# NickTravers/NeuralNetworkLibrary

Hardware: AMD Instinct MI355X
Metric: ResNet-34 224x224 training throughput (Learner.train1minibatch, fwd+loss+bwd+optimizer) (higher is better)
Workload: dtype f32; 1 GPU; DogsCats ResNet-34 classifier, 224x224, bs=64 per GPU, SGD momentum 0.9, fp32; global_batch=64, image_size=224, parallelism=dp1

## Files before the change

include/nnl.h:

```cpp
#ifndef NNL_H_
#define NNL_H_

#include <stddef.h>
#include <stdint.h>

#ifdef __cplusplus
extern "C" {
#endif

typedef enum {
  NNL_OK = 0,
  NNL_ERR_INVALID_ARG = -1,
  NNL_ERR_HIP = -2,
  NNL_ERR_UNSUPPORTED = -3,
  NNL_ERR_WORKSPACE = -4
} nnl_status_t;

int nnl_version(void);
const char* nnl_last_error(void);
int nnl_reload_env(void);

enum { NNL_PROF_CONV_FWD = 0, NNL_PROF_CONV_DGRAD = 1, NNL_PROF_CONV_WGRAD = 2, NNL_PROF_EMBDOT = 3,
       NNL_PROF_TABULAR = 4, NNL_PROF_RETINA_LOSS = 5, NNL_PROF_LSTM = 6, NNL_PROF_SOFTMAX_CE = 7,
       NNL_PROF_ELEMENTWISE = 8, NNL_PROF_GEMM = 9, NNL_PROF_OPTIM = 10, NNL_PROF_KINDS = 11 };
int nnl_prof_enable(int enable);
int nnl_prof_collect(int64_t* launches, double* total_ms, double* total_work);
int nnl_prof_collect2(int64_t* launches, double* total_ms, double* total_work, double* total_exec);
int nnl_dp_bump(int32_t* step, void* stream);
int nnl_dp_signal(int32_t* flag, const int32_t* step, void* stream);
int nnl_dp_wait(const int32_t* flag, int32_t value, int64_t timeout_us, int32_t* err, void* stream);
const char* nnl_source_stamp(void);

int nnl_embdotbias_fwd(const int64_t* x, const float* U, const float* M, const float* bu, const float* bi,
                       float* y, float* z, int64_t n, int64_t n_user, int64_t n_item, int64_t D,
                       int has_range, float lo, float hi, int32_t* err_flag, void* stream);
size_t nnl_embdotbias_bwd_workspace_bytes(int64_t n);
int nnl_embdotbias_bwd(const int64_t* x, const float* U, const float* M, const float* z, const float* dy,
                       float* dU, float* dM, float* dbu, float* dbi, int64_t n, int64_t n_user,
                       int64_t n_item, int64_t D, int has_range, float lo, float hi, void* workspace, size_t workspace_bytes, void* stream);

typedef struct {
  int32_t N, H, W, C;
  int32_t K, R, S;
  int32_t stride, pad;
  int32_t P, Q;
} nnl_conv_geom_t;

size_t nnl_conv2d_fwd_workspace_bytes(const nnl_conv_geom_t* g);
int64_t nnl_conv2d_tile_counters(void);
int nnl_conv2d_fwd(const float* x, const float* w, const float* bias, float* y, const nnl_conv_geom_t* g,
                   int relu, void* workspace, size_t workspace_bytes, int32_t* tile_counters, float* bn_partials,
                   const float* bn_pivot, int32_t* bn_rows, void* stream);
int nnl_conv2d_fwd_add_up2(const float* x, const float* w, const float* bias, const float* small, float* y,
                           const nnl_conv_geom_t* g, void* stream);
int nnl_upsample2_bwd(const float* dy, float* dsmall, int64_t N, int64_t h, int64_t w, int64_t C, void* stream);
int nnl_conv2d_weight_transpose(const float* w, float* wt, int K, int R, int S, int C, void* stream);
typedef struct {
  const float* w;
  float* wt;
  int32_t K, RS, C, first_tile;
} nnl_wt_desc_t;
int nnl_conv2d_weight_transpose_multi(const nnl_wt_desc_t* desc, const int32_t* tile_tensor, int64_t n_tiles,
                                      double total_elems, void* stream);
size_t nnl_conv2d_dgrad_workspace_bytes(const nnl_conv_geom_t* g);
int nnl_conv2d_dgrad(const float* dy, const float* wt, float* dx, const nnl_conv_geom_t* g, const float* addend,
                     void* workspace, size_t workspace_bytes, int32_t* tile_counters, void* stream);
typedef struct {
  const float* src;
  float* dst;
  int32_t rows, ch, flip, first_block;
  int32_t two_d, reserved;
} nnl_wino_desc_t;
int nnl_conv2d_wino_preferred(const nnl_conv_geom_t* g, int dgrad);
int nnl_wino_filter_multi(const nnl_wino_desc_t* desc, const int32_t* block_desc, int64_t n_blocks, void* stream);
int nnl_conv2d_fwd_pre(const float* x, const float* w, const float* bias, float* y, const nnl_conv_geom_t* g, int relu,
                       void* workspace, size_t workspace_bytes, int32_t* tile_counters, float* bn_partials, const float* bn_pivot,
                       int32_t* bn_rows, const float* u, void* stream);
int nnl_conv2d_dgrad_pre(const float* dy, const float* wt, float* dx, const nnl_conv_geom_t* g, const float* addend,
                         void* workspace, size_t workspace_bytes, int32_t* tile_counters, const float* u, void* stream);
size_t nnl_debug_conv_wino_workspace_bytes(int N, int H, int W, int C, int K);
int nnl_debug_conv_wino_fwd(const float* x, const float* filt, const float* bias, const float* add, float* y, void* ws,
                            size_t ws_bytes, int32_t* counters, long n_counters, float* bn_part, const float* bn_pivot, int N,
                            int H, int W, int C, int K, int relu, int flip, void* stream);
size_t nnl_debug_conv_wino2_workspace_bytes(int N, int H, int W, int C, int K);
int nnl_debug_conv_wino2_fwd(const float* x, const float* filt, const float* bias, const float* add, float* y, void* ws,
                            size_t ws_bytes, int32_t* counters, long n_counters, float* bn_part, const float* bn_pivot, int N,
                            int H, int W, int C, int K, int relu, int flip, void* stream);
int nnl_debug_conv_plan_times(int N, int H, int W, int C, int K, double* out);

int nnl_debug_route_record(int enable);
int nnl_debug_route_collect(char* out, size_t n);
size_t nnl_conv2d_wgrad_workspace_bytes(const nnl_conv_geom_t* g);
int nnl_conv2d_wgrad(const float* x, const float* dy, float* dw, const nnl_conv_geom_t* g, void* workspace,
                     size_t workspace_bytes, void* stream);
size_t nnl_colsum_workspace_bytes(int64_t rows, int64_t cols);
int nnl_sum_tensors(const float* const* src, int n, float* out, int64_t numel, void* stream);
int nnl_colsum(const float* a, float* out, int64_t rows, int64_t cols, void* workspace, size_t workspace_bytes,
               void* stream);
int nnl_relu_gate_colsum(const float* dy, const float* y, float* g, float* colsum, int64_t rows, int64_t cols, void* workspace,
                         size_t workspace_bytes, void* stream);
int nnl_act_gate_colsum(const float* dy, const float* y, float* g, float* colsum, int64_t rows, int64_t cols, int act,
                        void* workspace, size_t workspace_bytes, void* stream);

size_t nnl_bn_workspace_bytes(int64_t rows, int64_t C);
int nnl_bn_fwd(const float* x, const float* gamma, const float* beta, const float* residual, float* y,
               float* save_mean, float* save_invstd, float* running_mean, float* running_var, int64_t rows,
               int64_t C, float eps, float momentum, int training, int relu, int64_t* num_batches_tracked,
               uint32_t* relu_mask, const float* ext_partials, int64_t ext_rows, const float* ext_pivot, float* pivot_out,
               void* workspace, size_t workspace_bytes, void* stream);
int nnl_bn_bwd(const float* dy, const float* y, const uint32_t* relu_mask, const float* x, const float* gamma,
               const float* mean, const float* invstd, float* dx, float* dres, float* dgamma, float* dbeta, int64_t rows,
               int64_t C, int training, int relu, void* workspace, size_t workspace_bytes, void* stream);

int nnl_bn_relu_maxpool_supported(int64_t C);
int nnl_bn_relu_maxpool_fwd(const float* x, const float* gamma, const float* beta, float* y, uint8_t* idx, float* save_mean,
                            float* save_invstd, float* save_scale, float* save_shift, float* running_mean, float* running_var,
                            int64_t N, int64_t H, int64_t W, int64_t C, int64_t P, int64_t Q, int ks, int stride, int pad, float eps,
                            float momentum, int training, int64_t* num_batches_tracked, void* workspace, size_t workspace_bytes,
                            void* stream);
int nnl_bn_relu_maxpool_bwd(const float* dpool, const float* y, const uint8_t* idx, const float* x, const float* gamma,
                            const float* beta, const float* mean, const float* invstd, const float* scale, const float* shift,
                            float* dx, float* dgamma, float* dbeta,
                            int64_t N, int64_t H, int64_t W, int64_t C, int64_t P, int64_t Q, int ks, int stride, int pad,
                            int training, void* workspace, size_t workspace_bytes, void* stream);

int nnl_bn_sync_stats(const float* x, float* stats, int64_t rows, int64_t C, void* workspace, size_t workspace_bytes,
                      void* stream);
int nnl_bn_sync_fwd(const float* x, const float* all_stats, int world, const float* gamma, const float* beta,
                    const float* residual, float* y, float* save_mean, float* save_invstd, float* running_mean,
                    float* running_var, int64_t rows, int64_t C, float eps, float momentum, int relu,
                    int64_t* num_batches_tracked, uint32_t* relu_mask, void* workspace, size_t workspace_bytes, void* stream);
int nnl_bn_sync_bwd_reduce(const float* dy, const float* y, const uint32_t* relu_mask, const float* x, const float* mean,
                           const float* invstd, float* sums, int64_t rows, int64_t C, int relu, void* workspace,
                           size_t workspace_bytes, void* stream);
int nnl_bn_sync_bwd(const float* dy, const float* y, const uint32_t* relu_mask, const float* x, const float* gamma,
                    const float* mean, const float* invstd, const float* local_sums, const float* global_sums,
                    const float* all_stats,
                    int world, float* dx, float* dres, float* dgamma, float* dbeta, int64_t rows, int64_t C, int relu,
                    void* workspace, size_t workspace_bytes, void* stream);

int nnl_maxpool2d_fwd(const float* x, float* y, uint8_t* idx, int64_t N, int64_t H, int64_t W, int64_t C, int64_t P,
                      int64_t Q, int ksize, int stride, int pad, void* stream);
int nnl_maxpool2d_bwd(const float* dy, const uint8_t* idx, float* dx, int64_t N, int64_t H, int64_t W, int64_t C,
                      int64_t P, int64_t Q, int ksize, int stride, int pad, void* stream);
int nnl_concat_pool_fwd(const float* x, float* out, int32_t* argmax, int64_t N, int64_t HW, int64_t C, void* stream);
int nnl_concat_pool_bwd(const float* dout, const int32_t* argmax, float* dx, int64_t N, int64_t HW, int64_t C, void* stream);

int nnl_bbox_decode(const float* anchors, const float* reg, const float* clas, int64_t bs, int64_t A, int64_t K,
                    const float* mean4, const float* std4, float thresh, float width, float height, float* cand_boxes,
                    int32_t* cand_classes, float* cand_scores, int32_t* cand_order, int32_t* cand_count, void* stream);
size_t nnl_nms_workspace_bytes(int64_t bs, int64_t top_k);
int nnl_nms(const float* cand_boxes, const int32_t* cand_classes, const float* cand_scores, const int32_t* cand_order,
            const int32_t* cand_count, int64_t bs, int64_t cap, int64_t top_k, float max_overlap, float* kept_boxes,
            int32_t* kept_classes, float* kept_scores, int32_t* kept_count, void* workspace, size_t workspace_bytes,
            void* stream);

int nnl_tab_renorm(const int64_t* xcat, float* const* tables, const int32_t* card, const int32_t* dim,
                   const int32_t* row_off, const int32_t* row_table, int32_t* flags, int64_t bs, int32_t ncat,
                   int32_t total_rows, float max_norm, int32_t* err_flag, void* stream);
int nnl_tab_gather_fwd(const int64_t* xcat, const float* const* tables, const int32_t* card, const int32_t* dim,
                       const int32_t* col_off, const int32_t* col_table, const float* row_mask, const float* cont,
                       const float* cont_mask, float* out, int64_t bs, int32_t ncat, int32_t cat_width,
                       int32_t n_cont, int32_t ld_out, void* stream);
size_t nnl_tab_scatter_bwd_workspace_bytes(int64_t bs, int32_t ncat);
int nnl_tab_scatter_bwd(const int64_t* xcat, const int32_t* card, const int32_t* dim, const int32_t* col_off,
                        const int32_t* col_table, const int64_t* grad_off, const float* row_mask,
                        const float* cont_mask, const float* dout, float* dtab_flat, int64_t dtab_elems,
                        float* dcont, int64_t bs, int32_t ncat, int32_t cat_width, int32_t n_cont, int32_t ld_out,
                        void* workspace, size_t workspace_bytes, void* stream);
int nnl_tab_scan_bwd(const int64_t* xcat, const int32_t* card, const int32_t* dim, const int32_t* col_off,
                     const int64_t* grad_off, const float* row_mask, const float* cont_mask, const float* dout,
                     float* dtab_flat, float* dcont, const int32_t* blk_col, const int32_t* blk_first, int32_t n_scan_blocks,
                     int32_t max_dim, int64_t bs, int32_t ncat, int32_t cat_width, int32_t n_cont, int32_t ld_out, void* stream);

int nnl_pad_cols(const float* src, float* dst, int64_t rows, int64_t C, int64_t Cp, void* stream);
int nnl_keep_masks(const float* u, float* a, int64_t na, float keep_a, float* b, int64_t nb, float keep_b, void* stream);

int nnl_linear_small_supported(int64_t N);
int nnl_linear_small_fwd(const float* x, const float* w, const float* bias, float* y, int64_t M, int64_t K, int64_t ldx, int64_t N,
                         void* stream);
size_t nnl_linear_small_bwd_workspace_bytes(int64_t M, int64_t K, int64_t N);
int nnl_linear_small_bwd(const float* dy, const float* x, const float* w, float* dx, float* dw, float* db, int64_t M, int64_t K,
                         int64_t ldx, int64_t N, void* workspace, size_t workspace_bytes, void* stream);

size_t nnl_retina_loss_workspace_bytes(int64_t bs, int64_t A);
int nnl_retina_loss_fwd(const float* anchors, const float* reg, const float* clas, const float* boxes,
                        const int64_t* cats, int32_t* state, float* npos, float* out, int64_t bs, int64_t A,
                        int64_t K, int64_t M, float beta, float alpha, float gamma, void* workspace,
                        size_t workspace_bytes, void* stream);
int nnl_retina_loss_bwd(const float* anchors, const float* reg, const float* clas, const float* boxes,
                        const int64_t* cats, const int32_t* state, const float* npos, const float* grad_out,
                        float* dreg, float* dclas, int64_t bs, int64_t A, int64_t K, int64_t M, float beta,
                        float alpha, float gamma, void* stream);

int64_t nnl_lstm_padded_hidden(int64_t H);
// ... 59 lines not shown
```

neuralnetworklibrary_amd/Applications/VisionModels/resnet.py:

```python
import torch.nn as nn

from .retinanet import BasicBlock, Bottleneck, HipConv2d, HipMaxPool2d, _Downsample
from ... import ops

__all__ = ['ResNet', 'resnet18', 'resnet34', 'resnet50', 'resnet101', 'resnet152']


class ResNet(nn.Module):
    def __init__(self, block, layers, num_classes=1000):
        super().__init__()
        self.inplanes = 64
        self.conv1 = HipConv2d(3, 64, kernel_size=7, stride=2, padding=3, bias=False)
        self.bn1 = nn.BatchNorm2d(64)
        self.relu = nn.ReLU(inplace=True)
        self.maxpool = HipMaxPool2d(kernel_size=3, stride=2, padding=1)
        self.layer1 = self._make_layer(block, 64, layers[0])
        self.layer2 = self._make_layer(block, 128, layers[1], stride=2)
        self.layer3 = self._make_layer(block, 256, layers[2], stride=2)
        self.layer4 = self._make_layer(block, 512, layers[3], stride=2)
        self.avgpool = nn.AdaptiveAvgPool2d((1, 1))
        self.fc = nn.Linear(512 * block.expansion, num_classes)
        for m in self.modules():
            if isinstance(m, nn.Conv2d):
                nn.init.kaiming_normal_(m.weight, mode='fan_out', nonlinearity='relu')
            elif isinstance(m, nn.BatchNorm2d):
                nn.init.constant_(m.weight, 1)
                nn.init.constant_(m.bias, 0)

    def _make_layer(self, block, planes, blocks, stride=1):
        downsample = None
        if stride != 1 or self.inplanes != planes * block.expansion:
            downsample = _Downsample(
                HipConv2d(self.inplanes, planes * block.expansion, kernel_size=1, stride=stride, bias=False),
                nn.BatchNorm2d(planes * block.expansion))
        layers = [block(self.inplanes, planes, stride, downsample)]
        self.inplanes = planes * block.expansion
        for _ in range(1, blocks):
            layers.append(block(self.inplanes, planes))
        return nn.Sequential(*layers)

    def forward(self, x):
        x = ops.conv_bn_relu_maxpool(self.conv1, self.bn1, self.maxpool, x)
        x = self.layer4(self.layer3(self.layer2(self.layer1(x))))
        x = self.avgpool(x).flatten(1)
        return ops.linear(x, self.fc.weight, self.fc.bias, relu=False)


class ResNetBody(nn.Sequential):

    def forward(self, x):
        mods = list(self.children())
        if len(mods) >= 4 and isinstance(mods[0], HipConv2d) and isinstance(mods[1], nn.BatchNorm2d) \
                and isinstance(mods[2], nn.ReLU) and isinstance(mods[3], nn.MaxPool2d):
            x = ops.conv_bn_relu_maxpool(mods[0], mods[1], mods[3], x)
            mods = mods[4:]
        elif len(mods) >= 3 and isinstance(mods[0], HipConv2d) and isinstance(mods[1], nn.BatchNorm2d) \
                and isinstance(mods[2], nn.ReLU):
            x = ops.conv_bn_act(mods[0], mods[1], x, relu=True)
            mods = mods[3:]
        for m in mods:
            x = m(x)
        return x


def resnet18(pretrained=False, **kw):
    return ResNet(BasicBlock, [2, 2, 2, 2], **kw)


def resnet34(pretrained=False, **kw):
    return ResNet(BasicBlock, [3, 4, 6, 3], **kw)


def resnet50(pretrained=False, **kw):
    return ResNet(Bottleneck, [3, 4, 6, 3], **kw)


def resnet101(pretrained=False, **kw):
    return ResNet(Bottleneck, [3, 4, 23, 3], **kw)


def resnet152(pretrained=False, **kw):
    return ResNet(Bottleneck, [3, 8, 36, 3], **kw)
```

neuralnetworklibrary_amd/Applications/VisionModels/retinanet.py:

```python
import numpy as np
import torch
import torch.nn as nn

from ... import ops
from ...General.Core import default_device

__all__ = ['HipConv2d', 'conv3x3', 'BasicBlock', 'Bottleneck', 'PyramidFeatures', 'RegressionModel',
           'ClassificationModel', 'RetinaNet', 'retinanet18', 'retinanet34', 'retinanet50', 'retinanet101',
           'retinanet152', 'get_anchor_set', 'get_anchor_shifts', 'AnchorGenerator', 'intersections', 'jaccard', 'nms',
           'BBoxPredictor']


class HipConv2d(nn.Conv2d):
    fuse_relu = False
    nnl_hip_conv = True

    def __init__(self, *args, **kwargs):
        super().__init__(*args, **kwargs)
        self.weight.data = self.weight.data.contiguous(memory_format=torch.channels_last)

    def forward(self, x, grad_slot=None, give_slot=None):
        if self.dilation != (1, 1) or self.groups != 1 or self.stride[0] != self.stride[1] \
                or self.padding[0] != self.padding[1] or self.padding_mode != 'zeros':
            raise NotImplementedError('HipConv2d: only the symmetric, dense convolutions the reference uses')
        return ops.conv2d(x, ops.fan_param(self.weight), ops.fan_param(self.bias), self.stride[0], self.padding[0], relu=self.fuse_relu,
                          grad_slot=grad_slot, give_slot=give_slot)


class HipMaxPool2d(nn.MaxPool2d):

    def forward(self, x):
        k, s, p = self.kernel_size, self.stride, self.padding
        if self.dilation != 1 or self.ceil_mode or self.return_indices or not all(isinstance(v, int) for v in (k, s, p)):
            raise NotImplementedError('HipMaxPool2d: only the square floor-mode pooling the reference uses')
        return ops.maxpool2d(x, k, s, p)


class _ConvReLU(HipConv2d):
    fuse_relu = True


def conv3x3(in_planes, out_planes, stride=1):
    return HipConv2d(in_planes, out_planes, kernel_size=3, stride=stride, padding=1, bias=False)


class BasicBlock(nn.Module):
    expansion = 1

    def __init__(self, inplanes, planes, stride=1, downsample=None):
        super().__init__()
        self.conv1 = conv3x3(inplanes, planes, stride)
        self.bn1 = nn.BatchNorm2d(planes)
        self.relu = nn.ReLU(inplace=True)
        self.conv2 = conv3x3(planes, planes)
        self.bn2 = nn.BatchNorm2d(planes)
        self.downsample = downsample
        self.stride = stride

    def forward(self, x):
        slot = ops.GradSlot() if (x.requires_grad and torch.is_grad_enabled()) else None
        out = ops.conv_bn_act(self.conv1, self.bn1, x, relu=True, conv_slot=slot)
        if self.downsample is None:
            return ops.conv_bn_act(self.conv2, self.bn2, out, residual=x, relu=True, bn_slot=slot)
        return ops.conv_bn_act(self.conv2, self.bn2, out, residual=_shortcut(self.downsample, x, slot), relu=True)


class Bottleneck(nn.Module):
    expansion = 4

    def __init__(self, inplanes, planes, stride=1, downsample=None):
        super().__init__()
        self.conv1 = HipConv2d(inplanes, planes, kernel_size=1, bias=False)
        self.bn1 = nn.BatchNorm2d(planes)
        self.conv2 = HipConv2d(planes, planes, kernel_size=3, stride=stride, padding=1, bias=False)
        self.bn2 = nn.BatchNorm2d(planes)
        self.conv3 = HipConv2d(planes, planes * 4, kernel_size=1, bias=False)
        self.bn3 = nn.BatchNorm2d(planes * 4)
        self.relu = nn.ReLU(inplace=True)
        self.downsample = downsample
        self.stride = stride

    def forward(self, x):
        slot = ops.GradSlot() if (x.requires_grad and torch.is_grad_enabled()) else None
        out = ops.conv_bn_act(self.conv1, self.bn1, x, relu=True, conv_slot=slot)
        out = ops.conv_bn_act(self.conv2, self.bn2, out, relu=True)
        if self.downsample is None:
            return ops.conv_bn_act(self.conv3, self.bn3, out, residual=x, relu=True, bn_slot=slot)
        return ops.conv_bn_act(self.conv3, self.bn3, out, residual=_shortcut(self.downsample, x, slot), relu=True)


class _Downsample(nn.Sequential):

    def forward(self, x, give_slot=None):
        return ops.conv_bn_act(self[0], self[1], x, relu=False, conv_give=give_slot)


def _shortcut(downsample, x, slot):
    return downsample(x, give_slot=slot) if isinstance(downsample, _Downsample) else downsample(x)


class PyramidFeatures(nn.Module):

    def __init__(self, C3_size, C4_size, C5_size, feature_size=256):
        super().__init__()
        self.P5_1 = HipConv2d(C5_size, feature_size, kernel_size=1, stride=1, padding=0)
        self.P5_upsampled = nn.Upsample(scale_factor=2, mode='nearest')
        self.P5_2 = HipConv2d(feature_size, feature_size, kernel_size=3, stride=1, padding=1)
        self.P4_1 = HipConv2d(C4_size, feature_size, kernel_size=1, stride=1, padding=0)
        self.P4_upsampled = nn.Upsample(scale_factor=2, mode='nearest')
        self.P4_2 = HipConv2d(feature_size, feature_size, kernel_size=3, stride=1, padding=1)
        self.P3_1 = HipConv2d(C3_size, feature_size, kernel_size=1, stride=1, padding=0)
        self.P3_2 = HipConv2d(feature_size, feature_size, kernel_size=3, stride=1, padding=1)
        self.P6 = HipConv2d(C5_size, feature_size, kernel_size=3, stride=2, padding=1)
        self.P7_1 = nn.ReLU()
        self.P7_2 = HipConv2d(feature_size, feature_size, kernel_size=3, stride=2, padding=1)

    @staticmethod
    def _fusable(lateral, big, small):
        return (big.is_cuda and lateral.kernel_size == (1, 1) and lateral.stride == (1, 1) and big.shape[1] % 16 == 0
                and big.shape[2] == 2 * small.shape[2] and big.shape[3] == 2 * small.shape[3])

    def forward(self, inputs):
        C3, C4, C5 = inputs
        P5_x = self.P5_1(C5)
        if self._fusable(self.P4_1, C4, P5_x) and self._fusable(self.P3_1, C3, C4):
            P4_x = ops.conv_add_upsampled(C4, self.P4_1.weight, self.P4_1.bias, P5_x)
            P5_x = self.P5_2(P5_x)
            P3_x = self.P3_2(ops.conv_add_upsampled(C3, self.P3_1.weight, self.P3_1.bias, P4_x))
            P4_x = self.P4_2(P4_x)
        else:
            P5_up = self.P5_upsampled(P5_x)
            P5_x = self.P5_2(P5_x)
            P4_x = P5_up + self.P4_1(C4)
            P4_up = self.P4_upsampled(P4_x)
            P4_x = self.P4_2(P4_x)
            P3_x = self.P3_2(self.P3_1(C3) + P4_up)
        P6_x = self.P6(C5)
        P7_x = self.P7_2(self.P7_1(P6_x))
        return [P3_x, P4_x, P5_x, P6_x, P7_x]


class _Head(nn.Module):

    def _build(self, num_features_in, feature_size, n_out, bn, drop):
        self.drop0 = nn.Dropout(drop[0]) if drop else None
        self.drop = nn.Dropout(drop[1]) if drop else None
        self.bn0 = nn.BatchNorm2d(num_features_in, momentum=0.01) if bn else None
        chans = [num_features_in, feature_size, feature_size, feature_size, feature_size]
        for i in range(1, 5):
            setattr(self, 'conv%d' % i, _ConvReLU(chans[i - 1], feature_size, kernel_size=3, padding=1))
            setattr(self, 'act%d' % i, nn.ReLU())
            setattr(self, 'bn%d' % i, nn.BatchNorm2d(feature_size, momentum=0.01) if bn else None)
        self.output = HipConv2d(feature_size, n_out, kernel_size=3, padding=1)

    def _trunk(self, x, sigmoid=False):
        if self.bn0:
            x = self.bn0(x)
        if self.drop0:
            x = self.drop0(x)
        out = x
        for i in range(1, 5):
            out = getattr(self, 'conv%d' % i)(out)
            bn = getattr(self, 'bn%d' % i)
            if bn:
                out = bn(out)
            if self.drop:
                out = self.drop(out)
        o = self.output
        if sigmoid and out.shape[1] % 16 == 0 and o.stride == (1, 1) and o.padding[0] == o.padding[1]:
            return ops.conv2d(out, o.weight, o.bias, 1, o.padding[0], relu=2)
        out = o(out)
        return self.output_act(out) if sigmoid else out


class RegressionModel(_Head):

    def __init__(self, num_features_in, num_anchors=9, feature_size=256, bn=False, drop=None):
        super().__init__()
        self._build(num_features_in, feature_size, num_anchors * 4, bn, drop)

    def forward(self, x):
        out = self._trunk(x)
        return out.permute(0, 2, 3, 1).reshape(out.shape[0], -1, 4)


class ClassificationModel(_Head):

    def __init__(self, num_features_in, num_anchors=9, num_classes=80, feature_size=256, bn=False, drop=None):
        super().__init__()
        self.num_classes, self.num_anchors = num_classes, num_anchors
        self._build(num_features_in, feature_size, num_anchors * num_classes, bn, drop)
        self.output_act = nn.Sigmoid()

    def forward(self, x):
        out = self._trunk(x, sigmoid=True)
        return out.permute(0, 2, 3, 1).reshape(out.shape[0], -1, self.num_classes)


class RetinaNet(nn.Module):

    def __init__(self, num_classes, block, layers):
        self.inplanes = 64
        super().__init__()
        self.conv1 = HipConv2d(3, 64, kernel_size=7, stride=2, padding=3, bias=False)
        self.bn1 = nn.BatchNorm2d(64)
        self.relu = nn.ReLU(inplace=True)
        self.maxpool = HipMaxPool2d(kernel_size=3, stride=2, padding=1)
        self.layer1 = self._make_layer(block, 64, layers[0])
        self.layer2 = self._make_layer(block, 128, layers[1], stride=2)
        self.layer3 = self._make_layer(block, 256, layers[2], stride=2)
        self.layer4 = self._make_layer(block, 512, layers[3], stride=2)
        last = 'conv2' if block == BasicBlock else 'conv3'
        fpn_sizes = [getattr(self.layer2[layers[1] - 1], last).out_channels,
                     getattr(self.layer3[layers[2] - 1], last).out_channels,
                     getattr(self.layer4[layers[3] - 1], last).out_channels]
        self.fpn = PyramidFeatures(fpn_sizes[0], fpn_sizes[1], fpn_sizes[2])
        self.regressionModel = RegressionModel(256)
        self.classificationModel = ClassificationModel(256, num_classes=num_classes)
        self.AnchorGenerator = AnchorGenerator()
        self.BBoxPredictor = BBoxPredictor()
        init_retina_modules(self.modules())
        prior = 0.01
        nn.init.constant_(self.classificationModel.output.weight, 0)
        nn.init.constant_(self.classificationModel.output.bias, -np.log((1.0 - prior) / prior))
        nn.init.constant_(self.regressionModel.output.weight, 0)
        nn.init.constant_(self.regressionModel.output.bias, 0)

    def _make_layer(self, block, planes, blocks, stride=1):
        downsample = None
        if stride != 1 or self.inplanes != planes * block.expansion:
            downsample = _Downsample(
                HipConv2d(self.inplanes, planes * block.expansion, kernel_size=1, stride=stride, bias=False),
                nn.BatchNorm2d(planes * block.expansion))
        layers = [block(self.inplanes, planes, stride, downsample)]
        self.inplanes = planes * block.expansion
        for _ in range(1, blocks):
            layers.append(block(self.inplanes, planes))
        return nn.Sequential(*layers)

    def stem(self, x):
        return ops.conv_bn_relu_maxpool(self.conv1, self.bn1, self.maxpool, x)

    def forward(self, img_batch):
        x = self.stem(img_batch)
        x1 = self.layer1(x)
        x2 = self.layer2(x1)
        x3 = self.layer3(x2)
        x4 = self.layer4(x3)
        features = self.fpn([x2, x3, x4])
        with ops.shared_params([self.regressionModel, self.classificationModel], len(features)):
            reg = torch.cat([self.regressionModel(f) for f in features], dim=1)
            clas = torch.cat([self.classificationModel(f) for f in features], dim=1)
        return [self.AnchorGenerator(img_batch), reg, clas]


def init_retina_modules(modules):
    for m in modules:
        if isinstance(m, nn.Conv2d):
            n = m.kernel_size[0] * m.kernel_size[1] * m.out_channels
            nn.init.normal_(m.weight, mean=0.0, std=np.sqrt(2 / n))
        elif isinstance(m, nn.BatchNorm2d):
            nn.init.constant_(m.weight, 1)
            nn.init.constant_(m.bias, 0)


def retinanet18(num_classes, pretrained=False, **kwargs):
    return RetinaNet(num_classes, BasicBlock, [2, 2, 2, 2], **kwargs)


def retinanet34(num_classes, pretrained=False, **kwargs):
    return RetinaNet(num_classes, BasicBlock, [3, 4, 6, 3], **kwargs)


def retinanet50(num_classes, pretrained=False, **kwargs):
    return RetinaNet(num_classes, Bottleneck, [3, 4, 6, 3], **kwargs)


def retinanet101(num_classes, pretrained=False, **kwargs):
    return RetinaNet(num_classes, Bottleneck, [3, 4, 23, 3], **kwargs)


def retinanet152(num_classes, pretrained=False, **kwargs):
    return RetinaNet(num_classes, Bottleneck, [3, 8, 36, 3], **kwargs)


def retinanet(weights_path=None):
    model = RetinaNet(80, Bottleneck, [3, 4, 6, 3])
    if weights_path is not None:
        model.load_state_dict(torch.load(weights_path, map_location='cpu'))
    return model



def get_anchor_set(ratios=[0.5, 1, 2], scales=[2 ** 0, 2 ** (1 / 3), 2 ** (2 / 3)]):
    S = np.tile(scales, len(ratios))
    Rt = np.repeat(ratios, len(scales))
    Hs, Ws = S / np.sqrt(Rt), S * np.sqrt(Rt)
    return np.array([-Ws / 2, -Hs / 2, Ws / 2, Hs / 2]).T


def get_anchor_shifts(shape, stride, anchors):
    sx = (np.arange(0, shape[1]) + 0.5) * stride
    sy = (np.arange(0, shape[0]) + 0.5) * stride
    sx, sy = np.meshgrid(sx, sy)
    shifts = np.stack([sx.ravel(), sy.ravel(), sx.ravel(), sy.ravel()], axis=1)
    return (shifts[:, None, :] + anchors[None, :, :]).reshape(-1, 4)


class AnchorGenerator(object):

    def __init__(self, ratios=[0.5, 1, 2], scales=[2 ** 0, 2 ** (1 / 3), 2 ** (2 / 3)]):
        self.pyramid_levels = [3, 4, 5, 6, 7]
        self.strides = [2 ** x for x in self.pyramid_levels]
        self.sizes = [2 ** (x + 2) for x in self.pyramid_levels]
        self.ratios, self.scales = np.array(ratios), np.array(scales)
        self.anchor_set = get_anchor_set(ratios, scales)
        self._cache = {}

    def numpy_anchors(self, H, W):
        shape = np.array([H, W])
        out = []
# ... 150 lines not shown
```

neuralnetworklibrary_amd/_lib.py:

```python
import ctypes as C
import os

import torch

_HERE = os.path.dirname(os.path.abspath(__file__))
LIB_PATH = os.environ.get('NNL_LIB_PATH') or os.path.join(_HERE, 'libnnl_hip.so')

if not os.path.exists(LIB_PATH):
    raise ImportError(
        f"{LIB_PATH} not found: build it with `python -c 'import __graft_entry__ as g; g.build()'` "
        "(or `make -C neuralnetworklibrary_amd/csrc`). There is no CPU fallback for the HIP hot path.")

lib = C.CDLL(LIB_PATH)

c_p = C.c_void_p
i32, i64, f32, f64 = C.c_int32, C.c_int64, C.c_float, C.c_double
sz = C.c_size_t


class ConvGeom(C.Structure):
    _fields_ = [('N', i32), ('H', i32), ('W', i32), ('C', i32), ('K', i32), ('R', i32), ('S', i32),
                ('stride', i32), ('pad', i32), ('P', i32), ('Q', i32)]


SIGNATURES = {
    'nnl_version': (C.c_int, []),
    'nnl_last_error': (C.c_char_p, []),
    'nnl_reload_env': (C.c_int, []),
    'nnl_prof_enable': (C.c_int, [C.c_int]),
    'nnl_prof_collect': (C.c_int, [C.POINTER(i64), C.POINTER(f64), C.POINTER(f64)]),
    'nnl_prof_collect2': (C.c_int, [C.POINTER(i64), C.POINTER(f64), C.POINTER(f64), C.POINTER(f64)]),
    'nnl_source_stamp': (C.c_char_p, []),
    'nnl_dp_bump': (C.c_int, [c_p, c_p]),
    'nnl_dp_signal': (C.c_int, [c_p, c_p, c_p]),
    'nnl_dp_wait': (C.c_int, [c_p, i32, i64, c_p, c_p]),
    'nnl_embdotbias_fwd': (C.c_int, [c_p, c_p, c_p, c_p, c_p, c_p, c_p, i64, i64, i64, i64, C.c_int, f32, f32,
                                     c_p, c_p]),
    'nnl_embdotbias_bwd_workspace_bytes': (sz, [i64]),
    'nnl_embdotbias_bwd': (C.c_int, [c_p, c_p, c_p, c_p, c_p, c_p, c_p, c_p, c_p, i64, i64, i64, i64, C.c_int,
                                     f32, f32, c_p, sz, c_p]),
    'nnl_conv2d_fwd_workspace_bytes': (sz, [C.POINTER(ConvGeom)]),
    'nnl_conv2d_dgrad_workspace_bytes': (sz, [C.POINTER(ConvGeom)]),
    'nnl_conv2d_tile_counters': (i64, []),
    'nnl_conv2d_wino_preferred': (C.c_int, [C.POINTER(ConvGeom), C.c_int]),
    'nnl_wino_filter_multi': (C.c_int, [c_p, c_p, i64, c_p]),
    'nnl_conv2d_fwd_pre': (C.c_int, [c_p, c_p, c_p, c_p, C.POINTER(ConvGeom), C.c_int, c_p, sz, c_p, c_p, c_p, C.POINTER(i32), c_p, c_p]),
    'nnl_conv2d_dgrad_pre': (C.c_int, [c_p, c_p, c_p, C.POINTER(ConvGeom), c_p, c_p, sz, c_p, c_p, c_p]),
    'nnl_debug_conv_wino_workspace_bytes': (sz, [C.c_int] * 5),
    'nnl_debug_conv_wino_fwd': (C.c_int, [c_p] * 6 + [sz, c_p, C.c_long, c_p, c_p] + [C.c_int] * 7 + [c_p]),
    'nnl_debug_conv_wino2_workspace_bytes': (sz, [C.c_int] * 5),
    'nnl_debug_conv_wino2_fwd': (C.c_int, [c_p] * 6 + [sz, c_p, C.c_long, c_p, c_p] + [C.c_int] * 7 + [c_p]),
    'nnl_debug_conv_plan_times': (C.c_int, [C.c_int] * 5 + [C.POINTER(C.c_double)]),
    'nnl_debug_route_record': (C.c_int, [C.c_int]),
    'nnl_debug_route_collect': (C.c_int, [C.c_char_p, sz]),
    'nnl_conv2d_fwd': (C.c_int, [c_p, c_p, c_p, c_p, C.POINTER(ConvGeom), C.c_int, c_p, sz, c_p, c_p, c_p, C.POINTER(i32), c_p]),
    'nnl_conv2d_weight_transpose': (C.c_int, [c_p, c_p, C.c_int, C.c_int, C.c_int, C.c_int, c_p]),
    'nnl_conv2d_weight_transpose_multi': (C.c_int, [c_p, c_p, i64, f64, c_p]),
    'nnl_conv2d_dgrad': (C.c_int, [c_p, c_p, c_p, C.POINTER(ConvGeom), c_p, c_p, sz, c_p, c_p]),
    'nnl_conv2d_wgrad_workspace_bytes': (sz, [C.POINTER(ConvGeom)]),
    'nnl_conv2d_wgrad': (C.c_int, [c_p, c_p, c_p, C.POINTER(ConvGeom), c_p, sz, c_p]),
    'nnl_colsum_workspace_bytes': (sz, [i64, i64]),
    'nnl_colsum': (C.c_int, [c_p, c_p, i64, i64, c_p, sz, c_p]),
    'nnl_relu_gate_colsum': (C.c_int, [c_p, c_p, c_p, c_p, i64, i64, c_p, sz, c_p]),
    'nnl_conv2d_fwd_add_up2': (C.c_int, [c_p, c_p, c_p, c_p, c_p, C.POINTER(ConvGeom), c_p]),
    'nnl_upsample2_bwd': (C.c_int, [c_p, c_p, i64, i64, i64, i64, c_p]),
    'nnl_act_gate_colsum': (C.c_int, [c_p, c_p, c_p, c_p, i64, i64, C.c_int, c_p, sz, c_p]),
    'nnl_maxpool2d_fwd': (C.c_int, [c_p, c_p, c_p, i64, i64, i64, i64, i64, i64, C.c_int, C.c_int, C.c_int, c_p]),
    'nnl_maxpool2d_bwd': (C.c_int, [c_p, c_p, c_p, i64, i64, i64, i64, i64, i64, C.c_int, C.c_int, C.c_int, c_p]),
    'nnl_sum_tensors': (C.c_int, [c_p, C.c_int, c_p, i64, c_p]),
    'nnl_bn_relu_maxpool_supported': (C.c_int, [i64]),
    'nnl_bn_relu_maxpool_fwd': (C.c_int, [c_p, c_p, c_p, c_p, c_p, c_p, c_p, c_p, c_p, c_p, c_p, i64, i64, i64, i64, i64, i64,
                                          C.c_int, C.c_int, C.c_int, f32, f32, C.c_int, c_p, c_p, sz, c_p]),
    'nnl_bn_relu_maxpool_bwd': (C.c_int, [c_p, c_p, c_p, c_p, c_p, c_p, c_p, c_p, c_p, c_p, c_p, c_p, c_p, i64, i64, i64, i64, i64, i64,
                                          C.c_int, C.c_int, C.c_int, C.c_int, c_p, sz, c_p]),
    'nnl_concat_pool_fwd': (C.c_int, [c_p, c_p, c_p, i64, i64, i64, c_p]),
    'nnl_concat_pool_bwd': (C.c_int, [c_p, c_p, c_p, i64, i64, i64, c_p]),
    'nnl_bbox_decode': (C.c_int, [c_p, c_p, c_p, i64, i64, i64, c_p, c_p, f32, f32, f32, c_p, c_p, c_p, c_p, c_p, c_p]),
    'nnl_nms_workspace_bytes': (sz, [i64, i64]),
    'nnl_nms': (C.c_int, [c_p, c_p, c_p, c_p, c_p, i64, i64, i64, f32, c_p, c_p, c_p, c_p, c_p, sz, c_p]),
    'nnl_tab_renorm': (C.c_int, [c_p, c_p, c_p, c_p, c_p, c_p, c_p, i64, i32, i32, f32, c_p, c_p]),
    'nnl_tab_gather_fwd': (C.c_int, [c_p, c_p, c_p, c_p, c_p, c_p, c_p, c_p, c_p, c_p, i64, i32, i32, i32, i32, c_p]),
    'nnl_tab_scatter_bwd_workspace_bytes': (sz, [i64, i32]),
    'nnl_tab_scatter_bwd': (C.c_int, [c_p, c_p, c_p, c_p, c_p, c_p, c_p, c_p, c_p, c_p, i64, c_p, i64, i32, i32, i32, i32, c_p, sz, c_p]),
    'nnl_tab_scan_bwd': (C.c_int, [c_p] * 12 + [i32, i32, i64, i32, i32, i32, i32, c_p]),
    'nnl_pad_cols': (C.c_int, [c_p, c_p, i64, i64, i64, c_p]),
    'nnl_keep_masks': (C.c_int, [c_p, c_p, i64, f32, c_p, i64, f32, c_p]),
    'nnl_linear_small_supported': (C.c_int, [i64]),
    'nnl_linear_small_fwd': (C.c_int, [c_p, c_p, c_p, c_p, i64, i64, i64, i64, c_p]),
    'nnl_linear_small_bwd_workspace_bytes': (sz, [i64, i64, i64]),
    'nnl_linear_small_bwd': (C.c_int, [c_p, c_p, c_p, c_p, c_p, c_p, i64, i64, i64, i64, c_p, sz, c_p]),
    'nnl_retina_loss_workspace_bytes': (sz, [i64, i64]),
    'nnl_retina_loss_fwd': (C.c_int, [c_p, c_p, c_p, c_p, c_p, c_p, c_p, c_p, i64, i64, i64, i64, f32, f32, f32, c_p, sz, c_p]),
    'nnl_retina_loss_bwd': (C.c_int, [c_p, c_p, c_p, c_p, c_p, c_p, c_p, c_p, c_p, c_p, i64, i64, i64, i64, f32, f32, f32, c_p]),
    'nnl_lstm_padded_hidden': (i64, [i64]),
    'nnl_lstm_padded_gates': (i64, [i64]),
    'nnl_lstm_workspace_bytes': (sz, [i64, i64, i64]),
    'nnl_lstm_fwd': (C.c_int, [c_p, c_p, c_p, c_p, c_p, c_p, c_p, i64, i64, i64, c_p, sz, c_p, c_p]),
    'nnl_lstm_bwd': (C.c_int, [c_p, c_p, c_p, c_p, c_p, c_p, c_p, c_p, c_p, c_p, i64, i64, i64, c_p, sz, c_p, c_p]),
    'nnl_debug_lstm_bptt2_plan': (C.c_int, [i64, i64, c_p]),
    'nnl_embedding_rowmask_fwd': (C.c_int, [c_p, c_p, c_p, c_p, i64, i64, i64, c_p, c_p]),
    'nnl_embedding_rowmask_bwd_workspace_bytes': (sz, [i64]),
    'nnl_embedding_rowmask_bwd': (C.c_int, [c_p, c_p, c_p, c_p, i64, i64, i64, i64, c_p, sz, c_p]),
    'nnl_softmax_ce_fwd': (C.c_int, [c_p, c_p, c_p, c_p, c_p, i64, i64, c_p, c_p]),
    'nnl_softmax_ce_bwd': (C.c_int, [c_p, c_p, c_p, c_p, c_p, i64, i64, i64, c_p]),
    'nnl_mse_workspace_bytes': (sz, [i64]),
    'nnl_mse_fwd': (C.c_int, [c_p, c_p, c_p, i64, c_p, sz, c_p]),
    'nnl_mse_bwd': (C.c_int, [c_p, c_p, c_p, c_p, i64, c_p]),
    'nnl_scaled_sigmoid_fwd': (C.c_int, [c_p, c_p, c_p, i64, C.c_float, C.c_float, c_p]),
    'nnl_scaled_sigmoid_bwd': (C.c_int, [c_p, c_p, c_p, i64, C.c_float, C.c_float, c_p]),
    'nnl_seq_reg_workspace_bytes': (sz, [i64, i64]),
    'nnl_seq_reg_fwd': (C.c_int, [c_p, c_p, i64, i64, C.c_float, C.c_float, c_p, sz, c_p]),
    'nnl_seq_reg_bwd': (C.c_int, [c_p, c_p, c_p, i64, i64, C.c_float, C.c_float, c_p]),
    'nnl_weight_drop': (C.c_int, [c_p, i64, c_p, c_p, i64, i64, i64, C.c_uint64, C.c_float, c_p]),
    'nnl_attn_pool_workspace_bytes': (sz, [i64, i64, i64, i64]),
    'nnl_attn_pool_fwd': (C.c_int, [c_p, c_p, c_p, c_p, c_p, i64, c_p, c_p, i64, i64, i64, i64, c_p, sz, c_p, i64, c_p]),
    'nnl_attn_pool_bwd': (C.c_int, [c_p, c_p, c_p, c_p, c_p, c_p, c_p, c_p, c_p, c_p, i64, i64, i64, i64, c_p, sz, c_p, i64, c_p]),
    'nnl_optim_chunk_elems': (i64, []),
    'nnl_optim_patch': (C.c_int, [c_p, c_p, c_p, i64, c_p]),
    'nnl_optim_step': (C.c_int, [c_p, c_p, c_p, i64, C.c_int, c_p, C.c_int, c_p, c_p]),
    'nnl_bn_workspace_bytes': (sz, [i64, i64]),
    'nnl_bn_fwd': (C.c_int, [c_p, c_p, c_p, c_p, c_p, c_p, c_p, c_p, c_p, i64, i64, f32, f32, C.c_int, C.c_int, c_p, c_p, c_p, i64,
                             c_p, c_p, c_p, sz, c_p]),
    'nnl_bn_sync_stats': (C.c_int, [c_p, c_p, i64, i64, c_p, sz, c_p]),
    'nnl_bn_sync_fwd': (C.c_int, [c_p, c_p, C.c_int, c_p, c_p, c_p, c_p, c_p, c_p, c_p, c_p, i64, i64, f32, f32, C.c_int, c_p,
                                  c_p, c_p, sz, c_p]),
    'nnl_bn_sync_bwd_reduce': (C.c_int, [c_p, c_p, c_p, c_p, c_p, c_p, c_p, i64, i64, C.c_int, c_p, sz, c_p]),
    'nnl_bn_sync_bwd': (C.c_int, [c_p, c_p, c_p, c_p, c_p, c_p, c_p, c_p, c_p, c_p, C.c_int, c_p, c_p, c_p, c_p, i64, i64,
                                  C.c_int, c_p, sz, c_p]),
    'nnl_bn_bwd': (C.c_int, [c_p, c_p, c_p, c_p, c_p, c_p, c_p, c_p, c_p, c_p, c_p, i64, i64, C.c_int, C.c_int, c_p, sz, c_p]),
}

for _name, (_res, _args) in SIGNATURES.items():
    try:
        _fn = getattr(lib, _name)
    except AttributeError as e:
        raise ImportError(f"libnnl_hip.so does not export {_name}; rebuild it") from e
    _fn.restype = _res
    _fn.argtypes = _args

PROF_KINDS = ['conv_fwd', 'conv_dgrad', 'conv_wgrad', 'embdot', 'tabular', 'retina_loss', 'lstm',
              'softmax_ce', 'elementwise', 'gemm', 'optim']


class NnlError(RuntimeError):
    pass


def check(status):
    if status != 0:
        raise NnlError(f"nnl error {status}: {lib.nnl_last_error().decode()}")


def ptr(t):
    return None if t is None else C.c_void_p(t.data_ptr())


def stream():
    return C.c_void_p(torch.cuda.current_stream().cuda_stream)


def require_cuda(*tensors):
    for t in tensors:
        if t is not None and not t.is_cuda:
            raise NnlError("nnl HIP op called with a non-CUDA tensor: the MI355X path has no CPU fallback")


def prof_enable(flag=True):
    check(lib.nnl_prof_enable(1 if flag else 0))


def prof_collect():
    n = len(PROF_KINDS)
    a, b, c, d = (i64 * n)(), (f64 * n)(), (f64 * n)(), (f64 * n)()
    check(lib.nnl_prof_collect2(a, b, c, d))
    return {k: {'launches': int(a[i]), 'ms': float(b[i]), 'work': float(c[i]), 'exec': float(d[i])} for i, k in enumerate(PROF_KINDS)}


def source_stamp_of_tree():
    import glob
    import hashlib
    csrc = os.path.join(os.path.dirname(os.path.abspath(__file__)), 'csrc')
    names = sorted(os.path.basename(p) for p in glob.glob(os.path.join(csrc, '*.hip')) + glob.glob(os.path.join(csrc, '*.h')))
    hsh = hashlib.sha256()
    for p in [os.path.join(csrc, n) for n in names] + [os.path.join(csrc, 'Makefile'), os.path.join(csrc, '..', '..', 'include', 'nnl.h')]:
        with open(p, 'rb') as f:
            hsh.update(f.read())
    return hsh.hexdigest()[:16]


def source_stamp():
    return lib.nnl_source_stamp().decode()
```

neuralnetworklibrary_amd/csrc/batchnorm.hip:

```cpp
#include "nnl_common.h"

namespace {

typedef float f32x4 __attribute__((ext_vector_type(4)));

template <int VEC> struct VecT;
template <> struct VecT<4> { typedef f32x4 type; };
template <> struct VecT<1> { typedef float type; };

template <int VEC> __device__ __forceinline__ float vget(const typename VecT<VEC>::type& v, int i);
template <> __device__ __forceinline__ float vget<4>(const f32x4& v, int i) { return v[i]; }
template <> __device__ __forceinline__ float vget<1>(const float& v, int i) { return v; }
template <int VEC> __device__ __forceinline__ void vset(typename VecT<VEC>::type& v, int i, float x);
template <> __device__ __forceinline__ void vset<4>(f32x4& v, int i, float x) { v[i] = x; }
template <> __device__ __forceinline__ void vset<1>(float& v, int i, float x) { v = x; }

constexpr int kBlock = 256;
constexpr int kMaxRowBlocks = 1024;
constexpr int kFinLanes = 64;

struct Shape {
  int L;
  int rpb;
  int gx, gy;
// ... 273 lines not shown
                                                                const float* __restrict__ x, const float* __restrict__ mean,
                                                                const float* __restrict__ invstd, float* __restrict__ part,
                                                                long rows, int C, int L, int relu,
                                                                const unsigned* __restrict__ mask) {
  typedef typename VecT<VEC>::type V;
  __shared__ float red[kBlock * 2 * VEC];
  const int CG = C / VEC;
  const int tx = threadIdx.x & (L - 1), ty = threadIdx.x / L;
  const int rpb = kBlock / L;
  const int g = blockIdx.y * L + tx;
  const bool ok = g < CG;
  float s1[VEC], s2[VEC], mu[VEC], is[VEC];
#pragma unroll
  for (int e = 0; e < VEC; ++e) { s1[e] = 0.f; s2[e] = 0.f; mu[e] = 0.f; is[e] = 0.f; }
  if (ok) {
#pragma unroll
    for (int e = 0; e < VEC; ++e) { mu[e] = mean[(long)g * VEC + e]; is[e] = invstd[(long)g * VEC + e]; }
    const long rstep = (long)gridDim.x * rpb;
    long r = (long)blockIdx.x * rpb + ty;
    for (; r + rstep < rows; r += 2 * rstep) {
      V dv[2], xv[2], yv[2];
      unsigned kb[2] = {~0u, ~0u};
#pragma unroll
      for (int u = 0; u < 2; ++u) {
        const long off = (r + u * rstep) * C + (long)g * VEC;
        dv[u] = *reinterpret_cast<const V*>(dy + off);
        xv[u] = *reinterpret_cast<const V*>(x + off);
        yv[u] = dv[u];
        if (relu) {
          if (mask) kb[u] = keep_bits<VEC>(mask, off / VEC);
          else yv[u] = *reinterpret_cast<const V*>(y + off);
        }
      }
#pragma unroll
      for (int u = 0; u < 2; ++u)
#pragma unroll
        for (int e = 0; e < VEC; ++e) {
          float gg = vget<VEC>(dv[u], e);
          if (relu && (mask ? !((kb[u] >> e) & 1u) : !(vget<VEC>(yv[u], e) > 0.f))) gg = 0.f;
          s1[e] += gg;
          s2[e] += gg * ((vget<VEC>(xv[u], e) - mu[e]) * is[e]);
        }
    }
    for (; r < rows; r += rstep) {
      const long off = r * C + (long)g * VEC;
      const V dv = *reinterpret_cast<const V*>(dy + off);
      const V xv = *reinterpret_cast<const V*>(x + off);
      V yv = dv;
      unsigned kb = ~0u;
      if (relu) {
        if (mask) kb = keep_bits<VEC>(mask, off / VEC);
        else yv = *reinterpret_cast<const V*>(y + off);
      }
#pragma unroll
      for (int e = 0; e < VEC; ++e) {
        float gg = vget<VEC>(dv, e);
        if (relu && (mask ? !((kb >> e) & 1u) : !(vget<VEC>(yv, e) > 0.f))) gg = 0.f;
        s1[e] += gg;
        s2[e] += gg * ((vget<VEC>(xv, e) - mu[e]) * is[e]);
      }
    }
  }
#pragma unroll
  for (int e = 0; e < VEC; ++e) {
    red[(threadIdx.x * VEC + e) * 2 + 0] = s1[e];
    red[(threadIdx.x * VEC + e) * 2 + 1] = s2[e];
  }
  __syncthreads();
  if (ty == 0 && ok) {
#pragma unroll
    for (int e = 0; e < VEC; ++e) {
      float a = 0.f, b = 0.f;
      for (int j = 0; j < rpb; ++j) {
        a += red[((j * L + tx) * VEC + e) * 2 + 0];
        b += red[((j * L + tx) * VEC + e) * 2 + 1];
      }
      const long c = (long)g * VEC + e;
      part[((long)blockIdx.x * C + c) * 2 + 0] = a;
      part[((long)blockIdx.x * C + c) * 2 + 1] = b;
    }
  }
}

__global__ void bn_bwd_finalize_kernel(const float* __restrict__ part, int nparts, const float* __restrict__ gamma,
                                       const float* __restrict__ mean, const float* __restrict__ invstd,
                                       float* __restrict__ dgamma, float* __restrict__ dbeta, float* __restrict__ coef,
                                       long rows, int C, int training) {
  __shared__ float red[4][kFinLanes][2];
  const int c = blockIdx.x * 4 + threadIdx.x / kFinLanes;
  float s1, s2;
  reduce_partials(part, nparts, C, c, c < C, red, s1, s2);
  if (c >= C || (threadIdx.x & (kFinLanes - 1)) != 0) return;
  if (dbeta) dbeta[c] = s1;
  if (dgamma) dgamma[c] = s2;
  const float gm = gamma ? gamma[c] : 1.f;
  const float is = invstd[c], mu = mean[c];
  const float a = gm * is;
  if (training) {
    const float n = (float)rows;
    const float bq = -a * is * (s2 / n);
    coef[c] = a;
    coef[C + c] = bq;
    coef[2 * C + c] = -a * (s1 / n) - bq * mu;
  } else {
    coef[c] = a;
    coef[C + c] = 0.f;
    coef[2 * C + c] = 0.f;
  }
}

__global__ void bn_sync_bwd_sums_kernel(const float* __restrict__ part, int nparts, float* __restrict__ sums, int C) {
  __shared__ float red[4][kFinLanes][2];
  const int c = blockIdx.x * 4 + threadIdx.x / kFinLanes;
  float s1, s2;
  reduce_partials(part, nparts, C, c, c < C, red, s1, s2);
  if (c >= C || (threadIdx.x & (kFinLanes - 1)) != 0) return;
  sums[c] = s1;
  sums[C + c] = s2;
}

__global__ void bn_sync_bwd_coef_kernel(const float* __restrict__ local_sums, const float* __restrict__ global_sums,
                                        const float* __restrict__ all_stats, int world, const float* __restrict__ gamma,
                                        const float* __restrict__ mean, const float* __restrict__ invstd,
                                        float* __restrict__ dgamma, float* __restrict__ dbeta, float* __restrict__ coef, int C) {
  const int c = blockIdx.x * blockDim.x + threadIdx.x;
  if (c >= C) return;
  float n = 0.f;
  for (int r = 0; r < world; ++r) n += sync_count(all_stats + r * (2L * C + 2), C);
  if (dbeta) dbeta[c] = local_sums[c];
  if (dgamma) dgamma[c] = local_sums[C + c];
  const float s1 = global_sums[c], s2 = global_sums[C + c];
  const float is = invstd[c], mu = mean[c];
  const float a = (gamma ? gamma[c] : 1.f) * is;
  const float bq = -a * is * (s2 / n);
  coef[c] = a;
  coef[C + c] = bq;
  coef[2 * C + c] = -a * (s1 / n) - bq * mu;
}

template <int VEC>
__global__ __launch_bounds__(kBlock) void bn_bwd_apply_kernel(const float* __restrict__ dy, const float* __restrict__ y,
                                                               const float* __restrict__ x, const float* __restrict__ coef,
                                                               float* __restrict__ dx, float* __restrict__ dres,
                                                               long total_v, int CG, int C, int relu,
                                                               const unsigned* __restrict__ mask) {
  typedef typename VecT<VEC>::type V;
  const long stride = (long)gridDim.x * blockDim.x;
  const long i0 = (long)blockIdx.x * blockDim.x + threadIdx.x;
  const int g = (int)((unsigned)i0 % (unsigned)CG);
  const V ca = reinterpret_cast<const V*>(coef)[g];
  const V cb = reinterpret_cast<const V*>(coef + C)[g];
  const V cc = reinterpret_cast<const V*>(coef + 2 * C)[g];
  for (long i = i0; i < total_v; i += stride) {
    const V dv = reinterpret_cast<const V*>(dy)[i];
    const V xv = reinterpret_cast<const V*>(x)[i];
    V gv = dv;
    if (relu) {
      if (mask) {
        const unsigned kb = keep_bits<VEC>(mask, i);
#pragma unroll
        for (int e = 0; e < VEC; ++e)
          if (!((kb >> e) & 1u)) vset<VEC>(gv, e, 0.f);
      } else {
        const V yv = reinterpret_cast<const V*>(y)[i];
#pragma unroll
        for (int e = 0; e < VEC; ++e)
          if (!(vget<VEC>(yv, e) > 0.f)) vset<VEC>(gv, e, 0.f);
      }
    }
    V out;
#pragma unroll
    for (int e = 0; e < VEC; ++e)
      vset<VEC>(out, e, vget<VEC>(ca, e) * vget<VEC>(gv, e) + vget<VEC>(cb, e) * vget<VEC>(xv, e) + vget<VEC>(cc, e));
    reinterpret_cast<V*>(dx)[i] = out;
    if (dres) reinterpret_cast<V*>(dres)[i] = gv;
// ... 15 lines not shown

extern "C" size_t nnl_bn_workspace_bytes(int64_t rows, int64_t C) {
  if (rows <= 0 || C <= 0) return 0;
  return (size_t)((long)kMaxRowBlocks * C * 2 + 5 * C) * sizeof(float);
}

extern "C" int nnl_bn_fwd(const float* x, const float* gamma, const float* beta, const float* residual, float* y,
                          float* save_mean, float* save_invstd, float* running_mean, float* running_var, int64_t rows,
                          int64_t C, float eps, float momentum, int training, int relu, int64_t* num_batches_tracked,
                          uint32_t* relu_mask, const float* ext_partials, int64_t ext_rows, const float* ext_pivot,
                          float* pivot_out, void* workspace, size_t workspace_bytes, void* stream) {
  NNL_CHECK_ARG(rows > 0 && C > 0 && C < (1 << 24), "bn_fwd: bad sizes rows=%ld C=%ld", (long)rows, (long)C);
  NNL_CHECK_ARG(x && y && save_mean && save_invstd, "bn_fwd: null pointer");
  NNL_CHECK_ARG(training || (running_mean && running_var), "bn_fwd: eval mode needs running statistics");
  if (workspace == nullptr || workspace_bytes < nnl_bn_workspace_bytes(rows, C))
    return nnl_set_error(NNL_ERR_WORKSPACE, "bn_fwd: workspace too small");
  hipStream_t s = (hipStream_t)stream;
  float* part = (float*)workspace;
  float* scale = part + (long)kMaxRowBlocks * C * 2;
  float* shift = scale + C;
  const int VEC = (C % 4 == 0) ? 4 : 1;
  const long CG = C / VEC;
  NnlProfScope prof(NNL_PROF_ELEMENTWISE, s, (double)rows * C * (training ? 12.0 : 8.0) + (residual ? 4.0 * rows * C : 0.0));
  if (training && ext_partials != nullptr && ext_rows > 0 && ext_pivot != nullptr) {
    if (ext_rows >= 1024)
      hipLaunchKernelGGL(bn_finalize_kernel<256>, dim3((unsigned)C), dim3(256), 0, s, ext_pivot, ext_partials, (int)ext_rows, gamma, beta,
                         save_mean, save_invstd, running_mean, running_var, scale, shift, (long)rows, (int)C, eps, momentum,
                         (long long*)num_batches_tracked, pivot_out);
    else
      hipLaunchKernelGGL(bn_finalize_kernel<kFinLanes>, dim3((unsigned)nnl_cdiv(C, 4)), dim3(256), 0, s, ext_pivot, ext_partials,
                         (int)ext_rows, gamma, beta, save_mean, save_invstd, running_mean, running_var, scale, shift, (long)rows,
                         (int)C, eps, momentum, (long long*)num_batches_tracked, pivot_out);
    NNL_CHECK_LAUNCH();
  } else if (training) {
    const Shape sh = make_shape(rows, CG);
    if (VEC == 4)
      hipLaunchKernelGGL(bn_stats_kernel<4>, dim3(sh.gx, sh.gy), dim3(kBlock), 0, s, x, part, (long)rows, (int)C, sh.L);
    else
      hipLaunchKernelGGL(bn_stats_kernel<1>, dim3(sh.gx, sh.gy), dim3(kBlock), 0, s, x, part, (long)rows, (int)C, sh.L);
    NNL_CHECK_LAUNCH();
    hipLaunchKernelGGL(bn_finalize_kernel<kFinLanes>, dim3((unsigned)nnl_cdiv(C, 4)), dim3(256), 0, s, x, part, sh.gx, gamma, beta,
                       save_mean, save_invstd, running_mean, running_var, scale, shift, (long)rows, (int)C, eps, momentum,
                       (long long*)num_batches_tracked, pivot_out);
    NNL_CHECK_LAUNCH();
  } else {
    NNL_CHECK_HIP(hipMemcpyAsync(save_mean, running_mean, sizeof(float) * C, hipMemcpyDeviceToDevice, s));
    hipLaunchKernelGGL(bn_eval_scale_kernel, dim3((unsigned)nnl_cdiv(C, 256)), dim3(256), 0, s, gamma, beta, running_mean,
                       running_var, scale, shift, save_invstd, (int)C, eps);
    NNL_CHECK_LAUNCH();
  }
  const long total_v = rows * CG;
  if (VEC == 4)
    hipLaunchKernelGGL(bn_apply_kernel<4>, dim3(ew_grid(total_v, CG)), dim3(kBlock), 0, s, x, scale, shift, residual, y, total_v,
                       (int)CG, relu, relu ? relu_mask : nullptr);
  else
    hipLaunchKernelGGL(bn_apply_kernel<1>, dim3(ew_grid(total_v, CG)), dim3(kBlock), 0, s, x, scale, shift, residual, y, total_v,
                       (int)CG, relu, relu ? relu_mask : nullptr);
  NNL_CHECK_LAUNCH();
  return NNL_OK;
}

extern "C" int nnl_bn_bwd(const float* dy, const float* y, const uint32_t* relu_mask, const float* x, const float* gamma,
                          const float* mean, const float* invstd, float* dx, float* dres, float* dgamma, float* dbeta,
                          int64_t rows, int64_t C, int training, int relu, void* workspace, size_t workspace_bytes,
                          void* stream) {
  NNL_CHECK_ARG(rows > 0 && C > 0 && C < (1 << 24), "bn_bwd: bad sizes");
  NNL_CHECK_ARG(dy && x && mean && invstd && dx && (y || relu_mask || !relu), "bn_bwd: null pointer");
  if (workspace == nullptr || workspace_bytes < nnl_bn_workspace_bytes(rows, C))
    return nnl_set_error(NNL_ERR_WORKSPACE, "bn_bwd: workspace too small");
  hipStream_t s = (hipStream_t)stream;
  float* part = (float*)workspace;
  float* coef = part + (long)kMaxRowBlocks * C * 2 + 2 * C;
  const int VEC = (C % 4 == 0) ? 4 : 1;
  const long CG = C / VEC;
  const Shape sh = make_shape(rows, CG);
  NnlProfScope prof(NNL_PROF_ELEMENTWISE, s, (double)rows * C * (relu ? 28.0 : 20.0) + (dres ? 4.0 * rows * C : 0.0));
  if (VEC == 4)
    hipLaunchKernelGGL(bn_bwd_reduce_kernel<4>, dim3(sh.gx, sh.gy), dim3(kBlock), 0, s, dy, y, x, mean, invstd, part, (long)rows,
                       (int)C, sh.L, relu, relu_mask);
  else
    hipLaunchKernelGGL(bn_bwd_reduce_kernel<1>, dim3(sh.gx, sh.gy), dim3(kBlock), 0, s, dy, y, x, mean, invstd, part, (long)rows,
                       (int)C, sh.L, relu, relu_mask);
  NNL_CHECK_LAUNCH();
  hipLaunchKernelGGL(bn_bwd_finalize_kernel, dim3((unsigned)nnl_cdiv(C, 4)), dim3(256), 0, s, part, sh.gx, gamma, mean, invstd,
                     dgamma, dbeta, coef, (long)rows, (int)C, training);
  NNL_CHECK_LAUNCH();
  const long total_v = rows * CG;
  if (VEC == 4)
    hipLaunchKernelGGL(bn_bwd_apply_kernel<4>, dim3(ew_grid(total_v, CG)), dim3(kBlock), 0, s, dy, y, x, coef, dx, dres, total_v,
                       (int)CG, (int)C, relu, relu_mask);
  else
    hipLaunchKernelGGL(bn_bwd_apply_kernel<1>, dim3(ew_grid(total_v, CG)), dim3(kBlock), 0, s, dy, y, x, coef, dx, dres, total_v,
                       (int)CG, (int)C, relu, relu_mask);
  NNL_CHECK_LAUNCH();
  return NNL_OK;
}

namespace {

__device__ __forceinline__ f32x4 bnpool_affine(const f32x4& x, const f32x4& sc, const f32x4& sh) {
  f32x4 z;
#pragma unroll
  for (int e = 0; e < 4; ++e) z[e] = x[e] * sc[e] + sh[e];
  return z;
}

__global__ __launch_bounds__(kBlock) void bnpool_fwd_kernel(const float* __restrict__ x, const float* __restrict__ scale,
                                                            const float* __restrict__ shift, float* __restrict__ y,
                                                            uint8_t* __restrict__ idx, int N, int H, int W, int C4, int P, int Q,
                                                            int ks, int stride, int pad) {
  const long total = (long)N * P * Q * C4;
  const long i0 = (long)blockIdx.x * blockDim.x + threadIdx.x;
  const int c4 = (int)(i0 % C4);
  const f32x4 sc = reinterpret_cast<const f32x4*>(scale)[c4], sh = reinterpret_cast<const f32x4*>(shift)[c4];
  for (long i = i0; i < total; i += (long)gridDim.x * blockDim.x) {
    long r = i / C4;
    const int q = (int)(r % Q); r /= Q;
    const int p = (int)(r % P);
    const int n = (int)(r / P);
    f32x4 best = {0.f, 0.f, 0.f, 0.f};
    int bi[4] = {-1, -1, -1, -1};
    for (int kh = 0; kh < ks; ++kh) {
      const int h = p * stride - pad + kh;
      if ((unsigned)h >= (unsigned)H) continue;
      for (int kw = 0; kw < ks; ++kw) {
        const int w = q * stride - pad + kw;
        if ((unsigned)w >= (unsigned)W) continue;
        f32x4 v = bnpool_affine(reinterpret_cast<const f32x4*>(x)[((long)(n * H + h) * W + w) * C4 + c4], sc, sh);
        const int t = kh * ks + kw;
#pragma unroll
        for (int e = 0; e < 4; ++e) {
          v[e] = (v[e] != v[e]) ? v[e] : fmaxf(v[e], 0.f);
          if (bi[e] < 0 || v[e] > best[e] || v[e] != v[e]) { best[e] = v[e]; bi[e] = t; }
        }
      }
    }
    reinterpret_cast<f32x4*>(y)[i] = best;
    reinterpret_cast<uchar4*>(idx)[i] = make_uchar4((uint8_t)bi[0], (uint8_t)bi[1], (uint8_t)bi[2], (uint8_t)bi[3]);
  }
}

struct PoolGeom { int H, W, C4, P, Q, ks, stride, pad; };

__device__ __forceinline__ f32x4 bnpool_grad(const float* __restrict__ dpool, const uint8_t* __restrict__ idx, const f32x4& xv,
                                             const f32x4& sc, const f32x4& sh, int n, int h, int w, int c4, const PoolGeom& g) {
  f32x4 acc = {0.f, 0.f, 0.f, 0.f};
  int p_lo = h + g.pad - g.ks + 1; p_lo = p_lo > 0 ? (p_lo + g.stride - 1) / g.stride : 0;
  int p_hi = (h + g.pad) / g.stride; if (p_hi > g.P - 1) p_hi = g.P - 1;
  int q_lo = w + g.pad - g.ks + 1; q_lo = q_lo > 0 ? (q_lo + g.stride - 1) / g.stride : 0;
  int q_hi = (w + g.pad) / g.stride; if (q_hi > g.Q - 1) q_hi = g.Q - 1;
  for (int p = p_lo; p <= p_hi; ++p) {
    const int kh = h + g.pad - p * g.stride;
    for (int q = q_lo; q <= q_hi; ++q) {
      const int t = kh * g.ks + (w + g.pad - q * g.stride);
      const long o = ((long)(n * g.P + p) * g.Q + q) * g.C4 + c4;
      const uchar4 id = reinterpret_cast<const uchar4*>(idx)[o];
      const f32x4 d = reinterpret_cast<const f32x4*>(dpool)[o];
      if (id.x == t) acc[0] += d[0];
      if (id.y == t) acc[1] += d[1];
      if (id.z == t) acc[2] += d[2];
      if (id.w == t) acc[3] += d[3];
    }
  }
  const f32x4 z = bnpool_affine(xv, sc, sh);
#pragma unroll
  for (int e = 0; e < 4; ++e) if (!(z[e] > 0.f)) acc[e] = 0.f;
  return acc;
}

constexpr int kPoolRedBlock = 1024;

__global__ __launch_bounds__(kPoolRedBlock) void bnpool_bwd_reduce_kernel(const float* __restrict__ dpool, const uint8_t* __restrict__ idx,
                                                                   const float* __restrict__ x, const float* __restrict__ scale,
                                                                   const float* __restrict__ shift, const float* __restrict__ mean,
                                                                   const float* __restrict__ invstd, float* __restrict__ part,
                                                                   int N, int C, PoolGeom g) {
// ... 108 lines not shown
    f32x4 out;
#pragma unroll
    for (int e = 0; e < 4; ++e) out[e] = ca[e] * gg[e] + cb[e] * xv[e] + cc[e];
    reinterpret_cast<f32x4*>(dx)[i] = out;
  }
}

bool bnpool_ok(long C) { return C % 4 == 0 && C >= 4 && C <= 1024 && (kBlock % (C / 4)) == 0; }
unsigned bnpool_grid(long total) {
  long g = nnl_cdiv(total, (long)kPoolRedBlock * 4);
  if (g > kMaxRowBlocks) g = kMaxRowBlocks;
  return (unsigned)(g < 1 ? 1 : g);
}

}

extern "C" int nnl_bn_relu_maxpool_supported(int64_t C) { return bnpool_ok(C) ? 1 : 0; }

extern "C" int nnl_bn_relu_maxpool_fwd(const float* x, const float* gamma, const float* beta, float* y, uint8_t* idx,
                                       float* save_mean, float* save_invstd, float* save_scale, float* save_shift,
                                       float* running_mean, float* running_var, int64_t N, int64_t H, int64_t W, int64_t C,
                                       int64_t P, int64_t Q, int ks, int stride, int pad, float eps, float momentum, int training,
                                       int64_t* num_batches_tracked, void* workspace, size_t workspace_bytes, void* stream) {
  const long rows = (long)N * H * W;
  NNL_CHECK_ARG(N > 0 && H > 0 && W > 0 && P > 0 && Q > 0 && ks > 0 && ks * ks <= 255 && stride > 0 && pad >= 0 && 2 * pad <= ks,
                "bn_relu_maxpool_fwd: bad geometry");
  NNL_CHECK_ARG(P == (H + 2 * pad - ks) / stride + 1 && Q == (W + 2 * pad - ks) / stride + 1, "bn_relu_maxpool_fwd: P/Q do not match");
  NNL_CHECK_ARG(bnpool_ok(C), "bn_relu_maxpool_fwd: C=%ld needs C %% 4 == 0 and C/4 dividing 256", (long)C);
  NNL_CHECK_ARG(x && y && idx && save_mean && save_invstd && save_scale && save_shift, "bn_relu_maxpool_fwd: null pointer");
  NNL_CHECK_ARG(training || (running_mean && running_var), "bn_relu_maxpool_fwd: eval mode needs running statistics");
  NNL_CHECK_ARG(rows * C < (1L << 31) * 4, "bn_relu_maxpool_fwd: tensor too large");
  if (workspace == nullptr || workspace_bytes < nnl_bn_workspace_bytes(rows, C))
    return nnl_set_error(NNL_ERR_WORKSPACE, "bn_relu_maxpool_fwd: workspace too small");
  hipStream_t s = (hipStream_t)stream;
  float* part = (float*)workspace;
  float* scale = save_scale;
  float* shift = save_shift;
  const long CG = C / 4;
  NnlProfScope prof(NNL_PROF_ELEMENTWISE, s, (double)rows * C * (training ? 8.0 : 4.0) + (double)N * P * Q * C * 5.0);
  if (training) {
    const Shape sh = make_shape(rows, CG);
    hipLaunchKernelGGL(bn_stats_kernel<4>, dim3(sh.gx, sh.gy), dim3(kBlock), 0, s, x, part, rows, (int)C, sh.L);
    NNL_CHECK_LAUNCH();
    hipLaunchKernelGGL(bn_finalize_kernel<kFinLanes>, dim3((unsigned)nnl_cdiv(C, 4)), dim3(256), 0, s, x, part, sh.gx, gamma, beta,
                       save_mean, save_invstd, running_mean, running_var, scale, shift, rows, (int)C, eps, momentum,
                       (long long*)num_batches_tracked, (float*)nullptr);
    NNL_CHECK_LAUNCH();
  } else {
    NNL_CHECK_HIP(hipMemcpyAsync(save_mean, running_mean, sizeof(float) * C, hipMemcpyDeviceToDevice, s));
    hipLaunchKernelGGL(bn_eval_scale_kernel, dim3((unsigned)nnl_cdiv(C, 256)), dim3(256), 0, s, gamma, beta, running_mean,
                       running_var, scale, shift, save_invstd, (int)C, eps);
    NNL_CHECK_LAUNCH();
  }
  const long total = (long)N * P * Q * CG;
  hipLaunchKernelGGL(bnpool_fwd_kernel, dim3((unsigned)nnl_cdiv(total, kBlock)), dim3(kBlock), 0, s, x, scale, shift, y, idx, (int)N,
                     (int)H, (int)W, (int)CG, (int)P, (int)Q, ks, stride, pad);
  NNL_CHECK_LAUNCH();
  return NNL_OK;
}

extern "C" int nnl_bn_relu_maxpool_bwd(const float* dpool, const float* y, const uint8_t* idx, const float* x, const float* gamma,
                                       const float* beta, const float* mean, const float* invstd, const float* scale,
                                       const float* shift, float* dx, float* dgamma, float* dbeta, int64_t N,
                                       int64_t H, int64_t W, int64_t C, int64_t P, int64_t Q, int ks, int stride, int pad,
                                       int training, void* workspace, size_t workspace_bytes, void* stream) {
  const long rows = (long)N * H * W;
  NNL_CHECK_ARG(N > 0 && H > 0 && W > 0 && P > 0 && Q > 0 && ks > 0 && stride > 0 && pad >= 0, "bn_relu_maxpool_bwd: bad geometry");
  NNL_CHECK_ARG(bnpool_ok(C), "bn_relu_maxpool_bwd: C=%ld needs C %% 4 == 0 and C/4 dividing 256", (long)C);
  NNL_CHECK_ARG(dpool && idx && x && mean && invstd && scale && shift && dx, "bn_relu_maxpool_bwd: null pointer");
  if (workspace == nullptr || workspace_bytes < nnl_bn_workspace_bytes(rows, C))
    return nnl_set_error(NNL_ERR_WORKSPACE, "bn_relu_maxpool_bwd: workspace too small");
  hipStream_t s = (hipStream_t)stream;
  float* part = (float*)workspace;
  float* coef = part + (long)kMaxRowBlocks * C * 2 + 2 * C;
  const PoolGeom g{(int)H, (int)W, (int)(C / 4), (int)P, (int)Q, ks, stride, pad};
  const long total = rows * (C / 4);
  const unsigned grid = bnpool_grid(total);
  NnlProfScope prof(NNL_PROF_ELEMENTWISE, s, (double)rows * C * 12.0 + (double)N * P * Q * C * 10.0);
  if (y != nullptr) {
    const unsigned go = bnpool_grid((long)N * P * Q * (C / 4));
    hipLaunchKernelGGL(bnpool_bwd_reduce_out_kernel, dim3(go), dim3(kPoolRedBlock), 0, s, dpool, y, idx, x, gamma, beta, mean, invstd,
                       part, (int)N, (int)C, g);
    NNL_CHECK_LAUNCH();
    hipLaunchKernelGGL(bn_bwd_finalize_kernel, dim3((unsigned)nnl_cdiv(C, 4)), dim3(256), 0, s, part, (int)go, gamma, mean, invstd,
                       dgamma, dbeta, coef, rows, (int)C, training);
    NNL_CHECK_LAUNCH();
  } else {
    hipLaunchKernelGGL(bnpool_bwd_reduce_kernel, dim3(grid), dim3(kPoolRedBlock), 0, s, dpool, idx, x, scale, shift, mean, invstd, part,
                       (int)N, (int)C, g);
    NNL_CHECK_LAUNCH();
    hipLaunchKernelGGL(bn_bwd_finalize_kernel, dim3((unsigned)nnl_cdiv(C, 4)), dim3(256), 0, s, part, (int)grid, gamma, mean, invstd,
                       dgamma, dbeta, coef, rows, (int)C, training);
    NNL_CHECK_LAUNCH();
  }
  hipLaunchKernelGGL(bnpool_bwd_apply_kernel, dim3((unsigned)nnl_cdiv(total, kBlock)), dim3(kBlock), 0, s, dpool, idx, x, scale, shift, coef, dx, (int)N, (int)C, g);
  NNL_CHECK_LAUNCH();
  return NNL_OK;
}

namespace {
int launch_stats(const float* x, float* part, long rows, long C, hipStream_t s, Shape& sh) {
  const int VEC = (C % 4 == 0) ? 4 : 1;
  sh = make_shape(rows, C / VEC);
  if (VEC == 4)
    hipLaunchKernelGGL(bn_stats_kernel<4>, dim3(sh.gx, sh.gy), dim3(kBlock), 0, s, x, part, rows, (int)C, sh.L);
  else
    hipLaunchKernelGGL(bn_stats_kernel<1>, dim3(sh.gx, sh.gy), dim3(kBlock), 0, s, x, part, rows, (int)C, sh.L);
  NNL_CHECK_LAUNCH();
  return NNL_OK;
}
}

extern "C" int nnl_bn_sync_stats(const float* x, float* stats, int64_t rows, int64_t C, void* workspace,
                                 size_t workspace_bytes, void* stream) {
  NNL_CHECK_ARG(rows > 0 && C > 0 && C < (1 << 24) && x && stats, "bn_sync_stats: bad arguments");
  if (workspace == nullptr || workspace_bytes < nnl_bn_workspace_bytes(rows, C))
    return nnl_set_error(NNL_ERR_WORKSPACE, "bn_sync_stats: workspace too small");
  hipStream_t s = (hipStream_t)stream;
  NnlProfScope prof(NNL_PROF_ELEMENTWISE, s, (double)rows * C * 4.0);
  Shape sh;
  int rc = launch_stats(x, (float*)workspace, rows, C, s, sh);
  if (rc != NNL_OK) return rc;
  hipLaunchKernelGGL(bn_sync_local_kernel, dim3((unsigned)nnl_cdiv(C, 4)), dim3(256), 0, s, x, (const float*)workspace, sh.gx,
                     stats, (long)rows, (int)C);
  NNL_CHECK_LAUNCH();
  return NNL_OK;
}

extern "C" int nnl_bn_sync_fwd(const float* x, const float* all_stats, int world, const float* gamma, const float* beta,
                               const float* residual, float* y, float* save_mean, float* save_invstd, float* running_mean,
                               float* running_var, int64_t rows, int64_t C, float eps, float momentum, int relu,
                               int64_t* num_batches_tracked, uint32_t* relu_mask, void* workspace, size_t workspace_bytes,
                               void* stream) {
  NNL_CHECK_ARG(rows > 0 && C > 0 && C < (1 << 24) && world > 0, "bn_sync_fwd: bad sizes");
  NNL_CHECK_ARG(x && y && all_stats && save_mean && save_invstd, "bn_sync_fwd: null pointer");
  if (workspace == nullptr || workspace_bytes < nnl_bn_workspace_bytes(rows, C))
    return nnl_set_error(NNL_ERR_WORKSPACE, "bn_sync_fwd: workspace too small");
  hipStream_t s = (hipStream_t)stream;
  float* scale = (float*)workspace + (long)kMaxRowBlocks * C * 2;
  float* shift = scale + C;
  NnlProfScope prof(NNL_PROF_ELEMENTWISE, s, (double)rows * C * 8.0 + (residual ? 4.0 * rows * C : 0.0));
  hipLaunchKernelGGL(bn_sync_merge_kernel, dim3((unsigned)nnl_cdiv(C, 256)), dim3(256), 0, s, all_stats, world, gamma, beta,
                     save_mean, save_invstd, running_mean, running_var, scale, shift, (int)C, eps, momentum,
                     (long long*)num_batches_tracked);
  NNL_CHECK_LAUNCH();
  const int VEC = (C % 4 == 0) ? 4 : 1;
  const long CG = C / VEC, total_v = rows * CG;
  if (VEC == 4)
    hipLaunchKernelGGL(bn_apply_kernel<4>, dim3(ew_grid(total_v, CG)), dim3(kBlock), 0, s, x, scale, shift, residual, y, total_v,
                       (int)CG, relu, relu ? relu_mask : nullptr);
  else
    hipLaunchKernelGGL(bn_apply_kernel<1>, dim3(ew_grid(total_v, CG)), dim3(kBlock), 0, s, x, scale, shift, residual, y, total_v,
                       (int)CG, relu, relu ? relu_mask : nullptr);
  NNL_CHECK_LAUNCH();
  return NNL_OK;
}

extern "C" int nnl_bn_sync_bwd_reduce(const float* dy, const float* y, const uint32_t* relu_mask, const float* x,
                                      const float* mean, const float* invstd, float* sums, int64_t rows, int64_t C, int relu,
                                      void* workspace, size_t workspace_bytes, void* stream) {
  NNL_CHECK_ARG(rows > 0 && C > 0 && C < (1 << 24), "bn_sync_bwd_reduce: bad sizes");
  NNL_CHECK_ARG(dy && x && mean && invstd && sums && (y || relu_mask || !relu), "bn_sync_bwd_reduce: null pointer");
  if (workspace == nullptr || workspace_bytes < nnl_bn_workspace_bytes(rows, C))
    return nnl_set_error(NNL_ERR_WORKSPACE, "bn_sync_bwd_reduce: workspace too small");
  hipStream_t s = (hipStream_t)stream;
  float* part = (float*)workspace;
  const int VEC = (C % 4 == 0) ? 4 : 1;
  const Shape sh = make_shape(rows, C / VEC);
  NnlProfScope prof(NNL_PROF_ELEMENTWISE, s, (double)rows * C * (relu ? 12.0 : 8.0));
  if (VEC == 4)
    hipLaunchKernelGGL(bn_bwd_reduce_kernel<4>, dim3(sh.gx, sh.gy), dim3(kBlock), 0, s, dy, y, x, mean, invstd, part, (long)rows,
                       (int)C, sh.L, relu, relu_mask);
  else
    hipLaunchKernelGGL(bn_bwd_reduce_kernel<1>, dim3(sh.gx, sh.gy), dim3(kBlock), 0, s, dy, y, x, mean, invstd, part, (long)rows,
// ... 36 lines not shown
```

neuralnetworklibrary_amd/csrc/conv2d.hip:

```cpp
#include "igemm_kernels.h"
#include "igemm_taps.h"
#include "wino.h"
#include "igemm_wgrad.h"
#include "igemm_wgrad2d.h"

#ifdef NNL_TAPS_TIMING
static void* g_wgrad_dbg = nullptr;
extern "C" void* nnl_debug_wgrad_stamps(void) { return g_wgrad_dbg; }
#endif

namespace {

int check_geom(const nnl_conv_geom_t* g, const char* who) {
  if (!g) return nnl_set_error(NNL_ERR_INVALID_ARG, "%s: null geometry", who);
  if (g->N <= 0 || g->H <= 0 || g->W <= 0 || g->C <= 0 || g->K <= 0 || g->R <= 0 || g->S <= 0 || g->stride <= 0 ||
      g->pad < 0)
    return nnl_set_error(NNL_ERR_INVALID_ARG, "%s: non-positive dimension", who);
  if (g->H + 2L * g->pad < g->R || g->W + 2L * g->pad < g->S)
    return nnl_set_error(NNL_ERR_INVALID_ARG, "%s: the %d x %d filter is larger than the padded input (%d x %d, pad %d)", who, g->R, g->S,
                         g->H, g->W, g->pad);
  const int P = (g->H + 2 * g->pad - g->R) / g->stride + 1, Q = (g->W + 2 * g->pad - g->S) / g->stride + 1;
  if (P != g->P || Q != g->Q || P <= 0 || Q <= 0)
    return nnl_set_error(NNL_ERR_INVALID_ARG, "%s: P,Q=(%d,%d) do not match the geometry (%d,%d)", who, g->P, g->Q, P, Q);
  if (g->C % 4 != 0)
// ... 842 lines not shown
  return nnl_conv2d_fwd_pre(x, w, bias, y, g, relu, workspace, workspace_bytes, tile_counters, bn_partials, bn_pivot, bn_rows, nullptr, stream);
}

extern "C" int nnl_conv2d_fwd_pre(const float* x, const float* w, const float* bias, float* y, const nnl_conv_geom_t* g,
                                  int relu, void* workspace, size_t workspace_bytes, int32_t* tile_counters, float* bn_partials,
                                  const float* bn_pivot, int32_t* bn_rows, const float* u, void* stream) {
  if (bn_rows) *bn_rows = 0;
  int st = check_geom(g, "conv2d_fwd");
  if (st) return st;
  NNL_CHECK_ARG(x && w && y, "conv2d_fwd: null pointer");
  NNL_CHECK_ARG(relu >= 0 && relu <= 2, "conv2d_fwd: relu (activation) must be 0 none, 1 ReLU or 2 sigmoid");
  hipStream_t s = (hipStream_t)stream;
  IgemmRowkParams p{};
  p.a = x; p.b = w; p.y = y; p.bias = bias;
  p.N = g->N; p.H = g->H; p.W = g->W; p.C = g->C; p.P = g->P; p.Q = g->Q;
  p.R = g->R; p.S = g->S; p.stride = g->stride; p.pad = g->pad;
  p.M = g->N * g->P * g->Q; p.Nc = g->K; p.Kg = g->R * g->S * g->C; p.relu = relu;
  NnlProfScope prof(NNL_PROF_CONV_FWD, s, 2.0 * p.M * (double)p.Nc * p.Kg);
  const long a_elems = (long)g->N * g->H * g->W * g->C, b_elems = (long)g->K * g->R * g->S * g->C;
  const int wmode = (relu != 2 && workspace != nullptr) ? wino_mode(g->N, g->H, g->W, g->C, g->K, g->R, g->S, g->stride, g->pad) : 0;
  if (wmode && workspace_bytes >= wino_mode_workspace(wmode, g->N, g->H, g->W, g->C, g->K)) {
    WinoProblem wq{};
    wq.in = x; wq.filt = w; wq.out = y; wq.bias = bias; wq.add = nullptr;
    wq.N = g->N; wq.H = g->H; wq.W = g->W; wq.Cin = g->C; wq.Nc = g->K; wq.relu = relu; wq.flip = 0;
    const bool stats = bn_partials && bn_pivot && bn_rows;
    wq.bn_part = stats ? bn_partials : nullptr; wq.bn_pivot = bn_pivot;
    wq.u_pre = u;
    st = wino_mode_launch(wmode, wq, workspace, workspace_bytes, tile_counters, kTileCounters, s);
    if (st == NNL_OK && stats) *bn_rows = wmode >= 2 ? nnl_wino2_bn_rows(g->N, g->H, g->W) : nnl_wino_bn_rows(g->N, g->H, g->W);
    return st;
  }
  if (const int tk = taps_kind(a_elems, b_elems, g->C, g->R * g->S)) {
    IgemmTapsParams q = fwd_taps_params(g, x, w, y, bias, relu);
    q.ktail = tk == 2;
    q.bn_part = (bn_partials && bn_pivot && bn_rows) ? bn_partials : nullptr; q.bn_pivot = bn_pivot;
    return dispatch_taps(q, s, workspace, workspace_bytes, tile_counters, bn_rows);
  }
  if (relu == 2) return nnl_set_error(NNL_ERR_UNSUPPORTED, "conv2d_fwd: the sigmoid epilogue needs C %% 16 == 0 (C=%d)", g->C);
  return dispatch_rowk<IGEMM_MODE_FWD>(p, s);
}

extern "C" int nnl_conv2d_fwd_add_up2(const float* x, const float* w, const float* bias, const float* small, float* y,
                                      const nnl_conv_geom_t* g, void* stream) {
  int st = check_geom(g, "conv2d_fwd_add_up2");
  if (st) return st;
  NNL_CHECK_ARG(x && w && y && small, "conv2d_fwd_add_up2: null pointer");
  NNL_CHECK_ARG(g->P % 2 == 0 && g->Q % 2 == 0, "conv2d_fwd_add_up2: the output (%d x %d) must be twice the small map", g->P, g->Q);
  const long a_elems = (long)g->N * g->H * g->W * g->C, b_elems = (long)g->K * g->R * g->S * g->C;
  if (!taps_ok(a_elems, b_elems, g->C, g->R * g->S))
    return nnl_set_error(NNL_ERR_UNSUPPORTED, "conv2d_fwd_add_up2: needs C %% 16 == 0 (C=%d)", g->C);
  hipStream_t s = (hipStream_t)stream;
  const long M = (long)g->N * g->P * g->Q;
  NnlProfScope prof(NNL_PROF_CONV_FWD, s, 2.0 * M * (double)g->K * g->R * g->S * g->C);
  IgemmTapsParams q = fwd_taps_params(g, x, w, y, bias, 0);
  q.add = small; q.add_up2 = 1;
  return dispatch_taps(q, s);
}

extern "C" int nnl_conv2d_weight_transpose(const float* w, float* wt, int K, int R, int S, int C, void* stream) {
  NNL_CHECK_ARG(w && wt && K > 0 && R > 0 && S > 0 && C > 0, "conv2d_weight_transpose: bad argument");
  hipStream_t s = (hipStream_t)stream;
  NnlProfScope prof(NNL_PROF_ELEMENTWISE, s, 8.0 * K * R * S * C);
  hipLaunchKernelGGL(weight_transpose_kernel, dim3((unsigned)nnl_cdiv(C, 32), (unsigned)nnl_cdiv(K, 32), R * S), dim3(256), 0, s, w,
                     wt, K, R * S, C);
  NNL_CHECK_LAUNCH();
  return NNL_OK;
}

extern "C" int nnl_conv2d_weight_transpose_multi(const nnl_wt_desc_t* desc, const int32_t* tile_tensor, int64_t n_tiles,
                                                 double total_elems, void* stream) {
  NNL_CHECK_ARG(desc && tile_tensor && n_tiles > 0 && n_tiles < (1L << 31), "conv2d_weight_transpose_multi: bad argument");
  hipStream_t s = (hipStream_t)stream;
  NnlProfScope prof(NNL_PROF_ELEMENTWISE, s, 8.0 * total_elems);
  hipLaunchKernelGGL(weight_transpose_multi_kernel, dim3((unsigned)n_tiles), dim3(256), 0, s, desc, tile_tensor);
  NNL_CHECK_LAUNCH();
  return NNL_OK;
}

extern "C" int nnl_conv2d_dgrad(const float* dy, const float* wt, float* dx, const nnl_conv_geom_t* g, const float* addend,
                                void* workspace, size_t workspace_bytes, int32_t* tile_counters, void* stream) {
  return nnl_conv2d_dgrad_pre(dy, wt, dx, g, addend, workspace, workspace_bytes, tile_counters, nullptr, stream);
}

extern "C" int nnl_conv2d_dgrad_pre(const float* dy, const float* wt, float* dx, const nnl_conv_geom_t* g, const float* addend,
                                    void* workspace, size_t workspace_bytes, int32_t* tile_counters, const float* u, void* stream) {
  int st = check_geom(g, "conv2d_dgrad");
  if (st) return st;
  NNL_CHECK_ARG(dy && wt && dx, "conv2d_dgrad: null pointer");
  NNL_CHECK_ARG(g->K % 4 == 0, "conv2d_dgrad: K=%d must be a multiple of 4", g->K);
  {
    const bool taps = taps_ok((long)g->N * g->P * g->Q * g->K, (long)g->C * g->R * g->S * g->K, g->K, g->R * g->S) && dgrad_tap_table_ok(g);
    const bool s2_full = g->stride == 2 && g->R == 3 && g->S == 3 && g->pad == 1;
    if (addend != nullptr && !(taps && (g->stride == 1 || s2_full)))
      return nnl_set_error(NNL_ERR_UNSUPPORTED, "conv2d_dgrad: the fused addend needs K %% 16 == 0 and stride 1 (or a 3x3 / pad 1 filter at stride 2)");
  }
  hipStream_t s = (hipStream_t)stream;
  IgemmRowkParams p{};
  p.a = dy; p.b = wt; p.y = dx; p.bias = nullptr;
  p.N = g->N; p.H = g->P; p.W = g->Q; p.C = g->K;
  p.P = g->H; p.Q = g->W;
  p.R = g->R; p.S = g->S; p.stride = g->stride; p.pad = g->pad;
  p.M = g->N * g->H * g->W; p.Nc = g->C; p.Kg = g->R * g->S * g->K; p.relu = 0;
  NnlProfScope prof(NNL_PROF_CONV_DGRAD, s, 2.0 * g->N * (double)g->P * g->Q * g->K * g->R * g->S * g->C);
  const long a_elems = (long)g->N * g->P * g->Q * g->K, b_elems = (long)g->C * g->R * g->S * g->K;
  const int wmode = workspace != nullptr ? wino_mode(g->N, g->P, g->Q, g->K, g->C, g->R, g->S, g->stride, g->pad) : 0;
  if (wmode && workspace_bytes >= wino_mode_workspace(wmode, g->N, g->P, g->Q, g->K, g->C)) {
    WinoProblem wq{};
    wq.in = dy; wq.filt = wt; wq.out = dx; wq.bias = nullptr; wq.add = addend;
    wq.N = g->N; wq.H = g->P; wq.W = g->Q; wq.Cin = g->K; wq.Nc = g->C; wq.relu = 0; wq.flip = 1;
    wq.u_pre = u;
    return wino_mode_launch(wmode, wq, workspace, workspace_bytes, tile_counters, kTileCounters, s);
  }
  const int tk = dgrad_tap_table_ok(g) ? taps_kind(a_elems, b_elems, g->K, g->R * g->S) : 0;
  if (tk && (g->stride == 1 || g->stride == 2)) {
    IgemmTapsParams q{};
    q.ktail = tk == 2;
    q.a = dy; q.b = wt; q.y = dx; q.bias = nullptr; q.add = addend;
    q.a_bytes = (unsigned)(a_elems * 4); q.b_bytes = (unsigned)(b_elems * 4);
    q.H = g->P; q.W = g->Q; q.C = g->K;
    q.in_stride = 1; q.ih0 = 0; q.iw0 = 0;
    q.OH = g->H; q.OW = g->W; q.Nc = g->C; q.b_row_stride = g->R * g->S * g->K; q.relu = 0;
    const int st2 = g->stride;
    struct Cls { int ph, pw, P, Q, nt; signed char dh[IGEMM_MAX_TAPS], dw[IGEMM_MAX_TAPS]; int aoff[IGEMM_MAX_TAPS], woff[IGEMM_MAX_TAPS]; };
    Cls cls[4];
    int ncls = 0;
    bool need_zero = false;
    for (int ph = 0; ph < st2; ++ph)
      for (int pw = 0; pw < st2; ++pw) {
        Cls c{};
        c.ph = ph; c.pw = pw;
        c.P = (g->H - ph + st2 - 1) / st2; c.Q = (g->W - pw + st2 - 1) / st2;
        for (int r = 0; r < g->R; ++r) {
          if ((ph + g->pad - r) % st2 != 0) continue;
          for (int ss = 0; ss < g->S; ++ss) {
            if ((pw + g->pad - ss) % st2 != 0) continue;
            const int dh = (ph + g->pad - r) / st2, dw = (pw + g->pad - ss) / st2;
            c.dh[c.nt] = (signed char)dh; c.dw[c.nt] = (signed char)dw;
            c.aoff[c.nt] = (dh * g->Q + dw) * g->K; c.woff[c.nt] = (r * g->S + ss) * g->K;
            ++c.nt;
          }
        }
        if (c.P <= 0 || c.Q <= 0) continue;
        if (c.nt == 0) { need_zero = true; continue; }
        cls[ncls++] = c;
      }
    if (need_zero) NNL_ROUTE("dgrad:need_zero");
    if (need_zero) NNL_CHECK_HIP(hipMemsetAsync(dx, 0, sizeof(float) * g->N * g->H * g->W * g->C, s));
    auto fill = [&](IgemmTapsParams& c, const Cls& k, int at) {
      for (int t = 0; t < k.nt; ++t) {
        c.tap_dh[at + t] = k.dh[t]; c.tap_dw[at + t] = k.dw[t]; c.tap_aoff[at + t] = k.aoff[t]; c.tap_woff[at + t] = k.woff[t];
      }
    };
    bool merged = ncls > 1;
    for (int i = 1; i < ncls && merged; ++i) merged = cls[i].P == cls[0].P && cls[i].Q == cls[0].Q;
    if (merged) {
      NNL_ROUTE("dgrad:merged@ncls=%d", ncls);
      for (int i = 1; i < ncls; ++i)
        for (int j = i; j > 0 && cls[j].nt > cls[j - 1].nt; --j) { const Cls t = cls[j]; cls[j] = cls[j - 1]; cls[j - 1] = t; }
      IgemmTapsParams c = q;
      c.P = cls[0].P; c.Q = cls[0].Q; c.M = g->N * c.P * c.Q;
      c.out_stride = st2; c.oh0 = cls[0].ph; c.ow0 = cls[0].pw;
      c.ncls = ncls;
      int at = 0;
      for (int i = 0; i < ncls; ++i) {
        c.cls_tap0[i] = at; c.cls_ntaps[i] = cls[i].nt; c.cls_oh0[i] = cls[i].ph; c.cls_ow0[i] = cls[i].pw;
        fill(c, cls[i], at);
        at += cls[i].nt;
      }
      c.ntaps = cls[0].nt;
      return dispatch_taps(c, s, nullptr, 0, tile_counters);
    }
    if (st2 > 1) NNL_ROUTE("dgrad:per_class@ncls=%d", ncls);
    for (int i = 0; i < ncls; ++i) {
      IgemmTapsParams c = q;
      c.P = cls[i].P; c.Q = cls[i].Q; c.M = g->N * c.P * c.Q;
      c.out_stride = st2; c.oh0 = cls[i].ph; c.ow0 = cls[i].pw;
      fill(c, cls[i], 0);
      c.ntaps = cls[i].nt;
      if (st2 == 1 && cls[i].nt == g->R * g->S && affine_taps_ok(g->S)) {
        c.tap_affine = 1; c.tap_R = g->R; c.tap_S = g->S; c.tap_dh0 = g->pad; c.tap_dw0 = g->pad; c.tap_dstep = -1;
      }
      int st = dispatch_taps(c, s, st2 == 1 ? workspace : nullptr, workspace_bytes, tile_counters);
      if (st) return st;
    }
    return NNL_OK;
  }
  return dispatch_rowk<IGEMM_MODE_DGRAD>(p, s);
}

extern "C" size_t nnl_conv2d_wgrad_workspace_bytes(const nnl_conv_geom_t* g) {
  if (!g || check_geom(g, "conv2d_wgrad_workspace_bytes")) return 0;
  if (wgrad_wino2d_ok(g))
    return (size_t)plan_wgrad_wino2d(g).splits * g->K * 16 * g->C * sizeof(float);
  if (wgrad_wino_ok(g))
    return (size_t)plan_wgrad_wino(g).splits * g->K * 12 * g->C * sizeof(float);
  const WgradPlan pl = plan_wgrad(g->K, g->R * g->S * g->C, (long)g->N * g->P * g->Q);
  return pl.splits > 1 ? (size_t)pl.splits * g->K * g->R * g->S * g->C * sizeof(float) : 0;
}

extern "C" int nnl_conv2d_wgrad(const float* x, const float* dy, float* dw, const nnl_conv_geom_t* g, void* workspace,
                                size_t workspace_bytes, void* stream) {
  int st = check_geom(g, "conv2d_wgrad");
  if (st) return st;
  NNL_CHECK_ARG(x && dy && dw, "conv2d_wgrad: null pointer");
  NNL_CHECK_ARG(g->K % 4 == 0, "conv2d_wgrad: K=%d must be a multiple of 4", g->K);
  hipStream_t s = (hipStream_t)stream;
  IgemmKmajorParams p{};
  p.a = dy; p.b = x;
  p.N = g->N; p.H = g->H; p.W = g->W; p.C = g->C; p.P = g->P; p.Q = g->Q;
  p.R = g->R; p.S = g->S; p.stride = g->stride; p.pad = g->pad;
  p.Mc = g->K; p.Nc = g->R * g->S * g->C; p.Kp = (long)g->N * g->P * g->Q;
  const size_t need = nnl_conv2d_wgrad_workspace_bytes(g);
  if (need > 0 && (workspace == nullptr || workspace_bytes < need))
    return nnl_set_error(NNL_ERR_WORKSPACE, "conv2d_wgrad: workspace %zu B < required %zu B", workspace_bytes, need);
  NnlProfScope prof(NNL_PROF_CONV_WGRAD, s, 2.0 * p.Kp * (double)p.Mc * p.Nc);
  if (wgrad_wino2d_ok(g)) {
    const WgradPlan wp = plan_wgrad_wino2d(g);
    nnl_prof_exec_frac(1.0 / 2.25);
    int st2 = launch_wgrad_wino2d(dy, x, (float*)workspace, g, wp, s);
    if (st2) return st2;
    const long n_items = (long)g->K * (g->C / 4);
    NNL_ROUTE("wgrad_wino2d_finish");
    hipLaunchKernelGGL(wino2d_wgrad_finish_kernel, dim3((unsigned)nnl_cdiv(n_items, 16L)), dim3(256), 0, s, (const float*)workspace, dw, n_items,
                       g->C / 4, wp.splits, (long)g->K * 16 * (g->C / 4));
    NNL_CHECK_LAUNCH();
    return NNL_OK;
  }
  if (wgrad_wino_ok(g)) {
    const WgradPlan wp = plan_wgrad_wino(g);
    nnl_prof_exec_frac(1.0 / 1.5);
    int st2 = launch_wgrad_wino(dy, x, (float*)workspace, g, wp, s);
    if (st2) return st2;
    const long n4 = (long)g->K * 3 * (g->C / 4);
    NNL_ROUTE("wgrad_wino1d_finish");
    hipLaunchKernelGGL(wino_wgrad_finish_kernel, dim3((unsigned)nnl_cdiv(n4, 32L)), dim3(256), 0, s, (const float*)workspace, dw, n4,
                       g->C / 4, wp.splits, (long)g->K * 12 * (g->C / 4));
    NNL_CHECK_LAUNCH();
    return NNL_OK;
  }
  return launch_wgrad_direct(p, plan_wgrad(p.Mc, p.Nc, p.Kp), (float*)workspace, dw, s);
}

extern "C" size_t nnl_colsum_workspace_bytes(int64_t rows, int64_t cols) {
  if (rows <= 0 || cols <= 0) return 0;
  return (size_t)colsum_chunks(rows) * cols * sizeof(float);
}

extern "C" int nnl_act_gate_colsum(const float* dy, const float* y, float* g, float* colsum, int64_t rows, int64_t cols, int act,
                                   void* workspace, size_t workspace_bytes, void* stream) {
  NNL_CHECK_ARG(dy && y && g && rows > 0 && cols > 0 && cols < (1L << 30), "act_gate_colsum: bad argument");
  NNL_CHECK_ARG(act == 1 || act == 2, "act_gate_colsum: act must be 1 (ReLU) or 2 (sigmoid)");
  if (colsum != nullptr && (workspace == nullptr || workspace_bytes < nnl_colsum_workspace_bytes(rows, cols)))
    return nnl_set_error(NNL_ERR_WORKSPACE, "act_gate_colsum: workspace too small");
  hipStream_t s = (hipStream_t)stream;
  NnlProfScope prof(NNL_PROF_ELEMENTWISE, s, 12.0 * rows * cols);
  const int nchunk = colsum_chunks(rows);
  const long rpc = nnl_cdiv(nnl_cdiv(rows, nchunk), 4) * 4;
  const dim3 grid((unsigned)nnl_cdiv(cols, 64), nchunk);
  float* part = colsum ? (float*)workspace : nullptr;
  if (act == 1)
    hipLaunchKernelGGL(act_gate_colsum_kernel<1>, grid, dim3(256), 0, s, dy, y, g, part, (long)rows, (int)cols, rpc);
  else
    hipLaunchKernelGGL(act_gate_colsum_kernel<2>, grid, dim3(256), 0, s, dy, y, g, part, (long)rows, (int)cols, rpc);
  NNL_CHECK_LAUNCH();
  if (colsum != nullptr) {
    hipLaunchKernelGGL(colsum_final_kernel, dim3((unsigned)nnl_cdiv(cols, 16)), dim3(256), 0, s, (const float*)workspace, colsum,
                       (int)cols, nchunk);
    NNL_CHECK_LAUNCH();
  }
  return NNL_OK;
}

// ... 60 lines not shown
```

neuralnetworklibrary_amd/csrc/wino.h:

```cpp
#pragma once
#include "nnl_common.h"

struct WinoProblem {
  const float* in; const float* filt; float* out; const float* bias; const float* add;
  int N, H, W, Cin, Nc, relu, flip;
  float* bn_part; const float* bn_pivot;
  const float* u_pre;
};

bool nnl_wino_ok(int N, int H, int W, int Cin, int Nc, int R, int S, int stride, int pad);
double nnl_wino_plan_time_us(int N, int H, int W, int Cin, int Nc);
size_t nnl_wino_workspace_bytes(int N, int H, int W, int Cin, int Nc);
int nnl_wino_bn_rows(int N, int H, int W);
int nnl_wino_launch(const WinoProblem& q, void* ws, size_t ws_bytes, int* tile_counters, long n_counters, hipStream_t s);

bool nnl_wino2_ok(int N, int H, int W, int Cin, int Nc, int R, int S, int stride, int pad);
double nnl_wino2_plan_time_us(int N, int H, int W, int Cin, int Nc);
bool nnl_wino2_plan_is_pos(int N, int H, int W, int Cin, int Nc);
size_t nnl_wino2_workspace_bytes(int N, int H, int W, int Cin, int Nc);
int nnl_wino2_bn_rows(int N, int H, int W);
int nnl_wino2_launch(const WinoProblem& q, void* ws, size_t ws_bytes, int* tile_counters, long n_counters, hipStream_t s);
```

neuralnetworklibrary_amd/csrc/wino2.hip:

```cpp
#include "wino.h"
#include "wino_filter.h"
#include "igemm_taps.h"
#include <algorithm>

namespace {

constexpr int kCUs = 256;

template <int POL>
__device__ __forceinline__ f32x4 buf_load4_spol(__amdgpu_buffer_rsrc_t rsrc, unsigned voff, unsigned soff) {
  const i32x4 v = __builtin_bit_cast(i32x4, __builtin_amdgcn_raw_buffer_load_b128(rsrc, (int)voff, (int)soff, POL));
  return __builtin_bit_cast(f32x4, v);
}

struct Wino2Params {
  const float* a;
  const float* b;
  float* y;
  const float* bias;
  const float* add;
  unsigned a_bytes, b_bytes;
  int H, W, C, H2, W2;
  int ch;
  int prio;
  int M4;
  unsigned mg_W2, mg_H2;
  int Nc;
  int relu;
  int grid_m, grid_n;
  int bal, main_ks, n_main_tiles, tail_slices, tail_row0;
  float* main_out; long main_slab_stride;
  float* tail_out; long tail_slab_stride;
  int* tile_counters;
  float* bn_part; const float* bn_pivot;
  int pos_cs;
};

__global__ void wino2_filter_kernel(const float* __restrict__ w, float* __restrict__ u, long KC, int C, int flip) {
  const long i = (long)blockIdx.x * blockDim.x + threadIdx.x;
  if (i >= KC) return;
  const long c = i % C, k = i / C;
  wino2_filter_item(w + k * 9 * C + c, u + k * 16 * C + c, C, flip);
}

template <int BK, int OCC, bool POS = false>
__global__ __launch_bounds__(256, OCC) void wino2_kernel(const Wino2Params p) {
  constexpr int BM = 64, BN = 64, BKP = BK + 4, KC = BK / 4, RPP = 256 / KC, PA = BM / RPP, PB = BN / RPP;
  __shared__ __attribute__((aligned(16))) float lds[2][(BM + BN) * BKP];
  const int tid = threadIdx.x, lane = tid & 63, wave = tid >> 6, wm = wave >> 1, wn = wave & 1;
  int logical, kslice = 0, nslices = 1, row0 = 0;
  bool in_tail = false;
  if (p.bal) {
    const int nmb = p.n_main_tiles * p.main_ks;
    if ((int)blockIdx.x < nmb) {
      const int u = nnl_xcd_remap(blockIdx.x, nmb);
      logical = u / p.main_ks;
      kslice = u - logical * p.main_ks;
      nslices = p.main_ks;
    } else {
      const int tb = (int)blockIdx.x - nmb;
      const int t = tb / p.tail_slices;
      kslice = tb - t * p.tail_slices;
      logical = p.n_main_tiles + t;
      nslices = p.tail_slices;
      if (nslices > 1) { row0 = p.tail_row0; in_tail = true; }
    }
  } else {
    logical = nnl_xcd_remap(blockIdx.x, gridDim.x);
  }
  const bool partial = nslices > 1;
  const int tile_m = logical / p.grid_n, tile_n = logical - tile_m * p.grid_n;
  const int m0 = tile_m * BM, n0 = tile_n * BN;
  const int kc = tid % KC, lrow = tid / KC;
  auto qdiv = [](int n, unsigned mg) { return mg ? (int)__umulhi((unsigned)n, mg) : n; };
  const __amdgpu_buffer_rsrc_t ra_src = __builtin_amdgcn_make_buffer_rsrc(const_cast<float*>(p.a), 0, (int)p.a_bytes, 0x00020000);
  const __amdgpu_buffer_rsrc_t rb_src = __builtin_amdgcn_make_buffer_rsrc(const_cast<float*>(p.b), 0, (int)p.b_bytes, 0x00020000);

  int a_off[PA];
  unsigned rmask[PA], cmask[PA];
#pragma unroll
  for (int i = 0; i < PA; ++i) {
    const int m = m0 + lrow + i * RPP;
    const bool valid = m < p.M4;
    const int mm = valid ? m : 0;
    const int l2 = qdiv(mm, p.mg_W2), j = mm - l2 * p.W2;
    const int n = qdiv(l2, p.mg_H2), ii = l2 - n * p.H2;
    a_off[i] = (((n * p.H + 2 * ii - 1) * p.W + 2 * j - 1) * p.C + kc * 4) * 4;
    unsigned rm = 0, cm = 0;
    if (valid) {
      for (int a = 0; a < 4; ++a) if ((unsigned)(2 * ii - 1 + a) < (unsigned)p.H) rm |= 1u << a;
      for (int a = 0; a < 4; ++a) if ((unsigned)(2 * j - 1 + a) < (unsigned)p.W) cm |= 1u << a;
    }
    rmask[i] = rm; cmask[i] = cm;
  }
  unsigned b_off[PB];
#pragma unroll
  for (int i = 0; i < PB; ++i) {
    const int nr = n0 + lrow + i * RPP;
    b_off[i] = nr < p.Nc ? (unsigned)(nr * 16 * p.C + kc * 4) * 4u : 0xFFFFFFFFu;
  }
  unsigned v00[PA], v01[PA], v10[PA], v11[PA], b_tap = 0;
  float sr = 1.f, sc = 1.f;
  auto set_pos = [&](int t) {
    const int xi = t >> 2, nu = t & 3;
    const int ra_ = xi, rb_ = xi < 2 ? 2 : 1;
    const int ca = nu, cb = nu < 2 ? 2 : 1;
    sr = xi == 1 ? 1.f : -1.f;
    sc = nu == 1 ? 1.f : -1.f;
    b_tap = (unsigned)(t * p.C) * 4u;
    const int wc = p.W * p.C * 4, c4 = p.C * 4;
#pragma unroll
    for (int i = 0; i < PA; ++i) {
      const bool ra_ok = (rmask[i] >> ra_) & 1u, rb_ok = (rmask[i] >> rb_) & 1u;
      const bool ca_ok = (cmask[i] >> ca) & 1u, cb_ok = (cmask[i] >> cb) & 1u;
      v00[i] = (ra_ok && ca_ok) ? (unsigned)(a_off[i] + ra_ * wc + ca * c4) : 0xFFFFFFFFu;
      v01[i] = (ra_ok && cb_ok) ? (unsigned)(a_off[i] + ra_ * wc + cb * c4) : 0xFFFFFFFFu;
      v10[i] = (rb_ok && ca_ok) ? (unsigned)(a_off[i] + rb_ * wc + ca * c4) : 0xFFFFFFFFu;
      v11[i] = (rb_ok && cb_ok) ? (unsigned)(a_off[i] + rb_ * wc + cb * c4) : 0xFFFFFFFFu;
    }
  };
  f32x4 r00[PA], r01[PA], r10[PA], r11[PA], rb[PB];
  auto load_tile = [&](int c0) {
#pragma unroll
    for (int i = 0; i < PA; ++i) {
      r00[i] = buf_load4(ra_src, v00[i], (unsigned)c0 * 4u); r01[i] = buf_load4(ra_src, v01[i], (unsigned)c0 * 4u);
      r10[i] = buf_load4(ra_src, v10[i], (unsigned)c0 * 4u); r11[i] = buf_load4(ra_src, v11[i], (unsigned)c0 * 4u);
    }
#pragma unroll
// ... 68 lines not shown
  const int kend = kt0 + nk;
  int chunk_nx = kt0 / per_chunk, t_nx = (kt0 - chunk_nx * per_chunk) / cpc, cs_nx = kt0 - chunk_nx * per_chunk - t_nx * cpc;
  int c_nx = chunk_nx * p.ch + cs_nx * BK;
  int t_cur = t_nx, cs_cur = cs_nx;
  auto advance = [&]() {
    if (++cs_nx == cpc) {
      cs_nx = 0;
      if (++t_nx == 16) { t_nx = 0; ++chunk_nx; }
      set_pos(t_nx);
    }
    c_nx = chunk_nx * p.ch + cs_nx * BK;
  };
  if (nk > 0) {
    set_pos(t_nx);
    load_tile(c_nx);
    sr_ld = sr; sc_ld = sc;
    store_tile(0);
  }
  __syncthreads();
  int cur = 0;
  for (int kt = kt0; kt < kend; ++kt) {
    if (kt + 1 < kend) advance();
    load_tile(c_nx);
    const float sr_n = sr, sc_n = sc;
    __builtin_amdgcn_sched_barrier(0);
    if (p.prio) __builtin_amdgcn_s_setprio(2);
    compute(cur, tm);
    if (p.prio) __builtin_amdgcn_s_setprio(0);
    __builtin_amdgcn_sched_barrier(0);
    sr_ld = sr_n; sc_ld = sc_n;
    store_tile(cur ^ 1);
    __syncthreads();
    cur ^= 1;
    if (++cs_cur == cpc || kt + 1 == kend) {
      const int xi = t_cur >> 2, nu = t_cur & 3;
      const float cp0 = xi < 3 ? 1.f : 0.f, cp1 = xi == 0 ? 0.f : (xi == 2 ? -1.f : 1.f);
      const float cq0 = nu < 3 ? 1.f : 0.f, cq1 = nu == 0 ? 0.f : (nu == 2 ? -1.f : 1.f);
      const float k00 = cp0 * cq0, k01 = cp0 * cq1, k10 = cp1 * cq0, k11 = cp1 * cq1;
      if (k00 != 0.f) {
#pragma unroll
        for (int e = 0; e < 16; ++e) y00[e] = __builtin_fmaf(k00, tm[e], y00[e]);
      }
      if (k01 != 0.f) {
#pragma unroll
        for (int e = 0; e < 16; ++e) y01[e] = __builtin_fmaf(k01, tm[e], y01[e]);
      }
      if (k10 != 0.f) {
#pragma unroll
        for (int e = 0; e < 16; ++e) y10[e] = __builtin_fmaf(k10, tm[e], y10[e]);
      }
      if (k11 != 0.f) {
#pragma unroll
        for (int e = 0; e < 16; ++e) y11[e] = __builtin_fmaf(k11, tm[e], y11[e]);
      }
#pragma unroll
      for (int e = 0; e < 16; ++e) tm[e] = 0.f;
      cs_cur = 0; t_cur = (t_cur + 1) & 15;
    }
  }

  const int col_l = lane & 31, row_h = (lane >> 5) * 4;
  constexpr int kSc1 = 1 << 4;
  if constexpr (POS) {
    __shared__ int ticket;
    const long sstride = p.main_slab_stride;
    const __amdgpu_buffer_rsrc_t rs = __builtin_amdgcn_make_buffer_rsrc(p.main_out, 0, (int)((long)nslices * sstride * 4), 0x00020000);
    const int cl = n0 + wn * 32 + col_l;
#pragma unroll
    for (int e = 0; e < 16; ++e) {
      const int row = m0 + wm * 32 + (e & 3) + 8 * (e >> 2) + row_h;
      const long off = (long)kslice * sstride + (long)row * p.Nc + cl;
      const bool ok = row < p.M4 && cl < p.Nc;
      __builtin_amdgcn_raw_buffer_store_b32(__float_as_uint(tm[e]), rs, ok ? (int)(off * 4) : -1, 0, kSc1);
    }
    asm volatile("s_waitcnt vmcnt(0)" ::: "memory");
    __syncthreads();
    if (tid == 0) ticket = __hip_atomic_fetch_add(&p.tile_counters[logical], 1, __ATOMIC_RELAXED, __HIP_MEMORY_SCOPE_AGENT);
    __syncthreads();
    if (ticket != nslices - 1) return;
    if (tid == 0) __hip_atomic_store(&p.tile_counters[logical], 0, __ATOMIC_RELAXED, __HIP_MEMORY_SCOPE_AGENT);
    float fs1[4] = {0.f, 0.f, 0.f, 0.f}, fs2[4] = {0.f, 0.f, 0.f, 0.f};
    const int c4 = n0 + (tid & 15) * 4, cs = p.pos_cs;
    const int wrow = p.W * p.Nc;
    auto item_off = [&](int k4, bool& ok) {
      const int row = m0 + (tid >> 4) + 16 * k4;
      ok = row < p.M4 && c4 < p.Nc;
      return ok ? (unsigned)(((long)row * p.Nc + c4) * 4) : 0xFFFFFFFFu;
    };
    auto finish_item = [&](int k4, f32x4 (&m)[16]) {
      const int row = m0 + (tid >> 4) + 16 * k4;
      f32x4 r0[4], r1[4];
#pragma unroll
      for (int xi = 0; xi < 4; ++xi) {
        r0[xi] = (m[xi * 4 + 0] + m[xi * 4 + 1]) + m[xi * 4 + 2];
        r1[xi] = (m[xi * 4 + 1] - m[xi * 4 + 2]) + m[xi * 4 + 3];
      }
      f32x4 out[4];
      out[0] = (r0[0] + r0[1]) + r0[2];
      out[1] = (r1[0] + r1[1]) + r1[2];
      out[2] = (r0[1] - r0[2]) + r0[3];
      out[3] = (r1[1] - r1[2]) + r1[3];
      const int l2 = qdiv(row, p.mg_W2), j = row - l2 * p.W2;
      const int n = qdiv(l2, p.mg_H2), ii = l2 - n * p.H2;
      const long ob = (((long)n * p.H + 2 * ii) * p.W + 2 * j) * p.Nc + c4;
      const bool h1 = 2 * ii + 1 < p.H, w1 = 2 * j + 1 < p.W;
#pragma unroll
      for (int h = 0; h < 4; ++h) {
        if (((h >> 1) && !h1) || ((h & 1) && !w1)) continue;
        f32x4 v = out[h];
        const long o = ob + (h >> 1) * wrow + (h & 1) * p.Nc;
        if (p.bias) v += *reinterpret_cast<const f32x4*>(p.bias + c4);
        if (p.add) v += *reinterpret_cast<const f32x4*>(p.add + o);
        if (p.relu == 1) { v[0] = fmaxf(v[0], 0.f); v[1] = fmaxf(v[1], 0.f); v[2] = fmaxf(v[2], 0.f); v[3] = fmaxf(v[3], 0.f); }
        *reinterpret_cast<f32x4*>(p.y + o) = v;
        if (p.bn_part) {
          const f32x4 pv = *reinterpret_cast<const f32x4*>(p.bn_pivot + c4);
#pragma unroll
          for (int e = 0; e < 4; ++e) { const float d = v[e] - pv[e]; fs1[e] += d; fs2[e] += d * d; }
        }
      }
    };
#pragma unroll 1
    for (int k4 = 0; k4 < 4; ++k4) {
      bool ok_a;
      const unsigned oa = item_off(k4, ok_a);
      if (!ok_a) continue;
      f32x4 ma[16];
#pragma unroll
      for (int t = 0; t < 16; ++t) ma[t] = buf_load4_spol<kSc1>(rs, oa, (unsigned)((long)(t * cs) * sstride * 4));
      for (int sl = 1; sl < cs; ++sl) {
#pragma unroll
        for (int t0 = 0; t0 < 16; t0 += 8) {
          f32x4 pa[8];
#pragma unroll
          for (int t = 0; t < 8; ++t) pa[t] = buf_load4_spol<kSc1>(rs, oa, (unsigned)((long)((t0 + t) * cs + sl) * sstride * 4));
#pragma unroll
          for (int t = 0; t < 8; ++t) ma[t0 + t] += pa[t];
        }
      }
      finish_item(k4, ma);
    }
    if (p.bn_part) {
      __syncthreads();
      float* red = &lds[0][0];
#pragma unroll
      for (int e = 0; e < 4; ++e) {
        red[(((tid >> 4) * 64) + (tid & 15) * 4 + e) * 2 + 0] = fs1[e];
        red[(((tid >> 4) * 64) + (tid & 15) * 4 + e) * 2 + 1] = fs2[e];
      }
      __syncthreads();
      if (tid < 64 && n0 + tid < p.Nc) {
        float a = 0.f, b = 0.f;
        for (int r = 0; r < 16; ++r) { a += red[(r * 64 + tid) * 2]; b += red[(r * 64 + tid) * 2 + 1]; }
        p.bn_part[((long)tile_m * p.Nc + n0 + tid) * 2 + 0] = a;
        p.bn_part[((long)tile_m * p.Nc + n0 + tid) * 2 + 1] = b;
      }
    }
    return;
  }
  if (partial) {
    __shared__ int ticket;
    float* const base = in_tail ? p.tail_out : p.main_out;
    const long sstride = in_tail ? p.tail_slab_stride : p.main_slab_stride;
    const __amdgpu_buffer_rsrc_t rs = __builtin_amdgcn_make_buffer_rsrc(base, 0, (int)((long)nslices * sstride * 4), 0x00020000);
    const int cl = n0 + wn * 32 + col_l;
#pragma unroll
    for (int e = 0; e < 16; ++e) {
      const int row = m0 + wm * 32 + (e & 3) + 8 * (e >> 2) + row_h;
      const long off = (long)kslice * sstride + (long)(row - row0) * 4 * p.Nc + cl;
      const bool ok = row < p.M4 && cl < p.Nc;
      __builtin_amdgcn_raw_buffer_store_b32(__float_as_uint(y00[e]), rs, ok ? (int)(off * 4) : -1, 0, kSc1);
      __builtin_amdgcn_raw_buffer_store_b32(__float_as_uint(y01[e]), rs, ok ? (int)((off + p.Nc) * 4) : -1, 0, kSc1);
      __builtin_amdgcn_raw_buffer_store_b32(__float_as_uint(y10[e]), rs, ok ? (int)((off + 2 * p.Nc) * 4) : -1, 0, kSc1);
      __builtin_amdgcn_raw_buffer_store_b32(__float_as_uint(y11[e]), rs, ok ? (int)((off + 3 * p.Nc) * 4) : -1, 0, kSc1);
    }
    asm volatile("s_waitcnt vmcnt(0)" ::: "memory");
    __syncthreads();
    if (tid == 0) ticket = __hip_atomic_fetch_add(&p.tile_counters[logical], 1, __ATOMIC_RELAXED, __HIP_MEMORY_SCOPE_AGENT);
    __syncthreads();
    if (ticket != nslices - 1) return;
    if (tid == 0) __hip_atomic_store(&p.tile_counters[logical], 0, __ATOMIC_RELAXED, __HIP_MEMORY_SCOPE_AGENT);
    float fs1[4] = {0.f, 0.f, 0.f, 0.f}, fs2[4] = {0.f, 0.f, 0.f, 0.f};
    const int h = (tid >> 4) & 3, c4 = n0 + (tid & 15) * 4;
    for (int k16 = 0; k16 < 16; ++k16) {
      const int row = m0 + (tid >> 6) + 4 * k16;
      if (row >= p.M4 || c4 >= p.Nc) continue;
      const int l2 = qdiv(row, p.mg_W2), j = row - l2 * p.W2;
      const int n = qdiv(l2, p.mg_H2), ii = l2 - n * p.H2;
      const int oh = 2 * ii + (h >> 1), ow = 2 * j + (h & 1);
      if (oh >= p.H || ow >= p.W) continue;
      f32x4 v = {0.f, 0.f, 0.f, 0.f};
      for (int sl0 = 0; sl0 < nslices; sl0 += 8) {
        f32x4 part[8];
#pragma unroll
        for (int sl = 0; sl < 8; ++sl)
          if (sl0 + sl < nslices) part[sl] = buf_load4_pol(rs, (unsigned)(((long)(sl0 + sl) * sstride + ((long)(row - row0) * 4 + h) * p.Nc + c4) * 4), kSc1);
#pragma unroll
        for (int sl = 0; sl < 8; ++sl)
          if (sl0 + sl < nslices) v += part[sl];
      }
      const long o = (((long)n * p.H + oh) * p.W + ow) * p.Nc + c4;
      if (p.bias) v += *reinterpret_cast<const f32x4*>(p.bias + c4);
      if (p.add) v += *reinterpret_cast<const f32x4*>(p.add + o);
      if (p.relu == 1) { v[0] = fmaxf(v[0], 0.f); v[1] = fmaxf(v[1], 0.f); v[2] = fmaxf(v[2], 0.f); v[3] = fmaxf(v[3], 0.f); }
      *reinterpret_cast<f32x4*>(p.y + o) = v;
      if (p.bn_part) {
        const f32x4 pv = *reinterpret_cast<const f32x4*>(p.bn_pivot + c4);
#pragma unroll
        for (int e = 0; e < 4; ++e) { const float d = v[e] - pv[e]; fs1[e] += d; fs2[e] += d * d; }
      }
    }
    if (p.bn_part) {
      __syncthreads();
      float* red = &lds[0][0];
#pragma unroll
      for (int e = 0; e < 4; ++e) {
        red[(((tid >> 4) * 64) + (tid & 15) * 4 + e) * 2 + 0] = fs1[e];
        red[(((tid >> 4) * 64) + (tid & 15) * 4 + e) * 2 + 1] = fs2[e];
      }
      __syncthreads();
      if (tid < 64 && n0 + tid < p.Nc) {
        float a = 0.f, b = 0.f;
        for (int r = 0; r < 16; ++r) { a += red[(r * 64 + tid) * 2]; b += red[(r * 64 + tid) * 2 + 1]; }
        p.bn_part[((long)tile_m * p.Nc + n0 + tid) * 2 + 0] = a;
        p.bn_part[((long)tile_m * p.Nc + n0 + tid) * 2 + 1] = b;
      }
    }
    return;
  }
  constexpr int LDT = 68;
  float* tl = &lds[0][0];
  float fs1[4] = {0.f, 0.f, 0.f, 0.f}, fs2[4] = {0.f, 0.f, 0.f, 0.f};
  const int c4 = n0 + (tid & 15) * 4;
  int pb[4];
  unsigned okm[4];
#pragma unroll
  for (int k4 = 0; k4 < 4; ++k4) {
    const int row = m0 + (tid >> 4) + 16 * k4;
    const int l2 = qdiv(row, p.mg_W2), j = row - l2 * p.W2;
    const int n = qdiv(l2, p.mg_H2), ii = l2 - n * p.H2;
    pb[k4] = ((n * p.H + 2 * ii) * p.W + 2 * j) * p.Nc + c4;
    const bool ok = row < p.M4 && c4 < p.Nc, h1 = 2 * ii + 1 < p.H, w1 = 2 * j + 1 < p.W;
    okm[k4] = ok ? (1u | (w1 ? 2u : 0u) | (h1 ? 4u : 0u) | ((h1 && w1) ? 8u : 0u)) : 0u;
  }
  const int wrow = p.W * p.Nc;
#pragma unroll
  for (int h = 0; h < 4; ++h) {
    if (h) __syncthreads();
#pragma unroll
    for (int e = 0; e < 16; ++e)
      tl[(wm * 32 + (e & 3) + 8 * (e >> 2) + row_h) * LDT + wn * 32 + col_l] = h == 0 ? y00[e] : (h == 1 ? y01[e] : (h == 2 ? y10[e] : y11[e]));
    __syncthreads();
#pragma unroll
    for (int k4 = 0; k4 < 4; ++k4) {
      if (!((okm[k4] >> h) & 1u)) continue;
      f32x4 v = *reinterpret_cast<const f32x4*>(tl + ((tid >> 4) + 16 * k4) * LDT + (tid & 15) * 4);
      const int o = pb[k4] + (h >> 1) * wrow + (h & 1) * p.Nc;
      if (p.bias) v += *reinterpret_cast<const f32x4*>(p.bias + c4);
      if (p.add) v += *reinterpret_cast<const f32x4*>(p.add + o);
      if (p.relu == 1) { v[0] = fmaxf(v[0], 0.f); v[1] = fmaxf(v[1], 0.f); v[2] = fmaxf(v[2], 0.f); v[3] = fmaxf(v[3], 0.f); }
      *reinterpret_cast<f32x4*>(p.y + o) = v;
      if (p.bn_part) {
        const f32x4 pv = *reinterpret_cast<const f32x4*>(p.bn_pivot + c4);
#pragma unroll
        for (int e = 0; e < 4; ++e) { const float d = v[e] - pv[e]; fs1[e] += d; fs2[e] += d * d; }
      }
    }
  }
  if (p.bn_part) {
    __syncthreads();
    float* red = &lds[0][0];
#pragma unroll
    for (int e = 0; e < 4; ++e) {
      red[(((tid >> 4) * 64) + (tid & 15) * 4 + e) * 2 + 0] = fs1[e];
      red[(((tid >> 4) * 64) + (tid & 15) * 4 + e) * 2 + 1] = fs2[e];
    }
    __syncthreads();
    if (tid < 64 && n0 + tid < p.Nc) {
      float a = 0.f, b = 0.f;
      for (int r = 0; r < 16; ++r) { a += red[(r * 64 + tid) * 2]; b += red[(r * 64 + tid) * 2 + 1]; }
      p.bn_part[((long)tile_m * p.Nc + n0 + tid) * 2 + 0] = a;
      p.bn_part[((long)tile_m * p.Nc + n0 + tid) * 2 + 1] = b;
    }
  }
}

struct W2Plan {
  int bk, on, main_ks, n_main_tiles, tail_slices, tail_row0;
  size_t main_floats, tail_floats;
  double t_us;
  int pos_cs;
};

double w2_pos_cost(long T, long M4, int Nc, int C, int cs) {
  const double a = 0.363, b = 0.490, tfix = 4.0;
  const long occ = 4, nwg = T * 16 * cs, I = (C / 32) / cs;
  const long nb = nnl_cdiv(nwg, (long)kCUs);
  const double c = (double)(nb < occ ? nb : occ);
  const double slab_b = 2.0 * 16 * cs * (double)M4 * Nc * 4;
  return nb * I * (b + a / c) + tfix * nb / c + slab_b / 11.7e6 + (3.0 + 1.5 * cs) + 4.0;
}

double w2_cost(long T, long gn, long M4, int Nc, long I, int bk, int ks, int S, W2Plan* out) {
  const double a = bk == 32 ? 0.363 : 0.226, b = bk == 32 ? 0.490 : 0.243, tfix = bk == 32 ? 12.3 : 15.0;
  const long occ = bk == 16 ? 4 : 3;
  long n_main = ((T * ks / kCUs) * kCUs / ks / gn) * gn;
  if (n_main > T) n_main = T;
  const long tail = T - n_main;
  if (tail == 0 && S > 1) return -1.0;
  const long m = nnl_cdiv(n_main * ks, (long)kCUs), q = nnl_cdiv(tail * S, (long)kCUs);
  const long W = m * nnl_cdiv(I, (long)ks) + q * nnl_cdiv(I, (long)S), nb = m + q;
  const double c = (double)(nb < occ ? nb : occ);
  const long row0 = (n_main / gn) * 64 < M4 ? (n_main / gn) * 64 : M4;
  const double main_b = ks > 1 ? (2.0 * ks + 1) * row0 * 4 * Nc * 4 : 0;
  const double tail_b = (S > 1 && tail) ? (2.0 * S + 1) * (M4 - row0) * 4 * Nc * 4 : 0;
  if (out) {
    out->bk = bk; out->on = (ks > 1 || (S > 1 && tail)) ? 1 : 0;
    out->main_ks = ks; out->n_main_tiles = (int)n_main; out->tail_slices = tail ? S : 1; out->tail_row0 = (int)row0;
    out->main_floats = ks > 1 ? (size_t)ks * row0 * 4 * Nc : 0;
    out->tail_floats = (S > 1 && tail) ? (size_t)S * (M4 - row0) * 4 * Nc : 0;
  }
  return W * (b + a / c) + tfix * nb / c + (main_b + tail_b) / 11.7e6 + 10.0;
}

W2Plan wino2_plan(long M4, int Nc, int C) {
  W2Plan best{};
  const long gm = nnl_cdiv(M4, 64), gn = nnl_cdiv(Nc, 64), T = gm * gn;
  const int f_ks = NNL_ENV_INT("NNL_WINO_PLAN_KS", 0), f_S = NNL_ENV_INT("NNL_WINO_PLAN_S", 0);
  const bool balance = NNL_ENV_INT("NNL_WINO_BALANCE", 1) != 0;
  double best_t = 1e300;
  static const int kSlices[] = {1, 2, 3, 4, 6, 8, 12, 16};
  for (int bk = 16; bk <= 32; bk *= 2) {
    if (C % bk != 0) continue;
    const long I = 16L * (C / bk);
    for (int ks = 1; ks <= 4; ks *= 2) {
      if (ks > 1 && (!balance || I / ks < 8)) break;
      if (f_ks > 0 && ks != f_ks && balance) continue;
      for (int S : kSlices) {
        if (S > 1 && (!balance || I / S < 4)) break;
        W2Plan cand{};
        const double t = w2_cost(T, gn, M4, Nc, I, bk, ks, S, &cand);
        if (t < 0) break;
        if (f_S > 0 && balance && cand.n_main_tiles < T && S != f_S) continue;
        if (t < best_t) { best_t = t; best = cand; best.t_us = t; }
      }
    }
  }
  if (best_t == 1e300) {
    best.t_us = w2_cost(T, gn, M4, Nc, 16L * (C / 16), 16, 1, 1, &best);
    best_t = best.t_us;
  }
  const int e_pos = NNL_ENV_INT("NNL_WINO2_POS", -1);
  if (e_pos != 0 && (balance || e_pos > 0) && C % 32 == 0) {
    const int csteps = C / 32;
    double pt = 1e300; int pcs = 0;
    for (int cs = 1; cs <= 8; cs *= 2) {
      if (csteps % cs != 0 || (csteps / cs < 2 && cs > 1)) break;
      if (e_pos > 0 && cs != e_pos && csteps % e_pos == 0) continue;
      const size_t fl = (size_t)16 * cs * M4 * Nc;
      if (fl * sizeof(float) >= (1UL << 31)) break;
      const double t = w2_pos_cost(T, M4, Nc, C, cs);
      if (t < pt) { pt = t; pcs = cs; }
    }
    if (pcs && (e_pos > 0 || pt < best_t)) {
      best = W2Plan{};
      best.bk = 32; best.on = 1; best.main_ks = 16 * pcs; best.n_main_tiles = (int)T; best.tail_slices = 1; best.tail_row0 = (int)M4;
      best.main_floats = (size_t)16 * pcs * M4 * Nc; best.tail_floats = 0; best.t_us = pt; best.pos_cs = pcs;
    }
  }
  return best;
}

size_t align4(size_t floats) { return (floats + 3) & ~(size_t)3; }

long quads(int N, int H, int W) { return (long)N * ((H + 1) / 2) * ((W + 1) / 2); }

}

bool nnl_wino2_ok(int N, int H, int W, int Cin, int Nc, int R, int S, int stride, int pad) {
  if (R != 3 || S != 3 || stride != 1 || pad != 1 || W < 2 || H < 2 || Cin % 16 != 0 || Nc % 4 != 0) return false;
  const long a_b = (long)N * H * W * Cin * 4, b_b = (long)Nc * 16 * Cin * 4, y_b = (long)N * H * W * Nc * 4;
  if ((quads(N, H, W) + 128) * (long)std::max((W + 1) / 2, (H + 1) / 2) >= (1L << 32)) return false;
  return a_b < (1L << 31) && b_b < (1L << 31) && y_b < (1L << 31);
}

double nnl_wino2_plan_time_us(int N, int H, int W, int Cin, int Nc) { return wino2_plan(quads(N, H, W), Nc, Cin).t_us; }
bool nnl_wino2_plan_is_pos(int N, int H, int W, int Cin, int Nc) { return wino2_plan(quads(N, H, W), Nc, Cin).pos_cs > 0; }

size_t nnl_wino2_workspace_bytes(int N, int H, int W, int Cin, int Nc) {
  const W2Plan pl = wino2_plan(quads(N, H, W), Nc, Cin);
  return (align4((size_t)Nc * 16 * Cin) + (pl.on ? pl.main_floats + pl.tail_floats : 0)) * sizeof(float);
}

int nnl_wino2_bn_rows(int N, int H, int W) { return (int)nnl_cdiv(quads(N, H, W), 64L); }

int nnl_wino2_launch(const WinoProblem& q, void* ws, size_t ws_bytes, int* tile_counters, long n_counters, hipStream_t s) {
  const long M4 = quads(q.N, q.H, q.W);
  const size_t u_floats = align4((size_t)q.Nc * 16 * q.Cin);
  if (ws == nullptr || ws_bytes < u_floats * sizeof(float)) return nnl_set_error(NNL_ERR_WORKSPACE, "wino2: workspace too small");
  float* u = (float*)ws;
  if (q.u_pre == nullptr) {
    const long KC = (long)q.Nc * q.Cin;
    NNL_ROUTE("wino2d_filter%s", q.flip ? ":flip" : "");
    hipLaunchKernelGGL(wino2_filter_kernel, dim3((unsigned)nnl_cdiv(KC, 256L)), dim3(256), 0, s, q.filt, u, KC, q.Cin, q.flip);
    NNL_CHECK_LAUNCH();
  }
  Wino2Params p{};
  p.a = q.in; p.b = q.u_pre ? q.u_pre : u; p.y = q.out; p.bias = q.bias; p.add = q.add;
  p.a_bytes = (unsigned)((long)q.N * q.H * q.W * q.Cin * 4); p.b_bytes = (unsigned)((long)q.Nc * 16 * q.Cin * 4);
  {
    const int e_ch = NNL_ENV_INT("NNL_WINO2_CHUNK", 0);
    p.ch = (e_ch > 0 && e_ch % 32 == 0 && q.Cin % e_ch == 0) ? e_ch : q.Cin;
    p.prio = 0;
  }
  p.H = q.H; p.W = q.W; p.C = q.Cin; p.H2 = (q.H + 1) / 2; p.W2 = (q.W + 1) / 2; p.M4 = (int)M4; p.Nc = q.Nc; p.relu = q.relu;
  {
    auto magic = [](int d) { return d <= 1 ? 0u : (unsigned)(((1ULL << 32) + d - 1) / (unsigned)d); };
    p.mg_W2 = magic(p.W2); p.mg_H2 = magic(p.H2);
  }
  p.grid_m = (int)nnl_cdiv(M4, 64L); p.grid_n = (int)nnl_cdiv(q.Nc, 64);
  p.bn_part = q.bn_part; p.bn_pivot = q.bn_pivot;
  const long T = (long)p.grid_m * p.grid_n;
  W2Plan pl = wino2_plan(M4, q.Nc, q.Cin);
  if (pl.on && (tile_counters == nullptr || T > n_counters || ws_bytes < (u_floats + pl.main_floats + pl.tail_floats) * sizeof(float) ||
                pl.main_floats * sizeof(float) >= (1UL << 31) || pl.tail_floats * sizeof(float) >= (1UL << 31))) {
    if (pl.pos_cs) {
      const int bk = q.Cin % 32 == 0 ? 32 : 16;
      w2_cost(T, p.grid_n, M4, q.Nc, 16L * (q.Cin / bk), bk, 1, 1, &pl);
      pl.pos_cs = 0;
    }
    pl.on = 0;
  }
  unsigned grid = (unsigned)T;
  if (pl.pos_cs) {
    p.bal = 1; p.main_ks = pl.main_ks; p.n_main_tiles = pl.n_main_tiles; p.tail_slices = 1; p.tail_row0 = (int)M4;
    p.main_out = u + u_floats; p.main_slab_stride = M4 * q.Nc; p.tile_counters = tile_counters; p.pos_cs = pl.pos_cs;
    grid = (unsigned)(T * pl.main_ks);
    NNL_ROUTE("wino2d<32,4,pos>:%s@slices=%d,pos_cs=%d", q.u_pre ? "u_pre" : "own_u", pl.main_ks, pl.pos_cs);
    hipLaunchKernelGGL((wino2_kernel<32, 4, true>), dim3(grid), dim3(256), 0, s, p);
    NNL_CHECK_LAUNCH();
    return NNL_OK;
  }
  if (pl.on) {
    p.bal = 1; p.main_ks = pl.main_ks; p.n_main_tiles = pl.n_main_tiles; p.tail_slices = pl.tail_slices; p.tail_row0 = pl.tail_row0;
    p.main_out = u + u_floats; p.main_slab_stride = (long)pl.tail_row0 * 4 * q.Nc;
    p.tail_out = p.main_out + pl.main_floats; p.tail_slab_stride = (long)(M4 - pl.tail_row0) * 4 * q.Nc;
    p.tile_counters = tile_counters;
    grid = (unsigned)(pl.n_main_tiles * pl.main_ks + (T - pl.n_main_tiles) * pl.tail_slices);
  }
  NNL_ROUTE("wino2d<%s>:%s:%s@main_ks=%d,tail_slices=%d", pl.bk == 32 ? "32,3" : "16,4", pl.on ? "ksliced" : "plain", q.u_pre ? "u_pre" : "own_u",
            pl.on ? pl.main_ks : 1, pl.on ? pl.tail_slices : 1);
  if (pl.bk == 32) hipLaunchKernelGGL((wino2_kernel<32, 3>), dim3(grid), dim3(256), 0, s, p);
  else hipLaunchKernelGGL((wino2_kernel<16, 4>), dim3(grid), dim3(256), 0, s, p);
  NNL_CHECK_LAUNCH();
  return NNL_OK;
}

extern "C" size_t nnl_debug_conv_wino2_workspace_bytes(int N, int H, int W, int C, int K) { return nnl_wino2_workspace_bytes(N, H, W, C, K); }
extern "C" int nnl_debug_conv_wino2_fwd(const float* x, const float* w, const float* bias, const float* add, float* y, void* ws,
                                        size_t ws_bytes, int32_t* counters, long n_counters, float* bn_part, const float* bn_pivot, int N,
                                        int H, int W, int C, int K, int relu, int flip, void* stream) {
  NNL_CHECK_ARG(nnl_wino2_ok(N, H, W, C, K, 3, 3, 1, 1), "wino2: unsupported shape");
  WinoProblem q{};
  q.in = x; q.filt = w; q.out = y; q.bias = bias; q.add = add; q.N = N; q.H = H; q.W = W; q.Cin = C; q.Nc = K; q.relu = relu; q.flip = flip;
  q.bn_part = bn_part; q.bn_pivot = bn_pivot;
  return nnl_wino2_launch(q, ws, ws_bytes, counters, n_counters, (hipStream_t)stream);
}
```

neuralnetworklibrary_amd/ops.py:

```python
import collections
import ctypes
import os
import weakref

import numpy as np
import torch

from . import _lib
from ._lib import check, lib, ptr, require_cuda, stream

__all__ = ['mse_loss', 'scaled_sigmoid', 'embdotbias', 'index_error_flag', 'raise_if_index_error', 'conv2d', 'to_nhwc', 'from_nhwc', 'linear', 'bn_act', 'concat_pool2d', 'TabularPlan', 'tab_embed_concat', 'embedding_renorm_drop', 'retina_loss']

_ERR_FLAGS = {}


def _flags(device):
    key = (device.type, device.index)
    if key not in _ERR_FLAGS:
        _ERR_FLAGS[key] = torch.zeros(2, dtype=torch.int32, device=device)
    return _ERR_FLAGS[key]


def index_error_flag(device):
    return _flags(device)[0:1]
# ... 279 lines not shown
    if len(ws) < 2 or sum(w.requires_grad for w in ws) * 2 < len(ws):
        return
    key = tuple((w.data_ptr(), tuple(w.shape)) for w in ws)
    batch = getattr(model, '_nnl_wt_batch', None)
    if batch is None or batch.key != key:
        if torch.cuda.is_current_stream_capturing():
            return
        batch = _WtBatch(ws)
        object.__setattr__(model, '_nnl_wt_batch', batch)
    batch.run()
    _WT_ACTIVE.clear()
    _WT_ACTIVE.update(batch.views)
    _WINO_U_BWD.clear()
    if os.environ.get('NNL_WINO_PREPARE', '1') != '0':
        items = [(w.data_ptr(), batch.views[w.data_ptr()], 1, mode) for w in ws if w.shape[2] == 3 and w.shape[3] == 3
                 for mode in sorted(_wino_modes(w.data_ptr(), 1))]
        _run_wino_batch(model, '_nnl_wino_bwd_batch', items, _WINO_U_BWD)


def finish_backward():
    _WT_ACTIVE.clear()
    _WT_PADDED.clear()
    _WINO_U_FWD.clear()
    _WINO_U_BWD.clear()
    _WINO_IN_STEP[0] = False


def _wino_pref(key_ptr, which, g):
    pref = int(lib.nnl_conv2d_wino_preferred(g, which)) if (g.R == 3 and g.S == 3 and g.stride == 1) else 0
    if (pref or key_ptr in _WINO_PREF) and (which == 1 or _WINO_IN_STEP[0]):
        if len(_WINO_PREF) > 8192:
            _WINO_PREF.clear()
        e = _WINO_PREF.setdefault(key_ptr, [[-1, set()], [-1, set()]])[which]
        if e[0] != _WINO_GEN[0]:
            e[0], e[1] = _WINO_GEN[0], set()
        if pref:
            e[1].add(pref)
    return pref


_PADDED_GRADS = {}


def register_padded_grad(base, ld):
    if len(_PADDED_GRADS) > 64:
        for k in [k for k, (r, _) in _PADDED_GRADS.items() if r() is None]:
            del _PADDED_GRADS[k]
    _PADDED_GRADS[id(base)] = (weakref.ref(base), int(ld))


def _padded_rows(dy, K):
    base = dy._base if dy._is_view() else None
    ent = _PADDED_GRADS.get(id(base)) if base is not None else None
    if ent is None or ent[0]() is not base or dy.dim() != 4 or dy.shape[2] != 1 or dy.shape[3] != 1:
        return None
    ld = ent[1]
    if dy.dtype != torch.float32 or dy.stride(1) != 1 or dy.stride(0) != ld or ld < K or ld % 16 != 0 or dy.storage_offset() % ld != 0:
        return None
    if dy.storage_offset() + dy.shape[0] * ld > base.numel():
        return None
    return torch.as_strided(base, (dy.shape[0], 1, 1, ld), (ld, ld, ld, 1), dy.storage_offset())


_TILE_COUNTERS = {}


def _tile_counters(device):
    t = _TILE_COUNTERS.get(device.index)
    if t is None:
        if torch.cuda.is_current_stream_capturing():
            return None
        t = _TILE_COUNTERS[device.index] = torch.zeros(int(lib.nnl_conv2d_tile_counters()), dtype=torch.int32, device=device)
    return t


class GradSlot:
    __slots__ = ('tensor', 'closed')

    def __init__(self):
        self.tensor = None
        self.closed = False



_FAN = {}


class _FanOut(torch.autograd.Function):
    @staticmethod
    def forward(ctx, p, n):
        ctx.n = n
        return tuple(p.detach().view(p.shape) for _ in range(n))

    @staticmethod
    def backward(ctx, *grads):
        have = [g for g in grads if g is not None]
        if not have:
            return None, None
        if len(have) == 1:
            return have[0], None
        g0 = have[0]
        dense = all(g.is_cuda and g.dtype == torch.float32 and g.shape == g0.shape and g.stride() == g0.stride() and g.data_ptr() % 16 == 0
                    and (g.is_contiguous() or (g.dim() == 4 and g.is_contiguous(memory_format=torch.channels_last))) for g in have)
        if not dense or len(have) > 8:
            out = have[0]
            for g in have[1:]:
                out = out + g
            return out, None
        out = torch.empty_like(g0)
        arr = (ctypes.c_void_p * len(have))(*[g.data_ptr() for g in have])
        check(lib.nnl_sum_tensors(arr, len(have), ptr(out), g0.numel(), stream()))
        return out, None


class shared_params:

    def __init__(self, modules, n):
        self.modules, self.n, self.keys = modules, int(n), []

    def __enter__(self):
        if self.n > 1 and torch.is_grad_enabled():
            for m in self.modules:
                for p in m.parameters():
                    if p.requires_grad and p.is_cuda and id(p) not in _FAN:
                        _FAN[id(p)] = list(_FanOut.apply(p, self.n))
                        self.keys.append(id(p))
        return self

    def __exit__(self, *exc):
        for k in self.keys:
            _FAN.pop(k, None)
        return False


def fan_param(p):
    if p is None or not _FAN:
        return p
    lst = _FAN.get(id(p))
    return lst.pop(0) if lst else p


_ConvState = collections.namedtuple('_ConvState', 'g relu has_bias c_in w_layout slot give_slot grad_dst uses')


def _conv_operands(x, weight, bias, stride, pad):
    xn = _pad_c4(to_nhwc(_f32c(x) if x.dim() != 4 else x.float()))
    wn = _pad_c4(to_nhwc(weight.float()))
    N, H, W, C = xn.shape
    K, R, S, _ = wn.shape
    g = _geom(N, H, W, C, K, R, S, stride, pad)
    y = torch.empty((N, g.P, g.Q, K), dtype=torch.float32, device=x.device)
    return xn, wn, (None if bias is None else _f32c(bias)), g, y


def _conv_state(x, weight, bias, g, relu, slot=None, give_slot=None):
    uses = getattr(weight, '_nnl_uses', None)
    if uses is not None:
        uses[0] += 1
    return _ConvState(g, relu, bias is not None, x.shape[1], (tuple(weight.shape), tuple(weight.stride())), slot, give_slot,
                      getattr(weight, '_nnl_grad_dst', None), uses)


def _with_k(g, K):
    return _geom(g.N, g.H, g.W, g.C, K, g.R, g.S, g.stride, g.pad)


def _conv_backward(st, xn, wn, y, dy, needs):
    if dy is None:
        return None, None, None
    g, K = st.g, st.g.K
    want_db = st.has_bias and needs[2]
    db = None
    pre = _padded_rows(dy, K) if (not st.relu and g.R == 1 and g.S == 1 and g.H == 1 and g.W == 1) else None
    if pre is not None and pre.shape[-1] != K:
        dy4 = pre
    else:
        dy4 = to_nhwc(dy.float())
        if st.relu:
            dy4, db = _conv_act_gate(y, dy4, g, st.relu, want_db)
        if K % 4 != 0:
            dy4 = _pad_c4(dy4)
    w4, g4 = wn, g
    if dy4.shape[-1] != K:
        w4, g4 = torch.nn.functional.pad(wn, (0, 0, 0, 0, 0, 0, 0, dy4.shape[-1] - K)), _with_k(g, dy4.shape[-1])
    dx = dw = None
    if needs[0]:
        dx = _conv_dgrad(st, dy4, w4, g4, K)
    elif st.slot is not None:
        st.slot.tensor, st.slot.closed = None, True
    if needs[1]:
        dw = _conv_wgrad(st, xn, dy4, g4, K)
    if db is None and want_db:
        db = _conv_bias_grad(dy4, g4, K)
    return dx, dw, db


def _conv_act_gate(y, dyn, g, relu, want_db):
    rows = g.N * g.P * g.Q
    gated = torch.empty_like(dyn)
    cb = int(lib.nnl_colsum_workspace_bytes(rows, g.K)) if want_db else 0
    cws = _workspace(cb, dyn.device, floor=True) if want_db else None
    db = torch.empty(g.K, dtype=torch.float32, device=dyn.device) if want_db else None
    check(lib.nnl_act_gate_colsum(ptr(dyn), ptr(y), ptr(gated), ptr(db), rows, g.K, int(relu), ptr(cws), cb, stream()))
    return gated, db


def _conv_dgrad_operands(dy4, w4, g4, K):
    ktail = g4.R == 1 and g4.S == 1 and g4.K % 4 == 0 and os.environ.get('NNL_IGEMM_KTAIL', '1') != '0'
    dyd, gd, padk, wkey = dy4, g4, 0, None
    if g4.K % 16 != 0 and g4.K >= 32 and not ktail:
        padk = 16 - g4.K % 16
        dyd, gd = torch.nn.functional.pad(dy4, (0, padk)), _with_k(g4, g4.K + padk)
        wkey = (w4.data_ptr(), tuple(w4.shape), padk)
        wt = _WT_PADDED.get(wkey) if _WT_ACTIVE else None
    else:
        wt = _WT_ACTIVE.get(w4.data_ptr()) if g4.K == K else None
        if wt is not None and tuple(wt.shape) != (g4.C, g4.R, g4.S, g4.K):
            wt = None
    if wt is None:
        wd = torch.nn.functional.pad(w4, (0, 0, 0, 0, 0, 0, 0, padk)) if padk else w4
        wt = torch.empty((gd.C, gd.R, gd.S, gd.K), dtype=torch.float32, device=dy4.device)
        check(lib.nnl_conv2d_weight_transpose(ptr(wd), ptr(wt), gd.K, gd.R, gd.S, gd.C, stream()))
        if wkey is not None and _WT_ACTIVE:
            _WT_PADDED[wkey] = wt
    return dyd, wt, gd


def _conv_dgrad(st, dy4, w4, g4, K):
    dyd, wt, g = _conv_dgrad_operands(dy4, w4, g4, K)
    dxn = torch.empty((g.N, g.H, g.W, g.C), dtype=torch.float32, device=dyd.device)
    wsb = int(lib.nnl_conv2d_dgrad_workspace_bytes(g))
    dws = _workspace(wsb, dyd.device)
    shortcut = None
    if st.slot is not None:
        shortcut, st.slot.tensor, st.slot.closed = st.slot.tensor, None, True
    fuse = shortcut is not None and g.K % 16 == 0 and g.R * g.S <= 49 and shortcut.numel() == dxn.numel() \
        and ((g.stride == 1 and (g.S <= 32 or g.pad <= 127)) or (g.stride == 2 and g.R == 3 and g.S == 3 and g.pad == 1))
    wmode = _wino_pref(w4.data_ptr() if g.K == K else 0, 1, g)
    u = _WINO_U_BWD.get((w4.data_ptr(), wmode)) if (wmode and g.K == K) else None
    if u is not None and u.numel() != _wino_u_numel(g.C, g.K, wmode):
        u = None
    check(lib.nnl_conv2d_dgrad_pre(ptr(dyd), ptr(wt), ptr(dxn), g, ptr(shortcut) if fuse else None, ptr(dws), wsb,
                                   ptr(_tile_counters(dyd.device) if wsb else None), ptr(u), stream()))
    if shortcut is not None and not fuse:
        dxn += shortcut.view_as(dxn)
    give = st.give_slot
    if give is not None and not give.closed and st.c_in == g.C:
        give.tensor = dxn
        return None
    return from_nhwc(dxn[..., :st.c_in] if st.c_in != g.C else dxn)


def _conv_wgrad(st, xn, dy4, g4, K):
    dst = st.grad_dst
    if dst is not None and st.uses is not None and st.uses[0] == 1 and dst.dim() == 4 and g4.K == K and st.c_in == g4.C \
            and dst.permute(0, 2, 3, 1).is_contiguous() and tuple(dst.shape) == (g4.K, g4.C, g4.R, g4.S):
        dwn = dst.permute(0, 2, 3, 1)
    else:
        dwn = torch.empty((g4.K, g4.R, g4.S, g4.C), dtype=torch.float32, device=dy4.device)
    wsb = int(lib.nnl_conv2d_wgrad_workspace_bytes(g4))
    ws = _workspace(wsb, dy4.device, floor=True)
    check(lib.nnl_conv2d_wgrad(ptr(xn), ptr(dy4), ptr(dwn), g4, ptr(ws), wsb, stream()))
    dw = from_nhwc(dwn[:K, :, :, :st.c_in])
    wshape, wstride = st.w_layout
    if (g4.R == 1 and g4.S == 1 and wshape == tuple(dw.shape) and wstride != tuple(dw.stride()) and dw.is_contiguous(memory_format=torch.channels_last)
            and wstride[1] == 1 and wstride[0] == dw.shape[1]):
        dw = dw.as_strided(wshape, wstride)
    return dw


def _conv_bias_grad(dy4, g4, K):
    rows = g4.N * g4.P * g4.Q
    db_full = torch.empty(g4.K, dtype=torch.float32, device=dy4.device)
    cb = int(lib.nnl_colsum_workspace_bytes(rows, g4.K))
    cws = _workspace(cb, dy4.device, floor=True)
    check(lib.nnl_colsum(ptr(dy4), ptr(db_full), rows, g4.K, ptr(cws), cb, stream()))
    return db_full[:K]


class _Conv2d(torch.autograd.Function):

    @staticmethod
    def forward(ctx, x, weight, bias, stride, pad, relu, slot=None, bn_pivot=None, give_slot=None):
        require_cuda(x, weight, bias)
        xn, wn, b, g, y = _conv_operands(x, weight, bias, stride, pad)
        N, K, C = g.N, g.K, g.C
        ctx.st = _conv_state(x, weight, bias, g, relu, slot, give_slot)
        wsb = int(lib.nnl_conv2d_fwd_workspace_bytes(g))
        ws = _workspace(wsb, x.device)
        part, rows = None, _lib.i32(0)
        if bn_pivot is not None:
            part = torch.empty(((N * g.P * g.Q + 63) // 64) * K * 2, dtype=torch.float32, device=x.device)
        wmode = _wino_pref(wn.data_ptr(), 0, g)
        u = _WINO_U_FWD.get((wn.data_ptr(), wmode)) if wmode else None
        if u is not None and u.numel() != _wino_u_numel(K, C, wmode):
            u = None
        check(lib.nnl_conv2d_fwd_pre(ptr(xn), ptr(wn), ptr(b), ptr(y), g, int(relu), ptr(ws), wsb, ptr(_tile_counters(x.device) if wsb else None),
                                     ptr(part), ptr(bn_pivot), ctypes.byref(rows) if part is not None else None, ptr(u), stream()))
        if part is None or rows.value == 0:
            part = torch.empty(0, dtype=torch.float32, device=x.device)
        else:
            part = part[:rows.value * K * 2]
        ctx.mark_non_differentiable(part)
        ctx.set_materialize_grads(False)
        ctx.save_for_backward(xn, wn, y if relu else None)
        return from_nhwc(y), part

    @staticmethod
    def backward(ctx, dy, _dpart=None):
        xn, wn, y = ctx.saved_tensors
        return _conv_backward(ctx.st, xn, wn, y, dy, ctx.needs_input_grad[:3]) + (None,) * 6


def _conv(x, weight, bias, *, stride=1, pad=0, relu=0, slot=None, bn_pivot=None, give_slot=None):
    return _Conv2d.apply(x, weight, bias, int(stride), int(pad), int(relu), slot, bn_pivot, give_slot)


def conv2d(x, weight, bias=None, stride=1, pad=0, relu=False, grad_slot=None, give_slot=None):
    return _conv(x, weight, bias, stride=stride, pad=pad, relu=relu, slot=grad_slot, give_slot=give_slot)[0]


class _ConvAddUp2(torch.autograd.Function):

    @staticmethod
    def forward(ctx, x, weight, bias, small, stride, pad):
        require_cuda(x, weight, bias, small)
        xn, wn, b, g, y = _conv_operands(x, weight, bias, stride, pad)
        sn = to_nhwc(small.float())
        ctx.small_shape = (g.N, g.P // 2, g.Q // 2, g.K)
        if tuple(sn.shape) != ctx.small_shape or g.P % 2 or g.Q % 2:
            raise _lib.NnlError('conv_add_upsampled: `small` %s is not [N, K, P/2, Q/2] of the %dx%d output' % (tuple(small.shape), g.P, g.Q))
        ctx.st = _conv_state(x, weight, bias, g, 0)
        check(lib.nnl_conv2d_fwd_add_up2(ptr(xn), ptr(wn), ptr(b), ptr(sn), ptr(y), g, stream()))
        ctx.save_for_backward(xn, wn)
        return from_nhwc(y)

    @staticmethod
    def backward(ctx, dy):
        dsmall = None
        if ctx.needs_input_grad[3]:
            dyn = to_nhwc(dy.float())
            N, h, w, K = ctx.small_shape
            ds = torch.empty(ctx.small_shape, dtype=torch.float32, device=dy.device)
            check(lib.nnl_upsample2_bwd(ptr(dyn), ptr(ds), N, h, w, K, stream()))
            dsmall = from_nhwc(ds)
        xn, wn = ctx.saved_tensors
        return _conv_backward(ctx.st, xn, wn, None, dy, ctx.needs_input_grad[:3]) + (dsmall, None, None)


def conv_add_upsampled(x, weight, bias, small, stride=1, pad=0):
    return _ConvAddUp2.apply(x, weight, bias, small, int(stride), int(pad))


def conv2d_with_bn_stats(x, weight, bias, stride, pad, bn_pivot, grad_slot=None, give_slot=None):
    return _conv(x, weight, bias, stride=stride, pad=pad, slot=grad_slot, bn_pivot=bn_pivot, give_slot=give_slot)


def _rows_in_place(x):
    return x.dtype == torch.float32 and x.dim() == 2 and x.stride(1) == 1 and x.stride(0) >= x.shape[1]


class _LinearSmall(torch.autograd.Function):

    @staticmethod
    def forward(ctx, x, weight, bias):
        require_cuda(x, weight, bias)
        x = x if _rows_in_place(x) else _f32c(x)
        w = _f32c(weight)
        b = None if bias is None else _f32c(bias)
        M, K = x.shape
        N = w.shape[0]
        y = torch.empty(M, N, dtype=torch.float32, device=x.device)
        check(lib.nnl_linear_small_fwd(ptr(x), ptr(w), ptr(b), ptr(y), M, K, x.stride(0) if M > 1 else K, N, stream()))
        ctx.save_for_backward(x, w)
        ctx.has_bias = bias is not None
        return y

    @staticmethod
    def backward(ctx, dy):
        x, w = ctx.saved_tensors
        M, K = x.shape
        N = w.shape[0]
        dy = _f32c(dy)
        dev = dy.device
        dx = torch.empty(M, K, dtype=torch.float32, device=dev) if ctx.needs_input_grad[0] else None
        dw = torch.empty(N, K, dtype=torch.float32, device=dev) if ctx.needs_input_grad[1] else None
        db = torch.empty(N, dtype=torch.float32, device=dev) if (ctx.has_bias and ctx.needs_input_grad[2]) else None
        wsb = int(lib.nnl_linear_small_bwd_workspace_bytes(M, K, N)) if (dw is not None or db is not None) else 0
        ws = _workspace(wsb, dev)
        check(lib.nnl_linear_small_bwd(ptr(dy), ptr(x), ptr(w), ptr(dx), ptr(dw), ptr(db), M, K, x.stride(0) if M > 1 else K, N, ptr(ws), wsb,
                                       stream()))
        return dx, dw, db


def linear(x, weight, bias=None, relu=False):
    lead = x.shape[:-1]
    x2 = x.reshape(-1, x.shape[-1])
    if not relu and weight.shape[0] <= 4 and x2.is_cuda and x2.shape[0] > 0:
        return _LinearSmall.apply(x2, weight, bias).reshape(*lead, weight.shape[0])
    y = _conv(x2[:, :, None, None], weight[:, :, None, None], bias, relu=relu)[0]
    return y.reshape(*lead, weight.shape[0])


def _rows_view(x):
    if x.dim() == 4:
        xn = to_nhwc(x.float())
        N, H, W, C = xn.shape
        return xn.view(-1, C), (lambda m: from_nhwc(m.view(N, H, W, C)))
    if x.dim() == 2:
        return _f32c(x), (lambda m: m)
    if x.dim() == 3:
        xn = x.float().permute(0, 2, 1).contiguous()
        N, L, C = xn.shape
        return xn.view(-1, C), (lambda m: m.view(N, L, C).permute(0, 2, 1))
    raise ValueError('bn_act: unsupported input rank %d' % x.dim())


def _relu_mask(rows, C, device):
    return torch.empty((rows * C + 31) // 32 + 2, dtype=torch.int32, device=device)


class _BNAct(torch.autograd.Function):
    @staticmethod
    def forward(ctx, x, residual, gamma, beta, running_mean, running_var, training, momentum, eps, relu, nbt, slot=None, ext=None,
                pivot_out=None):
        require_cuda(x, residual, gamma, beta)
        ctx.slot = slot
        xm, back = _rows_view(x)
        rows, C = xm.shape
        rm = None if residual is None else _rows_view(residual)[0]
        y = torch.empty_like(xm)
        mean = torch.empty(C, dtype=torch.float32, device=xm.device)
        invstd = torch.empty(C, dtype=torch.float32, device=xm.device)
        wsb = int(lib.nnl_bn_workspace_bytes(rows, C))
        ws = _workspace(wsb, xm.device)
        mask = _relu_mask(rows, C, xm.device) if relu else None
        check(lib.nnl_bn_fwd(ptr(xm), ptr(gamma), ptr(beta), ptr(rm), ptr(y), ptr(mean), ptr(invstd), ptr(running_mean),
                             ptr(running_var), rows, C, float(eps), float(momentum), int(training), int(relu), ptr(nbt),
                             ptr(mask), ptr(ext[0]) if ext else None, (ext[0].numel() // (2 * C)) if ext else 0,
                             ptr(ext[1]) if ext else None, ptr(pivot_out), ptr(ws), wsb, stream()))
        ctx.save_for_backward(xm, mask, gamma, mean, invstd)
        ctx.cfg = (training, relu, residual is not None, back)
        return back(y)

    @staticmethod
    def backward(ctx, dy):
        xm, mask, gamma, mean, invstd = ctx.saved_tensors
        training, relu, has_res, back = ctx.cfg
        dym = _rows_view(dy)[0]
        rows, C = xm.shape
        dx = torch.empty_like(xm)
        dres = torch.empty_like(xm) if (has_res and ctx.needs_input_grad[1]) else None
        dgamma = torch.empty(C, dtype=torch.float32, device=xm.device) if gamma is not None else None
        dbeta = torch.empty(C, dtype=torch.float32, device=xm.device) if gamma is not None else None
        wsb = int(lib.nnl_bn_workspace_bytes(rows, C))
        ws = _workspace(wsb, xm.device)
        check(lib.nnl_bn_bwd(ptr(dym), None, ptr(mask), ptr(xm), ptr(gamma), ptr(mean), ptr(invstd), ptr(dx), ptr(dres),
                             ptr(dgamma), ptr(dbeta), rows, C, int(training), int(relu), ptr(ws), wsb, stream()))
        if ctx.slot is not None and dres is not None:
            ctx.slot.tensor, dres = dres, None
        return (back(dx), None if dres is None else back(dres), dgamma, dbeta) + (None,) * 10


def _sync_group_size(group):
    import torch.distributed as dist
    return dist.get_world_size(group)


class _SyncBNAct(torch.autograd.Function):

    @staticmethod
    def forward(ctx, x, residual, gamma, beta, running_mean, running_var, momentum, eps, relu, nbt, group, comm, slot=None):
        require_cuda(x, residual, gamma, beta)
        ctx.slot = slot
        xm, back = _rows_view(x)
        rows, C = xm.shape
        rm = None if residual is None else _rows_view(residual)[0]
        dev = xm.device
        wsb = int(lib.nnl_bn_workspace_bytes(rows, C))
        ws = _workspace(wsb, dev)
        stats = torch.empty(2 * C + 2, dtype=torch.float32, device=dev)
        check(lib.nnl_bn_sync_stats(ptr(xm), ptr(stats), rows, C, ptr(ws), wsb, stream()))
        all_stats = comm.all_gather(stats, group)
        world = all_stats.shape[0]
        y = torch.empty_like(xm)
        mean = torch.empty(C, dtype=torch.float32, device=dev)
        invstd = torch.empty(C, dtype=torch.float32, device=dev)
        mask = _relu_mask(rows, C, dev) if relu else None
        check(lib.nnl_bn_sync_fwd(ptr(xm), ptr(all_stats), world, ptr(gamma), ptr(beta), ptr(rm), ptr(y), ptr(mean), ptr(invstd),
                                  ptr(running_mean), ptr(running_var), rows, C, float(eps), float(momentum), int(relu), ptr(nbt),
                                  ptr(mask), ptr(ws), wsb, stream()))
        ctx.save_for_backward(xm, mask, gamma, mean, invstd, all_stats)
        ctx.cfg = (relu, residual is not None, back, group, comm)
        return back(y)

    @staticmethod
    def backward(ctx, dy):
        xm, mask, gamma, mean, invstd, all_stats = ctx.saved_tensors
        relu, has_res, back, group, comm = ctx.cfg
        dym = _rows_view(dy)[0]
        rows, C = xm.shape
        dev = xm.device
        wsb = int(lib.nnl_bn_workspace_bytes(rows, C))
        ws = _workspace(wsb, dev)
        sums = torch.empty(2 * C, dtype=torch.float32, device=dev)
        check(lib.nnl_bn_sync_bwd_reduce(ptr(dym), None, ptr(mask), ptr(xm), ptr(mean), ptr(invstd), ptr(sums), rows, C, int(relu),
                                         ptr(ws), wsb, stream()))
        total = comm.all_reduce_sum(sums, group)
        dx = torch.empty_like(xm)
        dres = torch.empty_like(xm) if (has_res and ctx.needs_input_grad[1]) else None
        dgamma = torch.empty(C, dtype=torch.float32, device=dev) if gamma is not None else None
        dbeta = torch.empty(C, dtype=torch.float32, device=dev) if gamma is not None else None
        check(lib.nnl_bn_sync_bwd(ptr(dym), None, ptr(mask), ptr(xm), ptr(gamma), ptr(mean), ptr(invstd), ptr(sums), ptr(total),
                                  ptr(all_stats), int(all_stats.shape[0]), ptr(dx), ptr(dres), ptr(dgamma), ptr(dbeta), rows, C,
                                  int(relu), ptr(ws), wsb, stream()))
        if ctx.slot is not None and dres is not None:
            ctx.slot.tensor, dres = dres, None
        return (back(dx), None if dres is None else back(dres), dgamma, dbeta) + (None,) * 9


class DistComm:

    @staticmethod
    def all_gather(t, group):
        import torch.distributed as dist
        w = dist.get_world_size(group)
        out = torch.empty((w,) + tuple(t.shape), dtype=t.dtype, device=t.device)
        dist.all_gather(list(out.unbind(0)), t, group=group)
        return out

    @staticmethod
    def all_reduce_sum(t, group):
        import torch.distributed as dist
        out = t.clone()
        dist.all_reduce(out, op=dist.ReduceOp.SUM, group=group)
        return out


def _bn_mode(bn):
    training = bn.training or (bn.running_mean is None)
    momentum, nbt = 0.0, None
    if bn.training and bn.track_running_stats:
        nbt, momentum = bn.num_batches_tracked, bn.momentum
    stats = not training or bn.track_running_stats
    return training, momentum, nbt, (bn.running_mean if stats else None), (bn.running_var if stats else None)


def bn_act(bn, x, residual=None, relu=True, grad_slot=None, ext_stats=None, pivot_out=None):
    training, momentum, nbt, rmean, rvar = _bn_mode(bn)
    if momentum is None:
        nbt.add_(1)
        momentum, nbt = 1.0 / float(nbt.item()), None
    sync = getattr(bn, 'nnl_sync', None)
    if sync is not None and training:
        return _SyncBNAct.apply(x, residual, bn.weight, bn.bias, rmean, rvar, momentum, bn.eps, relu, nbt, sync[0], sync[1],
                                grad_slot)
    ext = ext_stats if (ext_stats is not None and training and ext_stats[0].numel() > 0) else None
    return _BNAct.apply(x, residual, bn.weight, bn.bias, rmean, rvar, training, momentum, bn.eps, relu, nbt, grad_slot, ext,
                        pivot_out if training else None)


class _ConcatPool(torch.autograd.Function):
    @staticmethod
    def forward(ctx, x):
        require_cuda(x)
        xn = to_nhwc(x.float())
        N, H, W, C = xn.shape
        out = torch.empty(N, 2 * C, dtype=torch.float32, device=x.device)
        am = torch.empty(N, C, dtype=torch.int32, device=x.device)
        check(lib.nnl_concat_pool_fwd(ptr(xn), ptr(out), ptr(am), N, H * W, C, stream()))
        ctx.save_for_backward(am)
        ctx.shape = (N, H, W, C)
        return out.view(N, 2 * C, 1, 1)

    @staticmethod
    def backward(ctx, dout):
        (am,) = ctx.saved_tensors
        N, H, W, C = ctx.shape
        dx = torch.empty(N, H, W, C, dtype=torch.float32, device=dout.device)
        check(lib.nnl_concat_pool_bwd(ptr(_f32c(dout.reshape(N, 2 * C))), ptr(am), ptr(dx), N, H * W, C, stream()))
        return from_nhwc(dx)


def conv_bn_act(conv, bn, x, residual=None, relu=True, conv_slot=None, bn_slot=None, conv_give=None):
    fuse = (bn.training and bn.track_running_stats and bn.running_mean is not None and bn.momentum is not None
            and getattr(bn, 'nnl_sync', None) is None and x.is_cuda and conv.bias is None and not conv.fuse_relu
            and torch.is_grad_enabled() and os.environ.get('NNL_BN_EPI_STATS', '1') != '0')

    def unfused(**kw):
        return bn_act(bn, conv(x, grad_slot=conv_slot, give_slot=conv_give), residual=residual, relu=relu, grad_slot=bn_slot, **kw)
    if not fuse:
        return unfused()
    pivot = getattr(bn, '_nnl_pivot', None)
    if pivot is None or pivot.device != x.device or pivot.numel() != bn.num_features:
        if torch.cuda.is_current_stream_capturing():
            return unfused()
        pivot = torch.empty(bn.num_features, dtype=torch.float32, device=x.device)
        object.__setattr__(bn, '_nnl_pivot', pivot)
        return unfused(pivot_out=pivot)
    y, part = conv2d_with_bn_stats(x, conv.weight, None, conv.stride[0], conv.padding[0], pivot, conv_slot, conv_give)
    return bn_act(bn, y, residual=residual, relu=relu, grad_slot=bn_slot, ext_stats=(part, pivot), pivot_out=pivot)


def linear_relu_bn(lin, bn, x):
    fuse = (bn.training and bn.track_running_stats and bn.running_mean is not None and bn.momentum is not None
            and getattr(bn, 'nnl_sync', None) is None and x.is_cuda and x.dim() == 2 and torch.is_grad_enabled()
            and os.environ.get('NNL_BN_EPI_STATS', '1') != '0')
    pivot = getattr(bn, '_nnl_pivot', None) if fuse else None
    if not fuse or pivot is None or pivot.device != x.device or pivot.numel() != bn.num_features:
        y = linear(x, lin.weight, lin.bias, relu=True)
        if not fuse or torch.cuda.is_current_stream_capturing():
            return bn_act(bn, y, relu=False)
        pivot = torch.empty(bn.num_features, dtype=torch.float32, device=x.device)
        object.__setattr__(bn, '_nnl_pivot', pivot)
        return bn_act(bn, y, relu=False, pivot_out=pivot)
    y, part = _conv(x[:, :, None, None], lin.weight[:, :, None, None], lin.bias, relu=1, bn_pivot=pivot)
    return bn_act(bn, y.reshape(x.shape[0], lin.weight.shape[0]), relu=False, ext_stats=(part, pivot), pivot_out=pivot)


def concat_pool2d(x):
    return _ConcatPool.apply(x)


class _MaxPool2d(torch.autograd.Function):
    @staticmethod
    def forward(ctx, x, ksize, stride, pad):
        require_cuda(x)
        xn = to_nhwc(x.float())
        N, H, W, C = xn.shape
        P, Q = (H + 2 * pad - ksize) // stride + 1, (W + 2 * pad - ksize) // stride + 1
        y = torch.empty(N, P, Q, C, dtype=torch.float32, device=x.device)
        idx = torch.empty(N, P, Q, C, dtype=torch.uint8, device=x.device)
        check(lib.nnl_maxpool2d_fwd(ptr(xn), ptr(y), ptr(idx), N, H, W, C, P, Q, ksize, stride, pad, stream()))
        ctx.save_for_backward(idx)
        ctx.cfg = (N, H, W, C, P, Q, ksize, stride, pad)
        return from_nhwc(y)

    @staticmethod
    def backward(ctx, dy):
        (idx,) = ctx.saved_tensors
        N, H, W, C, P, Q, ksize, stride, pad = ctx.cfg
        dyn = to_nhwc(dy.float())
        dx = torch.empty(N, H, W, C, dtype=torch.float32, device=dy.device)
        check(lib.nnl_maxpool2d_bwd(ptr(dyn), ptr(idx), ptr(dx), N, H, W, C, P, Q, ksize, stride, pad, stream()))
        return from_nhwc(dx), None, None, None


class _BNReLUMaxPool(torch.autograd.Function):

    @staticmethod
    def forward(ctx, x, gamma, beta, running_mean, running_var, training, momentum, eps, nbt, ksize, stride, pad):
        require_cuda(x, gamma, beta)
        xn = to_nhwc(x.float())
        N, H, W, C = xn.shape
        P, Q = (H + 2 * pad - ksize) // stride + 1, (W + 2 * pad - ksize) // stride + 1
        dev = x.device
        y = torch.empty(N, P, Q, C, dtype=torch.float32, device=dev)
        idx = torch.empty(N, P, Q, C, dtype=torch.uint8, device=dev)
        stats = torch.empty(4, C, dtype=torch.float32, device=dev)
        wsb = int(lib.nnl_bn_workspace_bytes(N * H * W, C))
        ws = _workspace(wsb, dev)
        check(lib.nnl_bn_relu_maxpool_fwd(ptr(xn), ptr(gamma), ptr(beta), ptr(y), ptr(idx), ptr(stats[0]), ptr(stats[1]),
                                          ptr(stats[2]), ptr(stats[3]), ptr(running_mean), ptr(running_var), N, H, W, C, P, Q,
                                          ksize, stride, pad, float(eps), float(momentum), int(training), ptr(nbt), ptr(ws), wsb,
                                          stream()))
        ctx.save_for_backward(xn, idx, gamma, beta, stats, y)
        ctx.cfg = (N, H, W, C, P, Q, ksize, stride, pad, training)
        return from_nhwc(y)

    @staticmethod
    def backward(ctx, dy):
        xn, idx, gamma, beta, stats, y = ctx.saved_tensors
        N, H, W, C, P, Q, ksize, stride, pad, training = ctx.cfg
        dyn = to_nhwc(dy.float())
        dx = torch.empty_like(xn)
        dgamma = torch.empty(C, dtype=torch.float32, device=xn.device) if gamma is not None else None
        dbeta = torch.empty(C, dtype=torch.float32, device=xn.device) if gamma is not None else None
        wsb = int(lib.nnl_bn_workspace_bytes(N * H * W, C))
        ws = _workspace(wsb, xn.device)
        check(lib.nnl_bn_relu_maxpool_bwd(ptr(dyn), ptr(y), ptr(idx), ptr(xn), ptr(gamma), ptr(beta), ptr(stats[0]), ptr(stats[1]),
                                          ptr(stats[2]), ptr(stats[3]), ptr(dx), ptr(dgamma), ptr(dbeta), N, H, W, C, P, Q, ksize, stride, pad,
                                          int(training), ptr(ws), wsb, stream()))
        return (from_nhwc(dx), dgamma, dbeta) + (None,) * 9

# ... 194 lines not shown
```

Before: 5546 images/s.

## Fuse BN backward reduction and ReLU gating into Winograd dgrad epilogue

```diff
diff --git a/include/nnl.h b/include/nnl.h
--- a/include/nnl.h
+++ b/include/nnl.h
@@ -78,6 +78,9 @@
                        int32_t* bn_rows, const float* u, void* stream);
 int nnl_conv2d_dgrad_pre(const float* dy, const float* wt, float* dx, const nnl_conv_geom_t* g, const float* addend,
                          void* workspace, size_t workspace_bytes, int32_t* tile_counters, const float* u, void* stream);
+int nnl_conv2d_dgrad_bn(const float* dy, const float* wt, float* dx, const nnl_conv_geom_t* g, const float* addend, void* workspace,
+                        size_t workspace_bytes, int32_t* tile_counters, const float* u, const float* bn_x, const uint32_t* bn_relu_mask,
+                        const float* bn_mean, const float* bn_invstd, float* bn_partials, int32_t* bn_rows, void* stream);
 size_t nnl_debug_conv_wino_workspace_bytes(int N, int H, int W, int C, int K);
 int nnl_debug_conv_wino_fwd(const float* x, const float* filt, const float* bias, const float* add, float* y, void* ws,
                             size_t ws_bytes, int32_t* counters, long n_counters, float* bn_part, const float* bn_pivot, int N,
@@ -111,6 +114,9 @@
 int nnl_bn_bwd(const float* dy, const float* y, const uint32_t* relu_mask, const float* x, const float* gamma,
                const float* mean, const float* invstd, float* dx, float* dres, float* dgamma, float* dbeta, int64_t rows,
                int64_t C, int training, int relu, void* workspace, size_t workspace_bytes, void* stream);
+int nnl_bn_bwd_ext(const float* g, const float* ext_partials, int64_t ext_rows, const float* x, const float* gamma, const float* mean,
+                   const float* invstd, float* dx, float* dgamma, float* dbeta, int64_t rows, int64_t C, int training, void* workspace,
+                   size_t workspace_bytes, void* stream);
 
 int nnl_bn_relu_maxpool_supported(int64_t C);
 int nnl_bn_relu_maxpool_fwd(const float* x, const float* gamma, const float* beta, float* y, uint8_t* idx, float* save_mean,
diff --git a/neuralnetworklibrary_amd/Applications/VisionModels/resnet.py b/neuralnetworklibrary_amd/Applications/VisionModels/resnet.py
--- a/neuralnetworklibrary_amd/Applications/VisionModels/resnet.py
+++ b/neuralnetworklibrary_amd/Applications/VisionModels/resnet.py
@@ -1,6 +1,6 @@
 import torch.nn as nn
 
-from .retinanet import BasicBlock, Bottleneck, HipConv2d, HipMaxPool2d, _Downsample
+from .retinanet import BasicBlock, Bottleneck, HipConv2d, HipMaxPool2d, _Downsample, _Stage
 from ... import ops
 
 __all__ = ['ResNet', 'resnet18', 'resnet34', 'resnet50', 'resnet101', 'resnet152']
@@ -37,7 +37,7 @@
         self.inplanes = planes * block.expansion
         for _ in range(1, blocks):
             layers.append(block(self.inplanes, planes))
-        return nn.Sequential(*layers)
+        return _Stage(*layers)
 
     def forward(self, x):
         x = ops.conv_bn_relu_maxpool(self.conv1, self.bn1, self.maxpool, x)
diff --git a/neuralnetworklibrary_amd/Applications/VisionModels/retinanet.py b/neuralnetworklibrary_amd/Applications/VisionModels/retinanet.py
--- a/neuralnetworklibrary_amd/Applications/VisionModels/retinanet.py
+++ b/neuralnetworklibrary_amd/Applications/VisionModels/retinanet.py
@@ -19,12 +19,12 @@
         super().__init__(*args, **kwargs)
         self.weight.data = self.weight.data.contiguous(memory_format=torch.channels_last)
 
-    def forward(self, x, grad_slot=None, give_slot=None):
+    def forward(self, x, grad_slot=None, give_slot=None, in_tap=None):
         if self.dilation != (1, 1) or self.groups != 1 or self.stride[0] != self.stride[1] \
                 or self.padding[0] != self.padding[1] or self.padding_mode != 'zeros':
             raise NotImplementedError('HipConv2d: only the symmetric, dense convolutions the reference uses')
         return ops.conv2d(x, ops.fan_param(self.weight), ops.fan_param(self.bias), self.stride[0], self.padding[0], relu=self.fuse_relu,
-                          grad_slot=grad_slot, give_slot=give_slot)
+                          grad_slot=grad_slot, give_slot=give_slot, in_tap=in_tap)
 
 
 class HipMaxPool2d(nn.MaxPool2d):
@@ -57,12 +57,16 @@
         self.downsample = downsample
         self.stride = stride
 
-    def forward(self, x):
+    def forward(self, x, in_tap=None, out_tap=None):
         slot = ops.GradSlot() if (x.requires_grad and torch.is_grad_enabled()) else None
-        out = ops.conv_bn_act(self.conv1, self.bn1, x, relu=True, conv_slot=slot)
+        if slot is None or self.downsample is not None:
+            in_tap = None
+        tap1 = ops.bn_tap(x)
+        out = ops.conv_bn_act(self.conv1, self.bn1, x, relu=True, conv_slot=slot, in_tap=in_tap, out_tap=tap1)
         if self.downsample is None:
-            return ops.conv_bn_act(self.conv2, self.bn2, out, residual=x, relu=True, bn_slot=slot)
-        return ops.conv_bn_act(self.conv2, self.bn2, out, residual=_shortcut(self.downsample, x, slot), relu=True)
+            return ops.conv_bn_act(self.conv2, self.bn2, out, residual=x, relu=True, bn_slot=slot, in_tap=tap1, out_tap=out_tap)
+        return ops.conv_bn_act(self.conv2, self.bn2, out, residual=_shortcut(self.downsample, x, slot), relu=True, in_tap=tap1,
+                               out_tap=out_tap)
 
 
 class Bottleneck(nn.Module):
@@ -80,13 +84,32 @@
         self.downsample = downsample
         self.stride = stride
 
-    def forward(self, x):
+    def forward(self, x, in_tap=None, out_tap=None):
         slot = ops.GradSlot() if (x.requires_grad and torch.is_grad_enabled()) else None
-        out = ops.conv_bn_act(self.conv1, self.bn1, x, relu=True, conv_slot=slot)
-        out = ops.conv_bn_act(self.conv2, self.bn2, out, relu=True)
+        tap1 = ops.bn_tap(x) if self.conv2.stride[0] == 1 else None
+        out = ops.conv_bn_act(self.conv1, self.bn1, x, relu=True, conv_slot=slot, out_tap=tap1)
+        out = ops.conv_bn_act(self.conv2, self.bn2, out, relu=True, in_tap=tap1)
         if self.downsample is None:
             return ops.conv_bn_act(self.conv3, self.bn3, out, residual=x, relu=True, bn_slot=slot)
         return ops.conv_bn_act(self.conv3, self.bn3, out, residual=_shortcut(self.downsample, x, slot), relu=True)
+
+
+class _Stage(nn.Sequential):
+
+    def forward(self, x):
+        mods = list(self.children())
+        tap = None
+        for i, m in enumerate(mods):
+            if not isinstance(m, (BasicBlock, Bottleneck)):
+                x, tap = m(x), None
+                continue
+            nxt = mods[i + 1] if i + 1 < len(mods) else None
+            out_tap = None
+            if isinstance(m, BasicBlock) and isinstance(nxt, BasicBlock) and nxt.downsample is None and nxt.conv1.stride[0] == 1:
+                out_tap = ops.bn_tap(x, needs_shortcut=True)
+            x = m(x, in_tap=tap, out_tap=out_tap)
+            tap = out_tap
+        return x
 
 
 class _Downsample(nn.Sequential):
@@ -236,7 +259,7 @@
         self.inplanes = planes * block.expansion
         for _ in range(1, blocks):
             layers.append(block(self.inplanes, planes))
-        return nn.Sequential(*layers)
+        return _Stage(*layers)
 
     def stem(self, x):
         return ops.conv_bn_relu_maxpool(self.conv1, self.bn1, self.maxpool, x)
diff --git a/neuralnetworklibrary_amd/_lib.py b/neuralnetworklibrary_amd/_lib.py
--- a/neuralnetworklibrary_amd/_lib.py
+++ b/neuralnetworklibrary_amd/_lib.py
@@ -46,6 +46,7 @@
     'nnl_wino_filter_multi': (C.c_int, [c_p, c_p, i64, c_p]),
     'nnl_conv2d_fwd_pre': (C.c_int, [c_p, c_p, c_p, c_p, C.POINTER(ConvGeom), C.c_int, c_p, sz, c_p, c_p, c_p, C.POINTER(i32), c_p, c_p]),
     'nnl_conv2d_dgrad_pre': (C.c_int, [c_p, c_p, c_p, C.POINTER(ConvGeom), c_p, c_p, sz, c_p, c_p, c_p]),
+    'nnl_conv2d_dgrad_bn': (C.c_int, [c_p, c_p, c_p, C.POINTER(ConvGeom), c_p, c_p, sz, c_p, c_p, c_p, c_p, c_p, c_p, c_p, C.POINTER(i32), c_p]),
     'nnl_debug_conv_wino_workspace_bytes': (sz, [C.c_int] * 5),
     'nnl_debug_conv_wino_fwd': (C.c_int, [c_p] * 6 + [sz, c_p, C.c_long, c_p, c_p] + [C.c_int] * 7 + [c_p]),
     'nnl_debug_conv_wino2_workspace_bytes': (sz, [C.c_int] * 5),
@@ -128,6 +129,7 @@
     'nnl_bn_sync_bwd': (C.c_int, [c_p, c_p, c_p, c_p, c_p, c_p, c_p, c_p, c_p, c_p, C.c_int, c_p, c_p, c_p, c_p, i64, i64,
                                   C.c_int, c_p, sz, c_p]),
     'nnl_bn_bwd': (C.c_int, [c_p, c_p, c_p, c_p, c_p, c_p, c_p, c_p, c_p, c_p, c_p, i64, i64, C.c_int, C.c_int, c_p, sz, c_p]),
+    'nnl_bn_bwd_ext': (C.c_int, [c_p, c_p, i64, c_p, c_p, c_p, c_p, c_p, c_p, c_p, i64, i64, C.c_int, c_p, sz, c_p]),
 }
 
 for _name, (_res, _args) in SIGNATURES.items():
diff --git a/neuralnetworklibrary_amd/csrc/batchnorm.hip b/neuralnetworklibrary_amd/csrc/batchnorm.hip
--- a/neuralnetworklibrary_amd/csrc/batchnorm.hip
+++ b/neuralnetworklibrary_amd/csrc/batchnorm.hip
@@ -379,15 +379,16 @@
   }
 }
 
+template <int LANES>
 __global__ void bn_bwd_finalize_kernel(const float* __restrict__ part, int nparts, const float* __restrict__ gamma,
                                        const float* __restrict__ mean, const float* __restrict__ invstd,
                                        float* __restrict__ dgamma, float* __restrict__ dbeta, float* __restrict__ coef,
                                        long rows, int C, int training) {
-  __shared__ float red[4][kFinLanes][2];
-  const int c = blockIdx.x * 4 + threadIdx.x / kFinLanes;
+  __shared__ float red[256 / LANES][LANES][2];
+  const int c = blockIdx.x * (256 / LANES) + threadIdx.x / LANES;
   float s1, s2;
-  reduce_partials(part, nparts, C, c, c < C, red, s1, s2);
-  if (c >= C || (threadIdx.x & (kFinLanes - 1)) != 0) return;
+  reduce_partials<LANES>(part, nparts, C, c, c < C, red, s1, s2);
+  if (c >= C || (threadIdx.x & (LANES - 1)) != 0) return;
   if (dbeta) dbeta[c] = s1;
   if (dgamma) dgamma[c] = s2;
   const float gm = gamma ? gamma[c] : 1.f;
@@ -569,7 +570,7 @@
     hipLaunchKernelGGL(bn_bwd_reduce_kernel<1>, dim3(sh.gx, sh.gy), dim3(kBlock), 0, s, dy, y, x, mean, invstd, part, (long)rows,
                        (int)C, sh.L, relu, relu_mask);
   NNL_CHECK_LAUNCH();
-  hipLaunchKernelGGL(bn_bwd_finalize_kernel, dim3((unsigned)nnl_cdiv(C, 4)), dim3(256), 0, s, part, sh.gx, gamma, mean, invstd,
+  hipLaunchKernelGGL(bn_bwd_finalize_kernel<kFinLanes>, dim3((unsigned)nnl_cdiv(C, 4)), dim3(256), 0, s, part, sh.gx, gamma, mean, invstd,
                      dgamma, dbeta, coef, (long)rows, (int)C, training);
   NNL_CHECK_LAUNCH();
   const long total_v = rows * CG;
@@ -579,6 +580,36 @@
   else
     hipLaunchKernelGGL(bn_bwd_apply_kernel<1>, dim3(ew_grid(total_v, CG)), dim3(kBlock), 0, s, dy, y, x, coef, dx, dres, total_v,
                        (int)CG, (int)C, relu, relu_mask);
+  NNL_CHECK_LAUNCH();
+  return NNL_OK;
+}
+
+extern "C" int nnl_bn_bwd_ext(const float* g, const float* ext_partials, int64_t ext_rows, const float* x, const float* gamma,
+                              const float* mean, const float* invstd, float* dx, float* dgamma, float* dbeta, int64_t rows, int64_t C,
+                              int training, void* workspace, size_t workspace_bytes, void* stream) {
+  NNL_CHECK_ARG(rows > 0 && C > 0 && C < (1 << 24) && ext_rows > 0 && ext_rows < (1L << 31), "bn_bwd_ext: bad sizes");
+  NNL_CHECK_ARG(g && ext_partials && x && mean && invstd && dx, "bn_bwd_ext: null pointer");
+  if (workspace == nullptr || workspace_bytes < nnl_bn_workspace_bytes(rows, C))
+    return nnl_set_error(NNL_ERR_WORKSPACE, "bn_bwd_ext: workspace too small");
+  hipStream_t s = (hipStream_t)stream;
+  float* coef = (float*)workspace + (long)kMaxRowBlocks * C * 2 + 2 * C;
+  const int VEC = (C % 4 == 0) ? 4 : 1;
+  const long CG = C / VEC;
+  NnlProfScope prof(NNL_PROF_ELEMENTWISE, s, (double)rows * C * 12.0);
+  if (ext_rows >= 1024)
+    hipLaunchKernelGGL(bn_bwd_finalize_kernel<256>, dim3((unsigned)C), dim3(256), 0, s, ext_partials, (int)ext_rows, gamma, mean, invstd,
+                       dgamma, dbeta, coef, (long)rows, (int)C, training);
+  else
+    hipLaunchKernelGGL(bn_bwd_finalize_kernel<kFinLanes>, dim3((unsigned)nnl_cdiv(C, 4)), dim3(256), 0, s, ext_partials, (int)ext_rows,
+                       gamma, mean, invstd, dgamma, dbeta, coef, (long)rows, (int)C, training);
+  NNL_CHECK_LAUNCH();
+  const long total_v = rows * CG;
+  if (VEC == 4)
+    hipLaunchKernelGGL(bn_bwd_apply_kernel<4>, dim3(ew_grid(total_v, CG)), dim3(kBlock), 0, s, g, nullptr, x, coef, dx, nullptr, total_v,
+                       (int)CG, (int)C, 0, nullptr);
+  else
+    hipLaunchKernelGGL(bn_bwd_apply_kernel<1>, dim3(ew_grid(total_v, CG)), dim3(kBlock), 0, s, g, nullptr, x, coef, dx, nullptr, total_v,
+                       (int)CG, (int)C, 0, nullptr);
   NNL_CHECK_LAUNCH();
   return NNL_OK;
 }
@@ -853,14 +884,14 @@
     hipLaunchKernelGGL(bnpool_bwd_reduce_out_kernel, dim3(go), dim3(kPoolRedBlock), 0, s, dpool, y, idx, x, gamma, beta, mean, invstd,
                        part, (int)N, (int)C, g);
     NNL_CHECK_LAUNCH();
-    hipLaunchKernelGGL(bn_bwd_finalize_kernel, dim3((unsigned)nnl_cdiv(C, 4)), dim3(256), 0, s, part, (int)go, gamma, mean, invstd,
+    hipLaunchKernelGGL(bn_bwd_finalize_kernel<kFinLanes>, dim3((unsigned)nnl_cdiv(C, 4)), dim3(256), 0, s, part, (int)go, gamma, mean, invstd,
                        dgamma, dbeta, coef, rows, (int)C, training);
     NNL_CHECK_LAUNCH();
   } else {
     hipLaunchKernelGGL(bnpool_bwd_reduce_kernel, dim3(grid), dim3(kPoolRedBlock), 0, s, dpool, idx, x, scale, shift, mean, invstd, part,
                        (int)N, (int)C, g);
     NNL_CHECK_LAUNCH();
-    hipLaunchKernelGGL(bn_bwd_finalize_kernel, dim3((unsigned)nnl_cdiv(C, 4)), dim3(256), 0, s, part, (int)grid, gamma, mean, invstd,
+    hipLaunchKernelGGL(bn_bwd_finalize_kernel<kFinLanes>, dim3((unsigned)nnl_cdiv(C, 4)), dim3(256), 0, s, part, (int)grid, gamma, mean, invstd,
                        dgamma, dbeta, coef, rows, (int)C, training);
     NNL_CHECK_LAUNCH();
   }
diff --git a/neuralnetworklibrary_amd/csrc/conv2d.hip b/neuralnetworklibrary_amd/csrc/conv2d.hip
--- a/neuralnetworklibrary_amd/csrc/conv2d.hip
+++ b/neuralnetworklibrary_amd/csrc/conv2d.hip
@@ -948,8 +948,10 @@
   return nnl_conv2d_dgrad_pre(dy, wt, dx, g, addend, workspace, workspace_bytes, tile_counters, nullptr, stream);
 }
 
-extern "C" int nnl_conv2d_dgrad_pre(const float* dy, const float* wt, float* dx, const nnl_conv_geom_t* g, const float* addend,
-                                    void* workspace, size_t workspace_bytes, int32_t* tile_counters, const float* u, void* stream) {
+struct DgradBnGate { const float* x; const uint32_t* mask; const float* mean; const float* invstd; float* partials; int32_t* rows; };
+
+static int dgrad_impl(const float* dy, const float* wt, float* dx, const nnl_conv_geom_t* g, const float* addend, void* workspace,
+                      size_t workspace_bytes, int32_t* tile_counters, const float* u, const DgradBnGate* bn, void* stream) {
   int st = check_geom(g, "conv2d_dgrad");
   if (st) return st;
   NNL_CHECK_ARG(dy && wt && dx, "conv2d_dgrad: null pointer");
@@ -975,7 +977,11 @@
     wq.in = dy; wq.filt = wt; wq.out = dx; wq.bias = nullptr; wq.add = addend;
     wq.N = g->N; wq.H = g->P; wq.W = g->Q; wq.Cin = g->K; wq.Nc = g->C; wq.relu = 0; wq.flip = 1;
     wq.u_pre = u;
-    return wino_mode_launch(wmode, wq, workspace, workspace_bytes, tile_counters, kTileCounters, s);
+    const bool gate = bn != nullptr && wmode == 2;
+    if (gate) { wq.bg_x = bn->x; wq.bg_mask = bn->mask; wq.bg_mean = bn->mean; wq.bg_invstd = bn->invstd; wq.bn_part = bn->partials; }
+    st = wino_mode_launch(wmode, wq, workspace, workspace_bytes, tile_counters, kTileCounters, s);
+    if (st == NNL_OK && gate) *bn->rows = nnl_wino2_bn_rows(g->N, g->P, g->Q);
+    return st;
   }
   const int tk = dgrad_tap_table_ok(g) ? taps_kind(a_elems, b_elems, g->K, g->R * g->S) : 0;
   if (tk && (g->stride == 1 || g->stride == 2)) {
@@ -1054,6 +1060,21 @@
   return dispatch_rowk<IGEMM_MODE_DGRAD>(p, s);
 }
 
+extern "C" int nnl_conv2d_dgrad_pre(const float* dy, const float* wt, float* dx, const nnl_conv_geom_t* g, const float* addend,
+                                    void* workspace, size_t workspace_bytes, int32_t* tile_counters, const float* u, void* stream) {
+  return dgrad_impl(dy, wt, dx, g, addend, workspace, workspace_bytes, tile_counters, u, nullptr, stream);
+}
+
+extern "C" int nnl_conv2d_dgrad_bn(const float* dy, const float* wt, float* dx, const nnl_conv_geom_t* g, const float* addend,
+                                   void* workspace, size_t workspace_bytes, int32_t* tile_counters, const float* u, const float* bn_x,
+                                   const uint32_t* bn_relu_mask, const float* bn_mean, const float* bn_invstd, float* bn_partials,
+                                   int32_t* bn_rows, void* stream) {
+  NNL_CHECK_ARG(bn_x && bn_relu_mask && bn_mean && bn_invstd && bn_partials && bn_rows, "conv2d_dgrad_bn: null pointer");
+  *bn_rows = 0;
+  const DgradBnGate bn{bn_x, bn_relu_mask, bn_mean, bn_invstd, bn_partials, bn_rows};
+  return dgrad_impl(dy, wt, dx, g, addend, workspace, workspace_bytes, tile_counters, u, &bn, stream);
+}
+
 extern "C" size_t nnl_conv2d_wgrad_workspace_bytes(const nnl_conv_geom_t* g) {
   if (!g || check_geom(g, "conv2d_wgrad_workspace_bytes")) return 0;
   if (wgrad_wino2d_ok(g))
diff --git a/neuralnetworklibrary_amd/csrc/wino.h b/neuralnetworklibrary_amd/csrc/wino.h
--- a/neuralnetworklibrary_amd/csrc/wino.h
+++ b/neuralnetworklibrary_amd/csrc/wino.h
@@ -6,6 +6,7 @@
   int N, H, W, Cin, Nc, relu, flip;
   float* bn_part; const float* bn_pivot;
   const float* u_pre;
+  const float* bg_x; const unsigned* bg_mask; const float* bg_mean; const float* bg_invstd;
 };
 
 bool nnl_wino_ok(int N, int H, int W, int Cin, int Nc, int R, int S, int stride, int pad);
diff --git a/neuralnetworklibrary_amd/csrc/wino2.hip b/neuralnetworklibrary_amd/csrc/wino2.hip
--- a/neuralnetworklibrary_amd/csrc/wino2.hip
+++ b/neuralnetworklibrary_amd/csrc/wino2.hip
@@ -34,7 +34,22 @@
   int* tile_counters;
   float* bn_part; const float* bn_pivot;
   int pos_cs;
+  const float* bg_x; const unsigned* bg_mask; const float* bg_mean; const float* bg_invstd;
 };
+
+__device__ __forceinline__ f32x4 wino2_bn_gate(const Wino2Params& p, f32x4 v, long o, const f32x4& mu, const f32x4& is, float (&s1)[4],
+                                               float (&s2)[4]) {
+  const f32x4 xv = *reinterpret_cast<const f32x4*>(p.bg_x + o);
+  const unsigned kb = p.bg_mask[o >> 5] >> (o & 31);
+#pragma unroll
+  for (int e = 0; e < 4; ++e) {
+    const float gg = ((kb >> e) & 1u) ? v[e] : 0.f;
+    s1[e] += gg;
+    s2[e] += gg * ((xv[e] - mu[e]) * is[e]);
+    v[e] = gg;
+  }
+  return v;
+}
 
 __global__ void wino2_filter_kernel(const float* __restrict__ w, float* __restrict__ u, long KC, int C, int flip) {
   const long i = (long)blockIdx.x * blockDim.x + threadIdx.x;
@@ -43,7 +58,7 @@
   wino2_filter_item(w + k * 9 * C + c, u + k * 16 * C + c, C, flip);
 }
 
-template <int BK, int OCC, bool POS = false>
+template <int BK, int OCC, bool POS = false, bool GATE = false>
 __global__ __launch_bounds__(256, OCC) void wino2_kernel(const Wino2Params p) {
   constexpr int BM = 64, BN = 64, BKP = BK + 4, KC = BK / 4, RPP = 256 / KC, PA = BM / RPP, PB = BN / RPP;
   __shared__ __attribute__((aligned(16))) float lds[2][(BM + BN) * BKP];
@@ -278,6 +293,10 @@
     float fs1[4] = {0.f, 0.f, 0.f, 0.f}, fs2[4] = {0.f, 0.f, 0.f, 0.f};
     const int c4 = n0 + (tid & 15) * 4, cs = p.pos_cs;
     const int wrow = p.W * p.Nc;
+    f32x4 g_mu = {0.f, 0.f, 0.f, 0.f}, g_is = g_mu;
+    if constexpr (GATE) {
+      if (c4 < p.Nc) { g_mu = *reinterpret_cast<const f32x4*>(p.bg_mean + c4); g_is = *reinterpret_cast<const f32x4*>(p.bg_invstd + c4); }
+    }
     auto item_off = [&](int k4, bool& ok) {
       const int row = m0 + (tid >> 4) + 16 * k4;
       ok = row < p.M4 && c4 < p.Nc;
@@ -308,8 +327,9 @@
         if (p.bias) v += *reinterpret_cast<const f32x4*>(p.bias + c4);
         if (p.add) v += *reinterpret_cast<const f32x4*>(p.add + o);
         if (p.relu == 1) { v[0] = fmaxf(v[0], 0.f); v[1] = fmaxf(v[1], 0.f); v[2] = fmaxf(v[2], 0.f); v[3] = fmaxf(v[3], 0.f); }
+        if constexpr (GATE) v = wino2_bn_gate(p, v, o, g_mu, g_is, fs1, fs2);
         *reinterpret_cast<f32x4*>(p.y + o) = v;
-        if (p.bn_part) {
+        if (!GATE && p.bn_part) {
           const f32x4 pv = *reinterpret_cast<const f32x4*>(p.bn_pivot + c4);
 #pragma unroll
           for (int e = 0; e < 4; ++e) { const float d = v[e] - pv[e]; fs1[e] += d; fs2[e] += d * d; }
@@ -378,6 +398,10 @@
     if (tid == 0) __hip_atomic_store(&p.tile_counters[logical], 0, __ATOMIC_RELAXED, __HIP_MEMORY_SCOPE_AGENT);
     float fs1[4] = {0.f, 0.f, 0.f, 0.f}, fs2[4] = {0.f, 0.f, 0.f, 0.f};
     const int h = (tid >> 4) & 3, c4 = n0 + (tid & 15) * 4;
+    f32x4 g_mu = {0.f, 0.f, 0.f, 0.f}, g_is = g_mu;
+    if constexpr (GATE) {
+      if (c4 < p.Nc) { g_mu = *reinterpret_cast<const f32x4*>(p.bg_mean + c4); g_is = *reinterpret_cast<const f32x4*>(p.bg_invstd + c4); }
+    }
     for (int k16 = 0; k16 < 16; ++k16) {
       const int row = m0 + (tid >> 6) + 4 * k16;
       if (row >= p.M4 || c4 >= p.Nc) continue;
@@ -399,8 +423,9 @@
       if (p.bias) v += *reinterpret_cast<const f32x4*>(p.bias + c4);
       if (p.add) v += *reinterpret_cast<const f32x4*>(p.add + o);
       if (p.relu == 1) { v[0] = fmaxf(v[0], 0.f); v[1] = fmaxf(v[1], 0.f); v[2] = fmaxf(v[2], 0.f); v[3] = fmaxf(v[3], 0.f); }
+      if constexpr (GATE) v = wino2_bn_gate(p, v, o, g_mu, g_is, fs1, fs2);
       *reinterpret_cast<f32x4*>(p.y + o) = v;
-      if (p.bn_part) {
+      if (!GATE && p.bn_part) {
         const f32x4 pv = *reinterpret_cast<const f32x4*>(p.bn_pivot + c4);
 #pragma unroll
         for (int e = 0; e < 4; ++e) { const float d = v[e] - pv[e]; fs1[e] += d; fs2[e] += d * d; }
@@ -428,6 +453,10 @@
   float* tl = &lds[0][0];
   float fs1[4] = {0.f, 0.f, 0.f, 0.f}, fs2[4] = {0.f, 0.f, 0.f, 0.f};
   const int c4 = n0 + (tid & 15) * 4;
+  f32x4 g_mu = {0.f, 0.f, 0.f, 0.f}, g_is = g_mu;
+  if constexpr (GATE) {
+    if (c4 < p.Nc) { g_mu = *reinterpret_cast<const f32x4*>(p.bg_mean + c4); g_is = *reinterpret_cast<const f32x4*>(p.bg_invstd + c4); }
+  }
   int pb[4];
   unsigned okm[4];
 #pragma unroll
@@ -455,8 +484,9 @@
       if (p.bias) v += *reinterpret_cast<const f32x4*>(p.bias + c4);
       if (p.add) v += *reinterpret_cast<const f32x4*>(p.add + o);
       if (p.relu == 1) { v[0] = fmaxf(v[0], 0.f); v[1] = fmaxf(v[1], 0.f); v[2] = fmaxf(v[2], 0.f); v[3] = fmaxf(v[3], 0.f); }
+      if constexpr (GATE) v = wino2_bn_gate(p, v, o, g_mu, g_is, fs1, fs2);
       *reinterpret_cast<f32x4*>(p.y + o) = v;
-      if (p.bn_part) {
+      if (!GATE && p.bn_part) {
         const f32x4 pv = *reinterpret_cast<const f32x4*>(p.bn_pivot + c4);
 #pragma unroll
         for (int e = 0; e < 4; ++e) { const float d = v[e] - pv[e]; fs1[e] += d; fs2[e] += d * d; }
@@ -616,6 +646,8 @@
   }
   p.grid_m = (int)nnl_cdiv(M4, 64L); p.grid_n = (int)nnl_cdiv(q.Nc, 64);
   p.bn_part = q.bn_part; p.bn_pivot = q.bn_pivot;
+  const bool gate = q.bg_x != nullptr;
+  p.bg_x = q.bg_x; p.bg_mask = q.bg_mask; p.bg_mean = q.bg_mean; p.bg_invstd = q.bg_invstd;
   const long T = (long)p.grid_m * p.grid_n;
   W2Plan pl = wino2_plan(M4, q.Nc, q.Cin);
   if (pl.on && (tile_counters == nullptr || T > n_counters || ws_bytes < (u_floats + pl.main_floats + pl.tail_floats) * sizeof(float) ||
@@ -633,7 +665,8 @@
     p.main_out = u + u_floats; p.main_slab_stride = M4 * q.Nc; p.tile_counters = tile_counters; p.pos_cs = pl.pos_cs;
     grid = (unsigned)(T * pl.main_ks);
     NNL_ROUTE("wino2d<32,4,pos>:%s@slices=%d,pos_cs=%d", q.u_pre ? "u_pre" : "own_u", pl.main_ks, pl.pos_cs);
-    hipLaunchKernelGGL((wino2_kernel<32, 4, true>), dim3(grid), dim3(256), 0, s, p);
+    if (gate) hipLaunchKernelGGL((wino2_kernel<32, 4, true, true>), dim3(grid), dim3(256), 0, s, p);
+    else hipLaunchKernelGGL((wino2_kernel<32, 4, true>), dim3(grid), dim3(256), 0, s, p);
     NNL_CHECK_LAUNCH();
     return NNL_OK;
   }
@@ -646,7 +679,10 @@
   }
   NNL_ROUTE("wino2d<%s>:%s:%s@main_ks=%d,tail_slices=%d", pl.bk == 32 ? "32,3" : "16,4", pl.on ? "ksliced" : "plain", q.u_pre ? "u_pre" : "own_u",
             pl.on ? pl.main_ks : 1, pl.on ? pl.tail_slices : 1);
-  if (pl.bk == 32) hipLaunchKernelGGL((wino2_kernel<32, 3>), dim3(grid), dim3(256), 0, s, p);
+  if (gate) {
+    if (pl.bk == 32) hipLaunchKernelGGL((wino2_kernel<32, 3, false, true>), dim3(grid), dim3(256), 0, s, p);
+    else hipLaunchKernelGGL((wino2_kernel<16, 4, false, true>), dim3(grid), dim3(256), 0, s, p);
+  } else if (pl.bk == 32) hipLaunchKernelGGL((wino2_kernel<32, 3>), dim3(grid), dim3(256), 0, s, p);
   else hipLaunchKernelGGL((wino2_kernel<16, 4>), dim3(grid), dim3(256), 0, s, p);
   NNL_CHECK_LAUNCH();
   return NNL_OK;
diff --git a/neuralnetworklibrary_amd/ops.py b/neuralnetworklibrary_amd/ops.py
--- a/neuralnetworklibrary_amd/ops.py
+++ b/neuralnetworklibrary_amd/ops.py
@@ -385,6 +385,21 @@
         self.closed = False
 
 
+class BNTap:
+    __slots__ = ('fwd', 'needs_shortcut', 'part', 'gated')
+
+    def __init__(self, needs_shortcut=False):
+        self.fwd = None
+        self.needs_shortcut = bool(needs_shortcut)
+        self.part = None
+        self.gated = None
+
+
+def bn_tap(x, needs_shortcut=False):
+    if os.environ.get('NNL_BN_EPI_BWD', '1') == '0' or not (x.is_cuda and torch.is_grad_enabled()):
+        return None
+    return BNTap(needs_shortcut)
+
 
 _FAN = {}
 
@@ -443,7 +458,7 @@
     return lst.pop(0) if lst else p
 
 
-_ConvState = collections.namedtuple('_ConvState', 'g relu has_bias c_in w_layout slot give_slot grad_dst uses')
+_ConvState = collections.namedtuple('_ConvState', 'g relu has_bias c_in w_layout slot give_slot grad_dst uses in_tap')
 
 
 def _conv_operands(x, weight, bias, stride, pad):
@@ -456,12 +471,12 @@
     return xn, wn, (None if bias is None else _f32c(bias)), g, y
 
 
-def _conv_state(x, weight, bias, g, relu, slot=None, give_slot=None):
+def _conv_state(x, weight, bias, g, relu, slot=None, give_slot=None, in_tap=None):
     uses = getattr(weight, '_nnl_uses', None)
     if uses is not None:
         uses[0] += 1
     return _ConvState(g, relu, bias is not None, x.shape[1], (tuple(weight.shape), tuple(weight.stride())), slot, give_slot,
-                      getattr(weight, '_nnl_grad_dst', None), uses)
+                      getattr(weight, '_nnl_grad_dst', None), uses, in_tap if (in_tap is not None and in_tap.fwd is not None) else None)
 
 
 def _with_k(g, K):
@@ -543,8 +558,23 @@
     u = _WINO_U_BWD.get((w4.data_ptr(), wmode)) if (wmode and g.K == K) else None
     if u is not None and u.numel() != _wino_u_numel(g.C, g.K, wmode):
         u = None
-    check(lib.nnl_conv2d_dgrad_pre(ptr(dyd), ptr(wt), ptr(dxn), g, ptr(shortcut) if fuse else None, ptr(dws), wsb,
-                                   ptr(_tile_counters(dyd.device) if wsb else None), ptr(u), stream()))
+    tap = st.in_tap
+    if tap is not None and not (tap.fwd is not None and g.R == 3 and g.S == 3 and g.stride == 1 and g.pad == 1 and g.K == K and dyd is dy4 and st.c_in == g.C
+                                and st.give_slot is None and wsb and (fuse if tap.needs_shortcut else shortcut is None)
+                                and tap.fwd[0].numel() == dxn.numel() and tap.fwd[0].shape[-1] == g.C):
+        tap = None
+    if tap is not None:
+        bx, bmask, bmean, binvstd = tap.fwd
+        part = torch.empty(((g.N * ((g.H + 1) // 2) * ((g.W + 1) // 2) + 63) // 64) * g.C * 2, dtype=torch.float32, device=dyd.device)
+        rows = _lib.i32(0)
+        check(lib.nnl_conv2d_dgrad_bn(ptr(dyd), ptr(wt), ptr(dxn), g, ptr(shortcut) if fuse else None, ptr(dws), wsb,
+                                      ptr(_tile_counters(dyd.device)), ptr(u), ptr(bx), ptr(bmask), ptr(bmean), ptr(binvstd), ptr(part),
+                                      ctypes.byref(rows), stream()))
+        if rows.value > 0:
+            tap.part, tap.gated = part[:rows.value * g.C * 2], dxn
+    else:
+        check(lib.nnl_conv2d_dgrad_pre(ptr(dyd), ptr(wt), ptr(dxn), g, ptr(shortcut) if fuse else None, ptr(dws), wsb,
+                                       ptr(_tile_counters(dyd.device) if wsb else None), ptr(u), stream()))
     if shortcut is not None and not fuse:
         dxn += shortcut.view_as(dxn)
     give = st.give_slot
@@ -584,11 +614,11 @@
 class _Conv2d(torch.autograd.Function):
 
     @staticmethod
-    def forward(ctx, x, weight, bias, stride, pad, relu, slot=None, bn_pivot=None, give_slot=None):
+    def forward(ctx, x, weight, bias, stride, pad, relu, slot=None, bn_pivot=None, give_slot=None, in_tap=None):
         require_cuda(x, weight, bias)
         xn, wn, b, g, y = _conv_operands(x, weight, bias, stride, pad)
         N, K, C = g.N, g.K, g.C
-        ctx.st = _conv_state(x, weight, bias, g, relu, slot, give_slot)
+        ctx.st = _conv_state(x, weight, bias, g, relu, slot, give_slot, in_tap)
         wsb = int(lib.nnl_conv2d_fwd_workspace_bytes(g))
         ws = _workspace(wsb, x.device)
         part, rows = None, _lib.i32(0)
@@ -612,15 +642,15 @@
     @staticmethod
     def backward(ctx, dy, _dpart=None):
         xn, wn, y = ctx.saved_tensors
-        return _conv_backward(ctx.st, xn, wn, y, dy, ctx.needs_input_grad[:3]) + (None,) * 6
-
-
-def _conv(x, weight, bias, *, stride=1, pad=0, relu=0, slot=None, bn_pivot=None, give_slot=None):
-    return _Conv2d.apply(x, weight, bias, int(stride), int(pad), int(relu), slot, bn_pivot, give_slot)
-
-
-def conv2d(x, weight, bias=None, stride=1, pad=0, relu=False, grad_slot=None, give_slot=None):
-    return _conv(x, weight, bias, stride=stride, pad=pad, relu=relu, slot=grad_slot, give_slot=give_slot)[0]
+        return _conv_backward(ctx.st, xn, wn, y, dy, ctx.needs_input_grad[:3]) + (None,) * 7
+
+
+def _conv(x, weight, bias, *, stride=1, pad=0, relu=0, slot=None, bn_pivot=None, give_slot=None, in_tap=None):
+    return _Conv2d.apply(x, weight, bias, int(stride), int(pad), int(relu), slot, bn_pivot, give_slot, in_tap)
+
+
+def conv2d(x, weight, bias=None, stride=1, pad=0, relu=False, grad_slot=None, give_slot=None, in_tap=None):
+    return _conv(x, weight, bias, stride=stride, pad=pad, relu=relu, slot=grad_slot, give_slot=give_slot, in_tap=in_tap)[0]
 
 
 class _ConvAddUp2(torch.autograd.Function):
@@ -655,8 +685,8 @@
     return _ConvAddUp2.apply(x, weight, bias, small, int(stride), int(pad))
 
 
-def conv2d_with_bn_stats(x, weight, bias, stride, pad, bn_pivot, grad_slot=None, give_slot=None):
-    return _conv(x, weight, bias, stride=stride, pad=pad, slot=grad_slot, bn_pivot=bn_pivot, give_slot=give_slot)
+def conv2d_with_bn_stats(x, weight, bias, stride, pad, bn_pivot, grad_slot=None, give_slot=None, in_tap=None):
+    return _conv(x, weight, bias, stride=stride, pad=pad, slot=grad_slot, bn_pivot=bn_pivot, give_slot=give_slot, in_tap=in_tap)
 
 
 def _rows_in_place(x):
@@ -726,9 +756,10 @@
 class _BNAct(torch.autograd.Function):
     @staticmethod
     def forward(ctx, x, residual, gamma, beta, running_mean, running_var, training, momentum, eps, relu, nbt, slot=None, ext=None,
-                pivot_out=None):
+                pivot_out=None, out_tap=None):
         require_cuda(x, residual, gamma, beta)
         ctx.slot = slot
+        ctx.out_tap = out_tap if relu else None
         xm, back = _rows_view(x)
         rows, C = xm.shape
         rm = None if residual is None else _rows_view(residual)[0]
@@ -744,6 +775,8 @@
                              ptr(ext[1]) if ext else None, ptr(pivot_out), ptr(ws), wsb, stream()))
         ctx.save_for_backward(xm, mask, gamma, mean, invstd)
         ctx.cfg = (training, relu, residual is not None, back)
+        if ctx.out_tap is not None:
+            ctx.out_tap.fwd = (xm, mask, mean, invstd)
         return back(y)
 
     @staticmethod
@@ -753,16 +786,26 @@
         dym = _rows_view(dy)[0]
         rows, C = xm.shape
         dx = torch.empty_like(xm)
-        dres = torch.empty_like(xm) if (has_res and ctx.needs_input_grad[1]) else None
         dgamma = torch.empty(C, dtype=torch.float32, device=xm.device) if gamma is not None else None
         dbeta = torch.empty(C, dtype=torch.float32, device=xm.device) if gamma is not None else None
         wsb = int(lib.nnl_bn_workspace_bytes(rows, C))
         ws = _workspace(wsb, xm.device)
-        check(lib.nnl_bn_bwd(ptr(dym), None, ptr(mask), ptr(xm), ptr(gamma), ptr(mean), ptr(invstd), ptr(dx), ptr(dres),
-                             ptr(dgamma), ptr(dbeta), rows, C, int(training), int(relu), ptr(ws), wsb, stream()))
+        tap, part = ctx.out_tap, None
+        if tap is not None:
+            if tap.part is not None and tap.gated is not None and tap.gated.data_ptr() == dym.data_ptr() and tap.gated.numel() == dym.numel():
+                part = tap.part
+            tap.part = tap.gated = None
+        if part is not None:
+            check(lib.nnl_bn_bwd_ext(ptr(dym), ptr(part), part.numel() // (2 * C), ptr(xm), ptr(gamma), ptr(mean), ptr(invstd), ptr(dx),
+                                     ptr(dgamma), ptr(dbeta), rows, C, int(training), ptr(ws), wsb, stream()))
+            dres = dym if (has_res and ctx.needs_input_grad[1]) else None
+        else:
+            dres = torch.empty_like(xm) if (has_res and ctx.needs_input_grad[1]) else None
+            check(lib.nnl_bn_bwd(ptr(dym), None, ptr(mask), ptr(xm), ptr(gamma), ptr(mean), ptr(invstd), ptr(dx), ptr(dres),
+                                 ptr(dgamma), ptr(dbeta), rows, C, int(training), int(relu), ptr(ws), wsb, stream()))
         if ctx.slot is not None and dres is not None:
             ctx.slot.tensor, dres = dres, None
-        return (back(dx), None if dres is None else back(dres), dgamma, dbeta) + (None,) * 10
+        return (back(dx), None if dres is None else back(dres), dgamma, dbeta) + (None,) * 11
 
 
 def _sync_group_size(group):
@@ -849,7 +892,7 @@
     return training, momentum, nbt, (bn.running_mean if stats else None), (bn.running_var if stats else None)
 
 
-def bn_act(bn, x, residual=None, relu=True, grad_slot=None, ext_stats=None, pivot_out=None):
+def bn_act(bn, x, residual=None, relu=True, grad_slot=None, ext_stats=None, pivot_out=None, out_tap=None):
     training, momentum, nbt, rmean, rvar = _bn_mode(bn)
     if momentum is None:
         nbt.add_(1)
@@ -860,7 +903,7 @@
                                 grad_slot)
     ext = ext_stats if (ext_stats is not None and training and ext_stats[0].numel() > 0) else None
     return _BNAct.apply(x, residual, bn.weight, bn.bias, rmean, rvar, training, momentum, bn.eps, relu, nbt, grad_slot, ext,
-                        pivot_out if training else None)
+                        pivot_out if training else None, out_tap)
 
 
 class _ConcatPool(torch.autograd.Function):
@@ -885,13 +928,14 @@
         return from_nhwc(dx)
 
 
-def conv_bn_act(conv, bn, x, residual=None, relu=True, conv_slot=None, bn_slot=None, conv_give=None):
+def conv_bn_act(conv, bn, x, residual=None, relu=True, conv_slot=None, bn_slot=None, conv_give=None, in_tap=None, out_tap=None):
     fuse = (bn.training and bn.track_running_stats and bn.running_mean is not None and bn.momentum is not None
             and getattr(bn, 'nnl_sync', None) is None and x.is_cuda and conv.bias is None and not conv.fuse_relu
             and torch.is_grad_enabled() and os.environ.get('NNL_BN_EPI_STATS', '1') != '0')
 
     def unfused(**kw):
-        return bn_act(bn, conv(x, grad_slot=conv_slot, give_slot=conv_give), residual=residual, relu=relu, grad_slot=bn_slot, **kw)
+        y = conv(x, grad_slot=conv_slot, give_slot=conv_give, in_tap=in_tap) if in_tap is not None else conv(x, grad_slot=conv_slot, give_slot=conv_give)
+        return bn_act(bn, y, residual=residual, relu=relu, grad_slot=bn_slot, out_tap=out_tap, **kw)
     if not fuse:
         return unfused()
     pivot = getattr(bn, '_nnl_pivot', None)
@@ -901,8 +945,8 @@
         pivot = torch.empty(bn.num_features, dtype=torch.float32, device=x.device)
         object.__setattr__(bn, '_nnl_pivot', pivot)
         return unfused(pivot_out=pivot)
-    y, part = conv2d_with_bn_stats(x, conv.weight, None, conv.stride[0], conv.padding[0], pivot, conv_slot, conv_give)
-    return bn_act(bn, y, residual=residual, relu=relu, grad_slot=bn_slot, ext_stats=(part, pivot), pivot_out=pivot)
+    y, part = conv2d_with_bn_stats(x, conv.weight, None, conv.stride[0], conv.padding[0], pivot, conv_slot, conv_give, in_tap)
+    return bn_act(bn, y, residual=residual, relu=relu, grad_slot=bn_slot, ext_stats=(part, pivot), pivot_out=pivot, out_tap=out_tap)
 
 
 def linear_relu_bn(lin, bn, x):
```

Result: slower. 5361 images/s (-3.3%).
